# terraytherapeutics/COATI

Hardware: AMD Instinct MI355X
Metric: molecules/sec (contrastive+AR train step), grande_closed (higher is better)
Workload: dtype bf16; 1 GPU; grande_closed d=256 L=16 nh=16 + E3GNN h=256x5, V=10322, batch 1024/GPU, seq_len 80, 16-atom point clouds, InfoNCE + AR loss, bf16 MFMA operands / fp32 accumulate + fp32 master weights, random-init weights; global_batch=1024, seq_len=80, parallelism=dp1

## Files before the change

coati_amd/_lib.py:

```python
import ctypes
import os

from . import _abi
from . import build as _build

try:
    with open(_build.HEADER) as _f:
        _ABI = _abi.parse(_f.read())
except OSError as e:
    raise RuntimeError(f"coati_amd: cannot read {_build.HEADER}, which the binding of libcoati_hip.so is derived from: {e}") from e
try:
    with open(_build.BEAM_HEADER) as _f:
        _BEAM_ABI = _abi.parse(_f.read(), guard="COATI_BEAM_H", name="coati_beam.h", base=_ABI)
except OSError as e:
    raise RuntimeError(f"coati_amd: cannot read {_build.BEAM_HEADER}, which the beam-search binding is derived from: {e}") from e
try:
    with open(_build.SEARCH_HEADER) as _f:
        _SEARCH_ABI = _abi.parse(_f.read(), guard="COATI_SEARCH_H", name="coati_search.h", base=_ABI)
except OSError as e:
    raise RuntimeError(f"coati_amd: cannot read {_build.SEARCH_HEADER}, which the library-search binding is derived from: {e}") from e
try:
    with open(_build.GRAMMAR_HEADER) as _f:
        _GRAMMAR_ABI = _abi.parse(_f.read(), guard="COATI_GRAMMAR_H", name="coati_grammar.h", base=_ABI)
except OSError as e:
    raise RuntimeError(f"coati_amd: cannot read {_build.GRAMMAR_HEADER}, which the constrained-decoding binding is derived from: {e}") from e
try:
    with open(_build.SCREEN_HEADER) as _f:
        _SCREEN_ABI = _abi.parse(_f.read(), guard="COATI_SCREEN_H", name="coati_screen.h", base=_ABI)
except OSError as e:
    raise RuntimeError(f"coati_amd: cannot read {_build.SCREEN_HEADER}, which the property-head binding is derived from: {e}") from e
try:
    with open(_build.GUIDE_HEADER) as _f:
        _GUIDE_ABI = _abi.parse(_f.read(), guard="COATI_GUIDE_H", name="coati_guide.h", base=_ABI)
except OSError as e:
    raise RuntimeError(f"coati_amd: cannot read {_build.GUIDE_HEADER}, which the head-gradient binding is derived from: {e}") from e
try:
    with open(_build.LN_XHAT_HEADER) as _f:
        _LN_XHAT_ABI = _abi.parse(_f.read(), guard="COATI_LN_XHAT_H", name="coati_ln_xhat.h", base=_ABI)
except OSError as e:
    raise RuntimeError(f"coati_amd: cannot read {_build.LN_XHAT_HEADER}, which the saved-xhat binding is derived from: {e}") from e
try:
    with open(_build.GP_HEADER) as _f:
        _GP_ABI = _abi.parse(_f.read(), guard="COATI_GP_H", name="coati_gp.h", base=_ABI)
except OSError as e:
    raise RuntimeError(f"coati_amd: cannot read {_build.GP_HEADER}, which the GP-head binding is derived from: {e}") from e
try:
    with open(_build.ACQ_HEADER) as _f:
        _ACQ_ABI = _abi.parse(_f.read(), guard="COATI_ACQ_H", name="coati_acq.h", base=_ABI)
except OSError as e:
    raise RuntimeError(f"coati_amd: cannot read {_build.ACQ_HEADER}, which the acquisition-gradient binding is derived from: {e}") from e
try:
    with open(_build.CLUSTER_HEADER) as _f:
        _CLUSTER_ABI = _abi.parse(_f.read(), guard="COATI_CLUSTER_H", name="coati_cluster.h", base=_ABI)
except OSError as e:
    raise RuntimeError(f"coati_amd: cannot read {_build.CLUSTER_HEADER}, which the library-clustering binding is derived from: {e}") from e
try:
    with open(_build.IVF_HEADER) as _f:
        _IVF_ABI = _abi.parse(_f.read(), guard="COATI_IVF_H", name="coati_ivf.h", base=_ABI)
except OSError as e:
    raise RuntimeError(f"coati_amd: cannot read {_build.IVF_HEADER}, which the IVF-search binding is derived from: {e}") from e
try:
    with open(_build.RADIUS_HEADER) as _f:
        _RADIUS_ABI = _abi.parse(_f.read(), guard="COATI_RADIUS_H", name="coati_radius.h", base=_ABI)
except OSError as e:
    raise RuntimeError(f"coati_amd: cannot read {_build.RADIUS_HEADER}, which the radius-search binding is derived from: {e}") from e
try:
    with open(_build.GNN_OPS_HEADER) as _f:
        _GNN_OPS_ABI = _abi.parse(_f.read(), guard="COATI_GNN_OPS_H", name="coati_gnn_ops.h", base=_ABI)
except OSError as e:
    raise RuntimeError(f"coati_amd: cannot read {_build.GNN_OPS_HEADER}, which the binding of the point encoder's single kernels is derived from: {e}") from e
try:
    with open(_build.SEARCH8_HEADER) as _f:
        _SEARCH8_ABI = _abi.parse(_f.read(), guard="COATI_SEARCH8_H", name="coati_search8.h", base=_ABI)
except OSError as e:
    raise RuntimeError(f"coati_amd: cannot read {_build.SEARCH8_HEADER}, which the quantised-search binding is derived from: {e}") from e
try:
    with open(_build.IVF8_HEADER) as _f:
        _IVF8_ABI = _abi.parse(_f.read(), guard="COATI_IVF8_H", name="coati_ivf8.h", base=_ABI)
except OSError as e:
    raise RuntimeError(f"coati_amd: cannot read {_build.IVF8_HEADER}, which the binding of the IVF search over fp8 lists is derived from: {e}") from e
try:
    with open(_build.IVF_RADIUS_HEADER) as _f:
        _IVF_RADIUS_ABI = _abi.parse(_f.read(), guard="COATI_IVF_RADIUS_H", name="coati_ivf_radius.h", base=_ABI)
except OSError as e:
    raise RuntimeError(f"coati_amd: cannot read {_build.IVF_RADIUS_HEADER}, which the binding of the radius search over inverted lists is derived from: {e}") from e
try:
    with open(_build.PQ_HEADER) as _f:
        _PQ_ABI = _abi.parse(_f.read(), guard="COATI_PQ_H", name="coati_pq.h", base=_ABI)
except OSError as e:
    raise RuntimeError(f"coati_amd: cannot read {_build.PQ_HEADER}, which the binding of the product-quantised search is derived from: {e}") from e
try:
    with open(_build.IVFPQ_HEADER) as _f:
        _IVFPQ_ABI = _abi.parse(_f.read(), guard="COATI_IVFPQ_H", name="coati_ivfpq.h", base=_ABI)
except OSError as e:
    raise RuntimeError(f"coati_amd: cannot read {_build.IVFPQ_HEADER}, which the binding of the IVF-PQ search is derived from: {e}") from e
try:
    with open(_build.SEARCH4_HEADER) as _f:
        _SEARCH4_ABI = _abi.parse(_f.read(), guard="COATI_SEARCH4_H", name="coati_search4.h", base=_ABI)
except OSError as e:
    raise RuntimeError(f"coati_amd: cannot read {_build.SEARCH4_HEADER}, which the binding of the four-bit search is derived from: {e}") from e

PROTOTYPES = _ABI.prototypes
CoatiConfig = _ABI.CoatiConfig
ABI_VERSION = _ABI.version
BEAM_PROTOTYPES = _BEAM_ABI.prototypes
SEARCH_PROTOTYPES = _SEARCH_ABI.prototypes
GRAMMAR_PROTOTYPES = _GRAMMAR_ABI.prototypes
SCREEN_PROTOTYPES = _SCREEN_ABI.prototypes
GUIDE_PROTOTYPES = _GUIDE_ABI.prototypes
LN_XHAT_PROTOTYPES = _LN_XHAT_ABI.prototypes
GP_PROTOTYPES = _GP_ABI.prototypes
ACQ_PROTOTYPES = _ACQ_ABI.prototypes
CLUSTER_PROTOTYPES = _CLUSTER_ABI.prototypes
IVF_PROTOTYPES = _IVF_ABI.prototypes
RADIUS_PROTOTYPES = _RADIUS_ABI.prototypes
GNN_OPS_PROTOTYPES = _GNN_OPS_ABI.prototypes
SEARCH8_PROTOTYPES = _SEARCH8_ABI.prototypes
IVF8_PROTOTYPES = _IVF8_ABI.prototypes
IVF_RADIUS_PROTOTYPES = _IVF_RADIUS_ABI.prototypes
PQ_PROTOTYPES = _PQ_ABI.prototypes
IVFPQ_PROTOTYPES = _IVFPQ_ABI.prototypes
SEARCH4_PROTOTYPES = _SEARCH4_ABI.prototypes

_lib = None


def has_experimental():
    return hasattr(lib(), "coati_attn_block_fwd")


def lib():
    global _lib
    if _lib is not None:
        return _lib
    path = _build.LIB
    try:
        _build.build(force=os.environ.get("COATI_AMD_REBUILD") == "1", verbose=False)
    except Exception:
        if not os.path.exists(path):
            raise
    if not os.path.exists(path):
        raise RuntimeError(f"coati_amd: {path} is missing and could not be built; there is no CPU fallback")
    import torch
    l = ctypes.CDLL(path)
    for name, (restype, argtypes) in list(PROTOTYPES.items()) + list(BEAM_PROTOTYPES.items()) + list(SEARCH_PROTOTYPES.items()) + list(GRAMMAR_PROTOTYPES.items()) + list(SCREEN_PROTOTYPES.items()) + list(GUIDE_PROTOTYPES.items()) + list(LN_XHAT_PROTOTYPES.items()) + list(GP_PROTOTYPES.items()) + list(ACQ_PROTOTYPES.items()) + list(CLUSTER_PROTOTYPES.items()) + list(IVF_PROTOTYPES.items()) + list(RADIUS_PROTOTYPES.items()) + list(GNN_OPS_PROTOTYPES.items()) + list(SEARCH8_PROTOTYPES.items()) + list(IVF8_PROTOTYPES.items()) + list(IVF_RADIUS_PROTOTYPES.items()) + list(PQ_PROTOTYPES.items()) + list(IVFPQ_PROTOTYPES.items()) + list(SEARCH4_PROTOTYPES.items()):
        if hasattr(l, name):
            getattr(l, name).restype = restype
            getattr(l, name).argtypes = argtypes
    if l.coati_abi_version() != ABI_VERSION:
        raise RuntimeError(f"coati_amd: {path} has ABI version {l.coati_abi_version()}, this package expects {ABI_VERSION}; "
                           "rebuild with `python -m coati_amd.build --force`")
    missing = [n for n in exported_symbols() + sorted(BEAM_PROTOTYPES) + sorted(SEARCH_PROTOTYPES) + sorted(GRAMMAR_PROTOTYPES) + sorted(SCREEN_PROTOTYPES) + sorted(GUIDE_PROTOTYPES) + sorted(LN_XHAT_PROTOTYPES) + sorted(GP_PROTOTYPES) + sorted(ACQ_PROTOTYPES) + sorted(CLUSTER_PROTOTYPES) + sorted(IVF_PROTOTYPES) + sorted(RADIUS_PROTOTYPES) + sorted(GNN_OPS_PROTOTYPES) + sorted(SEARCH8_PROTOTYPES) + sorted(IVF8_PROTOTYPES) + sorted(IVF_RADIUS_PROTOTYPES) + sorted(PQ_PROTOTYPES) + sorted(IVFPQ_PROTOTYPES) + sorted(SEARCH4_PROTOTYPES) if not hasattr(l, n)]
    if missing:
        raise RuntimeError(f"coati_amd: {path} lacks symbols {missing[:6]}; rebuild with `python -m coati_amd.build --force`")
    _lib = l
    return l


def exported_symbols():
    return sorted(n for n in PROTOTYPES if _build.EXPERIMENTAL or n not in _ABI.experimental)


def check(rc, what=""):
    if rc != 0:
        msg = lib().coati_last_error().decode("utf-8", "replace")
        raise RuntimeError(f"libcoati_hip: {what} failed (code {rc}): {msg}")


def call(name, *args):
    if name in _ABI.experimental and not hasattr(lib(), name):
        raise RuntimeError(f"libcoati_hip: {name} is an operator of csrc/experimental/ -- build and load with COATI_AMD_EXPERIMENTAL=1")
    check(getattr(lib(), name)(*args), name)
```

coati_amd/build.py:

```python
import os
import subprocess
import sys
from concurrent.futures import ThreadPoolExecutor

HERE = os.path.dirname(os.path.abspath(__file__))
CSRC = os.path.join(HERE, "csrc")
LIBDIR = os.path.join(HERE, "lib")
LIB = os.path.join(LIBDIR, "libcoati_hip_x.so" if os.environ.get("COATI_AMD_EXPERIMENTAL") == "1" else "libcoati_hip.so")
OBJDIR = os.path.join(HERE, "build")
HEADER = os.path.join(os.path.dirname(HERE), "include", "coati_hip.h")
BEAM_HEADER = os.path.join(os.path.dirname(HERE), "include", "coati_beam.h")
SEARCH_HEADER = os.path.join(os.path.dirname(HERE), "include", "coati_search.h")
GRAMMAR_HEADER = os.path.join(os.path.dirname(HERE), "include", "coati_grammar.h")
SCREEN_HEADER = os.path.join(os.path.dirname(HERE), "include", "coati_screen.h")
GUIDE_HEADER = os.path.join(os.path.dirname(HERE), "include", "coati_guide.h")
LN_XHAT_HEADER = os.path.join(os.path.dirname(HERE), "include", "coati_ln_xhat.h")
GP_HEADER = os.path.join(os.path.dirname(HERE), "include", "coati_gp.h")
ACQ_HEADER = os.path.join(os.path.dirname(HERE), "include", "coati_acq.h")
CLUSTER_HEADER = os.path.join(os.path.dirname(HERE), "include", "coati_cluster.h")
IVF_HEADER = os.path.join(os.path.dirname(HERE), "include", "coati_ivf.h")
RADIUS_HEADER = os.path.join(os.path.dirname(HERE), "include", "coati_radius.h")
GNN_OPS_HEADER = os.path.join(os.path.dirname(HERE), "include", "coati_gnn_ops.h")
SEARCH8_HEADER = os.path.join(os.path.dirname(HERE), "include", "coati_search8.h")
IVF8_HEADER = os.path.join(os.path.dirname(HERE), "include", "coati_ivf8.h")
IVF_RADIUS_HEADER = os.path.join(os.path.dirname(HERE), "include", "coati_ivf_radius.h")
PQ_HEADER = os.path.join(os.path.dirname(HERE), "include", "coati_pq.h")
IVFPQ_HEADER = os.path.join(os.path.dirname(HERE), "include", "coati_ivfpq.h")
SEARCH4_HEADER = os.path.join(os.path.dirname(HERE), "include", "coati_search4.h")
HIP_UNITS = ["gemm.hip", "gemm_rb.hip", "gemm_rb16.hip", "gemm_ring.hip", "gemm_mx8.hip", "norm.hip", "attention.hip", "attention16.hip", "embed.hip", "gnn.hip", "loss.hip", "optim.hip", "batch.hip", "decode.hip", "beam.hip", "search.hip", "grammar.hip", "screen.hip", "guide.hip", "gp.hip", "gp_grad.hip", "cluster.hip", "ivf.hip", "radius.hip", "search8.hip", "ivf8.hip", "ivf_radius.hip", "pq.hip", "ivfpq.hip", "search4.hip"]
CPP_UNITS = ["engine.cpp", "capi.cpp", "tokenizer.cpp", "comm.cpp"]
FLAGS = ["--offload-arch=gfx950", "-O3", "-std=c++17", "-fPIC", "-Wno-unused-value", "-mllvm", "-amdgpu-mfma-vgpr-form=1"] + os.environ.get("COATI_AMD_CXXFLAGS", "").split()


EXPERIMENTAL = os.environ.get("COATI_AMD_EXPERIMENTAL") == "1"
EXPERIMENTAL_UNITS = ["experimental/attn_block.hip", "experimental/mlp64.hip", "experimental/gemm_t32.hip"]
if EXPERIMENTAL:
    HIP_UNITS = HIP_UNITS + EXPERIMENTAL_UNITS
    FLAGS = FLAGS + ["-DCOATI_EXPERIMENTAL"]
UNIT_DROP_FLAGS = {"experimental/mlp64.hip": ("-mllvm", "-amdgpu-mfma-vgpr-form=1")}


def _hipcc():
    for c in (os.environ.get("HIPCC"), "/opt/rocm/bin/hipcc", "hipcc"):
        if c and (os.path.isabs(c) and os.path.exists(c) or not os.path.isabs(c)):
            return c
    return "hipcc"


def _sources():
    deps = [os.path.join(CSRC, f) for f in os.listdir(CSRC) if not os.path.isdir(os.path.join(CSRC, f))]
    if EXPERIMENTAL:
        deps += [os.path.join(CSRC, "experimental", f) for f in os.listdir(os.path.join(CSRC, "experimental"))]
    deps += [HEADER, BEAM_HEADER, SEARCH_HEADER, GRAMMAR_HEADER, SCREEN_HEADER, GUIDE_HEADER, LN_XHAT_HEADER, GP_HEADER, ACQ_HEADER, CLUSTER_HEADER, IVF_HEADER, RADIUS_HEADER, GNN_OPS_HEADER, SEARCH8_HEADER, IVF8_HEADER, IVF_RADIUS_HEADER, PQ_HEADER, IVFPQ_HEADER, SEARCH4_HEADER]
    return deps


def _stamp_path():
    return LIB + ".flags"


def needs_build():
    if not os.path.exists(LIB):
        return True
    try:
        with open(_stamp_path()) as f:
            if f.read() != " ".join(FLAGS):
                return True
    except OSError:
        return True
    t = os.path.getmtime(LIB)
    return any(os.path.getmtime(p) > t for p in _sources())


def build(force=False, verbose=True):
    if not force and not needs_build():
        return LIB
    os.makedirs(LIBDIR, exist_ok=True)
    os.makedirs(OBJDIR, exist_ok=True)
    import fcntl
    with open(os.path.join(LIBDIR, ".build.lock"), "w") as lock:
        fcntl.flock(lock, fcntl.LOCK_EX)
        try:
            if not force and not needs_build():
                return LIB
            return _build_locked(verbose)
        finally:
            fcntl.flock(lock, fcntl.LOCK_UN)


def _build_locked(verbose):
    hipcc = _hipcc()

    def compile_one(unit):
        src = os.path.join(CSRC, unit)
        obj = os.path.join(OBJDIR, unit.replace("/", "_") + (".x.o" if EXPERIMENTAL else ".o"))
        flags = [f for f in FLAGS if f not in UNIT_DROP_FLAGS.get(unit, ())]
        cmd = [hipcc] + flags + (["-x", "hip"] if unit.endswith(".cpp") else []) + ["-c", src, "-o", obj]
        r = subprocess.run(cmd, capture_output=True, text=True)
        if r.returncode != 0:
            raise RuntimeError(f"hipcc failed on {unit}:\n{r.stderr}")
        return obj

    with ThreadPoolExecutor(max_workers=8) as ex:
        objs = list(ex.map(compile_one, HIP_UNITS + CPP_UNITS))
    tmp = LIB + f".tmp{os.getpid()}"
    r = subprocess.run([hipcc, "--offload-arch=gfx950", "-shared", "-fPIC"] + objs + ["-lpthread", "-ldl", "-o", tmp], capture_output=True, text=True)
    if r.returncode != 0:
        raise RuntimeError(f"link failed:\n{r.stderr}")
    os.replace(tmp, LIB)
    with open(_stamp_path(), "w") as f:
        f.write(" ".join(FLAGS))
    if verbose:
        print(f"[coati_amd] built {LIB}", file=sys.stderr)
    return LIB


if __name__ == "__main__":
    build(force="--force" in sys.argv)
```

coati_amd/csrc/capi.cpp:

```cpp
#include <string.h>

#include "../../include/coati_hip.h"
#include "../../include/coati_beam.h"
#include "../../include/coati_search.h"
#include "../../include/coati_grammar.h"
#include "../../include/coati_screen.h"
#include "../../include/coati_guide.h"
#include "../../include/coati_ln_xhat.h"
#include "../../include/coati_gp.h"
#include "../../include/coati_acq.h"
#include "../../include/coati_cluster.h"
#include "../../include/coati_ivf.h"
#include "../../include/coati_radius.h"
#include "../../include/coati_search8.h"
#include "../../include/coati_ivf8.h"
#include "../../include/coati_ivf_radius.h"
#include "../../include/coati_pq.h"
#include "../../include/coati_ivfpq.h"
#include "../../include/coati_search4.h"
#include "../../include/coati_gnn_ops.h"
#include <vector>
#include "kernels.h"

#define S_(x) ((hipStream_t)(x))
#define LL(x) (reinterpret_cast<const long long*>(x))

extern "C" {

int coati_gemm_nt(const void* A, int a_f32, int64_t lda, const uint16_t* B, int64_t ldb, int M, int N, int K,
                  void* C, int64_t ldc, int n_store, const float* bias, const void* aux_in, void* aux_out,
                  int64_t ld_aux, int epi, void* stream) {
  COATI_CHECK_ARG((epi >= EPI_BF16 && epi <= EPI_ACC_F32) || epi == EPI_GELU_GRAD || epi == EPI_MUL_AUX, "coati_gemm_nt: epilogue %d is not a plain epilogue", epi);
  GemmArgs a;
  memset(&a, 0, sizeof(a));
  a.A = A; a.lda = lda; a.B = B; a.ldb = ldb; a.M = M; a.N = N; a.K = K; a.C = C; a.ldc = ldc; a.n_store = n_store;
  a.bias = bias; a.aux_in = aux_in; a.aux_out = aux_out; a.ld_aux = ld_aux;
  return launch_gemm_nt(a, a_f32, epi, S_(stream));
}

#ifdef COATI_EXPERIMENTAL
int coati_mlp_fwd(const float* x, const float* gamma, const float* beta, uint16_t* a2, float* mean, float* rstd, const uint16_t* W1,
                  const float* b1, const uint16_t* W2, const float* b2, uint16_t* g, uint8_t* codes, float* out, int M, void* stream) {
  COATI_CHECK_SHAPE(M >= 1 && M <= 65536, "mlp_fwd: M=%d out of range", M);
  Mlp64Args a;
  a.x = x; a.ldx = 256; a.gamma = gamma; a.beta = beta; a.a2 = a2; a.mean = mean; a.rstd = rstd; a.W1 = W1; a.b1 = b1; a.W2 = W2; a.b2 = b2;
  a.g = g; a.codes = codes; a.out = out; a.ldo = 256; a.M = M;
  return launch_mlp64_fwd(a, S_(stream));
}
#endif

int coati_gemm_lnbwd(const uint16_t* dY, int64_t lda, const uint16_t* WT, int64_t ldw, int M, int K, const float* x, const float* mean,
                     const float* rstd, const float* gamma, const float* dres, float* dx, uint16_t* dx16, float* partial,
                     int32_t* n_partial_rows, const uint16_t* chain_W, uint16_t* chain_C, void* stream) {
  COATI_CHECK_ARG(dY && WT && x && mean && rstd && gamma && dres && dx && partial && n_partial_rows, "gemm_lnbwd: null argument");
  GemmArgs a;
  memset(&a, 0, sizeof(a));
  a.A = dY; a.lda = lda; a.B = WT; a.ldb = ldw; a.M = M; a.N = 256; a.K = K; a.C = dx; a.ldc = 256; a.aux_in = dres; a.ld_aux = 256;
  a.aux_out = dx16; a.lnb_x = x; a.lnb_ldx = 256; a.lnb_mean = mean; a.lnb_rstd = rstd; a.lnb_gamma = gamma; a.lnb_partial = partial;
  COATI_CHECK_ARG((chain_W == nullptr) == (chain_C == nullptr) && (chain_W == nullptr || dx16 != nullptr), "gemm_lnbwd: the chained product needs chain_W, chain_C and dx16");
  a.chain_W = chain_W; a.chain_ldw = 256; a.chain_C = chain_C; a.chain_ldc = 256;
  int nwg = 0;
  COATI_CHECK_SHAPE(gemm_ring_lnbwd_supported(a, &nwg), "gemm_lnbwd: unsupported shape M=%d K=%d (256 columns, 40 961 .. 57 344 rows, K %% 64 == 0)", M, K);
  *n_partial_rows = nwg;
  return launch_gemm_nt(a, 0, EPI_LNBWD, S_(stream));
}

int coati_gemm_lnbwd_xhat(const uint16_t* dY, int64_t lda, const uint16_t* WT, int64_t ldw, int M, int K, const uint16_t* xhat, const float* rstd,
                          const float* gamma, const float* dres, float* dx, uint16_t* dx16, float* partial, int32_t* n_partial_rows,
                          const uint16_t* chain_W, uint16_t* chain_C, void* stream) {
  COATI_CHECK_ARG(dY && WT && xhat && rstd && gamma && dres && dx && partial && n_partial_rows, "gemm_lnbwd_xhat: null argument");
  GemmArgs a;
  memset(&a, 0, sizeof(a));
  a.A = dY; a.lda = lda; a.B = WT; a.ldb = ldw; a.M = M; a.N = 256; a.K = K; a.C = dx; a.ldc = 256; a.aux_in = dres; a.ld_aux = 256;
  a.aux_out = dx16; a.lnb_xhat = xhat; a.lnb_rstd = rstd; a.lnb_gamma = gamma; a.lnb_partial = partial;
  COATI_CHECK_ARG((chain_W == nullptr) == (chain_C == nullptr) && (chain_W == nullptr || dx16 != nullptr), "gemm_lnbwd_xhat: the chained product needs chain_W, chain_C and dx16");
  a.chain_W = chain_W; a.chain_ldw = 256; a.chain_C = chain_C; a.chain_ldc = 256;
  int nwg = 0;
  COATI_CHECK_SHAPE(gemm_ring_lnbwd_supported(a, &nwg), "gemm_lnbwd_xhat: unsupported shape M=%d K=%d (256 columns, 40 961 .. 57 344 rows, K %% 64 == 0)", M, K);
  *n_partial_rows = nwg;
  return launch_gemm_nt(a, 0, EPI_LNBWD, S_(stream));
}

int coati_gemm_ln_gelu_grad(const float* x, int64_t ldx, const float* gamma, const float* beta, const uint16_t* W, int64_t ldw, const float* bias,
                            int M, int N, uint16_t* saved, float* mean, float* rstd, uint16_t* g, uint8_t* codes, int save_xhat, void* stream) {
  COATI_CHECK_ARG(x && gamma && beta && W && saved && mean && rstd && g && codes, "gemm_ln_gelu_grad: null argument");
  COATI_CHECK_SHAPE(M > 0 && N > 0 && N % 16 == 0 && ldx >= 256 && ldx % 4 == 0 && ldw >= 256 && ldw % 8 == 0, "gemm_ln_gelu_grad: shape / alignment (M=%d N=%d ldx=%lld ldw=%lld)", M, N, (long long)ldx, (long long)ldw);
  GemmArgs a;
  memset(&a, 0, sizeof(a));
  a.A = saved; a.lda = 256; a.B = W; a.ldb = ldw; a.M = M; a.N = N; a.K = 256; a.C = g; a.ldc = N; a.bias = bias; a.aux_out = codes; a.ld_aux = N;
  a.ln_x = x; a.ln_ldx = ldx; a.ln_gamma = gamma; a.ln_beta = beta; a.ln_mean = mean; a.ln_rstd = rstd; a.ln_save_xhat = save_xhat ? 1 : 0;
  COATI_CHECK_SHAPE(gemm_rb16_supported(a, 0, EPI_GELU_GRAD), "gemm_ln_gelu_grad: the LayerNorm-fused 16-row-slab kernel takes 36 865 .. 65 536 rows (M=%d N=%d)", M, N);
  return launch_gemm_rb16(a, EPI_GELU_GRAD, S_(stream));
}

int coati_quant_mx8(const void* x, int x_f32, int64_t ldx, uint8_t* q, int64_t ldq, uint8_t* scales, int M, int K, void* stream) {
  return launch_quant_mx8(x, x_f32, ldx, q, ldq, scales, M, K, S_(stream));
}
int coati_gemm_mx8(const uint8_t* A, int64_t lda, const uint8_t* a_scales, const uint8_t* W, int64_t ldw, const uint8_t* w_scales,
                   int M, int N, int K, void* C, int64_t ldc, const float* bias, const void* aux_in, void* aux_out, int64_t ld_aux,
                   int epi, void* stream) {
  GemmArgs a;
  memset(&a, 0, sizeof(a));
  a.A = A; a.lda = lda; a.B = reinterpret_cast<const bf16_t*>(W); a.ldb = ldw; a.M = M; a.N = N; a.K = K; a.C = C; a.ldc = ldc;
  a.bias = bias; a.aux_in = aux_in; a.aux_out = aux_out; a.ld_aux = ld_aux;
  COATI_CHECK_ARG(epi != EPI_QKV_ROPE, "gemm_mx8: the rotary epilogue is an engine-internal call");
  return launch_gemm_mx8(a, a_scales, w_scales, epi, S_(stream));
}
int coati_gemm_ce_partial(const uint16_t* A, int64_t lda, const uint16_t* W, int64_t ldw, int M, int V, int K,
                          void* partial, void* stream) {
  GemmArgs a;
  memset(&a, 0, sizeof(a));
  a.A = A; a.lda = lda; a.B = W; a.ldb = ldw; a.M = M; a.N = V; a.K = K; a.partial = reinterpret_cast<float2*>(partial);
  return launch_gemm_nt(a, 0, EPI_CE_PARTIAL, S_(stream));
}

int coati_ce_finish(const void* partial, int tiles_n, const uint16_t* A, int64_t lda, const uint16_t* W,
                    int64_t ldw, const int64_t* target, float* lse, float* scal, int M, int K, int V, void* stream) {
  return launch_ce_finish(reinterpret_cast<const float2*>(partial), tiles_n, A, lda, W, ldw, LL(target), lse, scal, M, K, V, S_(stream));
}

int coati_gemm_ce_bwd(const uint16_t* A, int64_t lda, const uint16_t* W, int64_t ldw, int M, int V, int K,
                      uint16_t* dlogits, int64_t ldd, int n_store, const float* lse, const int64_t* target,
                      const float* scal, void* stream) {
  GemmArgs a;
  memset(&a, 0, sizeof(a));
  a.A = A; a.lda = lda; a.B = W; a.ldb = ldw; a.M = M; a.N = V; a.K = K; a.C = dlogits; a.ldc = ldd; a.n_store = n_store;
  a.lse = lse; a.target = LL(target); a.scal = scal;
  return launch_gemm_nt(a, 0, EPI_CE_BWD, S_(stream));
}

int coati_wgrad(const void* A, int a_f32, int64_t lda, const uint16_t* B, int64_t ldb, int M, int N, int K,
                float* dW, int64_t ldw, float* dbias, int n_out, void* stream) {
  WgradArgs a;
  a.A = A; a.lda = lda; a.B = B; a.ldb = ldb; a.M = M; a.N = N; a.K = K; a.dW = dW; a.ldw = ldw; a.dbias = dbias; a.n_out = n_out;
  return launch_wgrad(a, a_f32, S_(stream));
}

int64_t coati_wgrad_grouped_workspace_bytes(int n_problems, const int* N, const int* K, int tile_size) {
  if (n_problems <= 0 || !N || !K || (tile_size != 128 && tile_size != 256)) return 0;
  int64_t tiles = 0;
  for (int i = 0; i < n_problems; ++i) tiles += (int64_t)cdiv(N[i], tile_size) * cdiv(K[i], tile_size);
  return tiles * (int64_t)sizeof(WgradTile);
}

int coati_wgrad_grouped(int n_problems, const uint16_t* const* A, const int64_t* lda, const uint16_t* const* B, const int64_t* ldb,
                        int M, const int* N, const int* K, float* const* dW, const int64_t* ldw, float* const* dbias, int tile_size,
                        void* workspace, int64_t workspace_bytes, void* stream) {
  return coati_wgrad_grouped_affine(n_problems, A, lda, B, ldb, M, N, K, dW, ldw, dbias, nullptr, nullptr, tile_size, workspace, workspace_bytes, stream);
}

int coati_wgrad_grouped_affine(int n_problems, const uint16_t* const* A, const int64_t* lda, const uint16_t* const* B, const int64_t* ldb,
                               int M, const int* N, const int* K, float* const* dW, const int64_t* ldw, float* const* dbias,
                               const float* const* b_gamma, const float* const* b_beta, int tile_size, void* workspace, int64_t workspace_bytes,
                               void* stream) {
  COATI_CHECK_ARG(n_problems > 0 && A && lda && B && ldb && N && K && dW && ldw && dbias && workspace, "wgrad_grouped: null argument");
  COATI_CHECK_ARG((b_gamma == nullptr) == (b_beta == nullptr), "wgrad_grouped: b_gamma and b_beta come together");
  std::vector<WgradTile> tab;
  for (int i = 0; i < n_problems; ++i) {
    WgradArgs a;
    a.A = A[i]; a.lda = lda[i]; a.B = B[i]; a.ldb = ldb[i]; a.M = M; a.N = N[i]; a.K = K[i]; a.dW = dW[i]; a.ldw = ldw[i]; a.dbias = dbias[i]; a.n_out = 0;
    if (b_gamma != nullptr) { a.b_gamma = b_gamma[i]; a.b_beta = b_beta[i]; }
    COATI_TRY(wgrad_table_append(tab, a, tile_size));
  }
  COATI_CHECK_ARG((int64_t)(tab.size() * sizeof(WgradTile)) <= workspace_bytes, "wgrad_grouped: workspace too small (%zu tiles)", tab.size());
  hipStream_t s = S_(stream);
  if (hipMemcpyAsync(workspace, tab.data(), tab.size() * sizeof(WgradTile), hipMemcpyHostToDevice, s) != hipSuccess ||
      hipStreamSynchronize(s) != hipSuccess) {
    coati_set_error("wgrad_grouped: table upload failed");
    return COATI_EHIP;
  }
  return launch_wgrad_table(reinterpret_cast<const WgradTile*>(workspace), (int)tab.size(), s, tile_size);
}

int coati_sgemm(const float* A, int64_t ars, int64_t acs, const float* B, int64_t brs, int64_t bcs, float* C,
                int64_t ldc, int M, int N, int K, const float* bias, float alpha, int accumulate, void* stream) {
  return launch_sgemm(A, ars, acs, B, brs, bcs, C, ldc, M, N, K, bias, alpha, accumulate, S_(stream));
}

int coati_layernorm_fwd(const float* x, int64_t ldx, const float* gamma, const float* beta, uint16_t* y16,
                        int64_t ld16, float* y32, int64_t ld32, float* mean, float* rstd, int M, int C, void* stream) {
  return launch_layernorm_fwd(x, ldx, gamma, beta, y16, ld16, y32, ld32, mean, rstd, M, C, S_(stream));
}
int coati_layernorm_bwd(const void* dy, int dy_f32, int64_t lddy, const float* x, int64_t ldx, int x_is_xhat,
                        const float* mean, const float* rstd, const float* gamma, const float* dres, float* dx,
                        uint16_t* dx16, float* dgamma, float* dbeta, float* partial, int M, int C, void* stream) {
  return launch_layernorm_bwd(dy, dy_f32, lddy, x, ldx, x_is_xhat, mean, rstd, gamma, dres, dx, dx16, dgamma, dbeta, partial, M, C, S_(stream));
}

int coati_attn_fwd(const uint16_t* qkv, uint16_t* y, float* lse, int B, int T, int n_head, void* stream) {
  return launch_attn_fwd(qkv, y, lse, B, T, n_head, 16, S_(stream));
}
int coati_attn_fwd_hs(const uint16_t* qkv, uint16_t* y, float* lse, int B, int T, int n_head, int head_size, void* stream) {
  return launch_attn_fwd(qkv, y, lse, B, T, n_head, head_size, S_(stream));
}
int coati_seq_pack(const int64_t* tok, const int64_t* y, int pad_token, int B, int T, int rows_expect, int32_t* off,
                   int32_t* row_src, int32_t* row_t, int64_t* ypk, int32_t* err, void* stream) {
  return launch_seq_pack(LL(tok), LL(y), pad_token, B, T, rows_expect, off, row_src, row_t, reinterpret_cast<long long*>(ypk), err, S_(stream));
}
int coati_attn_fwd_varlen(const uint16_t* qkv, uint16_t* y, float* lse, const int32_t* seq_off, int B, int T, int n_head,
                          int head_size, void* stream) {
  COATI_CHECK_ARG(seq_off, "attn_fwd_varlen: null seq_off");
  return launch_attn_fwd(qkv, y, lse, B, T, n_head, head_size, S_(stream), seq_off);
}
int coati_attn_bwd_varlen(const uint16_t* qkv, const uint16_t* y, const uint16_t* dy, const float* lse, float* dscratch,
                          uint16_t* dqkv, const float* cos_t, const float* sin_t, const int32_t* seq_off, int B, int T,
                          int n_head, int head_size, void* stream) {
  COATI_CHECK_ARG(seq_off, "attn_bwd_varlen: null seq_off");
  return launch_attn_bwd(qkv, y, dy, lse, dscratch, dqkv, cos_t, sin_t, B, T, n_head, head_size, S_(stream), seq_off);
}
#ifdef COATI_EXPERIMENTAL
int coati_attn_groups(const int32_t* seq_off, int B, int T, int32_t* grp, void* stream) {
  return launch_attn_groups(seq_off, B, T, grp, S_(stream));
}
int coati_attn_block_fwd(const float* x, float* xmid, const float* ln_g, const float* ln_b, float* mean, float* rstd, uint16_t* a1,
                         const uint16_t* Wqkv, const float* bqkv, const uint16_t* Wproj, const float* bproj, uint16_t* qkv, uint16_t* y,
                         float* lse, const float* cos_t, const float* sin_t, const int32_t* row_src, const int32_t* grp, int T, int M,
                         void* stream) {
  AttnBlockArgs a;
  a.x = x; a.xmid = xmid; a.ln_g = ln_g; a.ln_b = ln_b; a.mean = mean; a.rstd = rstd; a.a1 = a1; a.Wqkv = Wqkv; a.bqkv = bqkv;
  a.Wproj = Wproj; a.bproj = bproj; a.qkv = qkv; a.y = y; a.lse = lse; a.cos_t = cos_t; a.sin_t = sin_t; a.row_src = row_src;
  a.grp = grp; a.Tl = T; a.M = M;
  return launch_attn_block_fwd(a, S_(stream));
}
int coati_ab_probe_swap(uint32_t* out, void* stream) { return launch_ab_probe_swap(out, S_(stream)); }
#endif
int coati_gemm_qkv_rope(const uint16_t* A, int64_t lda, const uint16_t* W, int64_t ldw, const float* bias, int M, int C,
                        uint16_t* qkv, int64_t ldc, const float* cos_t, const float* sin_t, int T, void* stream) {
  GemmArgs a;
  memset(&a, 0, sizeof(a));
  a.A = A; a.lda = lda; a.B = W; a.ldb = ldw; a.M = M; a.N = 3 * C; a.K = C; a.C = qkv; a.ldc = ldc; a.bias = bias;
  a.rope_cos = cos_t; a.rope_sin = sin_t; a.rope_T = T; a.rope_C = C; a.rope_hs = 16;
  return launch_gemm_nt(a, 0, EPI_QKV_ROPE, S_(stream));
}
int coati_gemm_qkv_rope_hs(const uint16_t* A, int64_t lda, const uint16_t* W, int64_t ldw, const float* bias, int M, int C,
                           uint16_t* qkv, int64_t ldc, const float* cos_t, const float* sin_t, int T, int head_size, void* stream) {
  GemmArgs a;
  memset(&a, 0, sizeof(a));
  a.A = A; a.lda = lda; a.B = W; a.ldb = ldw; a.M = M; a.N = 3 * C; a.K = C; a.C = qkv; a.ldc = ldc; a.bias = bias;
  a.rope_cos = cos_t; a.rope_sin = sin_t; a.rope_T = T; a.rope_C = C; a.rope_hs = head_size;
  return launch_gemm_nt(a, 0, EPI_QKV_ROPE, S_(stream));
}
int coati_attn_bwd(const uint16_t* qkv, const uint16_t* y, const uint16_t* dy, const float* lse, float* dscratch, uint16_t* dqkv,
                   const float* cos_t, const float* sin_t, int B, int T, int n_head, void* stream) {
  return launch_attn_bwd(qkv, y, dy, lse, dscratch, dqkv, cos_t, sin_t, B, T, n_head, 16, S_(stream));
}
int coati_attn_bwd_hs(const uint16_t* qkv, const uint16_t* y, const uint16_t* dy, const float* lse, float* dscratch, uint16_t* dqkv,
                      const float* cos_t, const float* sin_t, int B, int T, int n_head, int head_size, void* stream) {
  return launch_attn_bwd(qkv, y, dy, lse, dscratch, dqkv, cos_t, sin_t, B, T, n_head, head_size, S_(stream));
}

int coati_embed_fwd(const int64_t* idx, const float* table, const float* injection, int unk_token, float* x, int B,
                    int T, int C, int V, void* stream) {
  return launch_embed_fwd(LL(idx), table, injection, unk_token, x, B, T, C, V, S_(stream));
}
int coati_embed_bwd(const int64_t* idx, const float* dx, float* dtable, float* dinjection, int unk_token, int B, int T,
                    int C, int V, void* stream) {
  return launch_embed_bwd(LL(idx), dx, dtable, dinjection, unk_token, B, T, C, V, S_(stream));
}
int coati_find_stop(const int64_t* idx, int stop_token, int32_t* pos, int32_t* err, int B, int T, void* stream) {
  return launch_find_stop(LL(idx), stop_token, pos, err, B, T, S_(stream));
}
int coati_gather_rows(const float* x, const int32_t* pos, float* out, int B, int T, int C, void* stream) {
  return launch_gather_rows(x, pos, out, B, T, C, S_(stream));
}
int coati_scatter_rows_add(const float* dout, const int32_t* pos, float* dx, int B, int T, int C, void* stream) {
  return launch_scatter_rows_add(dout, pos, dx, B, T, C, S_(stream));
}
int coati_bad_rows(const int64_t* tokens, uint8_t* bad, int B, int T, void* stream) {
  return launch_bad_rows(LL(tokens), bad, B, T, S_(stream));
}
int coati_silu(const float* x, float* y, int64_t n, void* stream) { return launch_silu_fwd(x, y, n, S_(stream)); }
int coati_swiglu(const float* u, int64_t ldu, float* g, int64_t ldg, int B, int N, void* stream) {
  return launch_swiglu(u, ldu, g, ldg, B, N, S_(stream));
}
int coati_swiglu_bwd(const float* u, int64_t ldu, const float* dg, int64_t lddg, float* du, int64_t lddu, int B, int N, void* stream) {
  return launch_swiglu_bwd(u, ldu, dg, lddg, du, lddu, B, N, S_(stream));
}
int coati_group_mean_rows(const float* x, int64_t ldx, const int32_t* off, const float* w, const float* fallback, float* out, int G, int E,
                          void* stream) {
  return launch_group_mean_rows(x, ldx, off, w, fallback, out, G, E, S_(stream));
}
int coati_attn_decode(const uint16_t* qkv, uint16_t* cache, uint16_t* y, int B, int n_head, int Tmax, int pos, void* stream) {
  return launch_attn_decode(qkv, cache, y, B, n_head, 16, Tmax, pos, nullptr, S_(stream));
}
int coati_attn_decode_hs(const uint16_t* qkv, uint16_t* cache, uint16_t* y, int B, int n_head, int head_size, int Tmax, int pos, void* stream) {
  return launch_attn_decode(qkv, cache, y, B, n_head, head_size, Tmax, pos, nullptr, S_(stream));
}
int coati_topk_sample(const float* logits, int64_t ldl, int B, int V, int k, float inv_temp, const float* u,
                      int64_t* tokens_out, int32_t* stopped, int stop_token, int pad_token, void* stream) {
  return launch_topk_sample(logits, ldl, B, V, k, inv_temp, u, reinterpret_cast<long long*>(tokens_out), stopped, stop_token, pad_token, S_(stream));
}
int coati_topk_sample_prompt(const float* logits, int64_t ldl, int B, int V, int k, float inv_temp, const float* u, const int64_t* prompt,
                             int64_t ldp, const int32_t* plen, int pos, int64_t* tokens_out, int32_t* stopped, int stop_token, int pad_token,
                             void* stream) {
  return launch_topk_sample_prompt(logits, ldl, B, V, k, inv_temp, u, LL(prompt), ldp, plen, pos, reinterpret_cast<long long*>(tokens_out),
                                   stopped, stop_token, pad_token, S_(stream));
}
int coati_attn_decode_rows(const uint16_t* qkv, uint16_t* cache, uint16_t* y, int B, int n_head, int head_size, int Tmax, const int32_t* pos,
                           void* stream) {
  return launch_attn_decode_rows(qkv, cache, y, B, n_head, head_size, Tmax, pos, S_(stream));
}
int coati_attn_decode_anc(const uint16_t* qkv, uint16_t* cache, uint16_t* y, int B, int n_head, int head_size, int Tmax, int pos,
                          const int32_t* anc, void* stream) {
  return launch_attn_decode_anc(qkv, cache, y, B, n_head, head_size, Tmax, pos, anc, S_(stream));
}
int coati_beam_row_topk(const float* logits, int64_t ldl, int G, int W, int V, const float* cum, const int32_t* fin, int pad_token,
                        float* cand_score, int32_t* cand_tok, void* stream) {
  return launch_beam_row_topk(logits, ldl, G, W, V, cum, fin, pad_token, cand_score, cand_tok, S_(stream));
}
int coati_beam_merge(const float* cand_score, const int32_t* cand_tok, int G, int W, const float* cum_in, const int32_t* fin_in,
                     const int32_t* len_in, const int32_t* anc_in, const int64_t* hist_in, int64_t ldh, int Tmax, int pos, int n,
                     int stop_token, float* cum_out, int32_t* fin_out, int32_t* len_out, int32_t* anc_out, int64_t* hist_out,
                     int64_t* tok_next, int32_t* nfin, void* stream) {
  return launch_beam_merge(cand_score, cand_tok, G, W, cum_in, fin_in, len_in, anc_in, LL(hist_in), ldh, Tmax, pos, n, stop_token, cum_out,
                           fin_out, len_out, anc_out, reinterpret_cast<long long*>(hist_out), reinterpret_cast<long long*>(tok_next), nfin,
                           S_(stream));
}
int coati_search_topk(const uint16_t* lib, int64_t N, int E, const float* bias, const uint16_t* q, int Q, int k, float alpha, int S,
                      float* part_score, int32_t* part_row, float* out_score, int64_t* out_row, void* stream) {
  return launch_search_topk(lib, N, E, bias, q, Q, k, alpha, S, part_score, part_row, out_score, reinterpret_cast<long long*>(out_row),
                            S_(stream));
}
int coati_search_slices(int64_t N, int Q, int k) { return search_slices(N, Q, k); }
int coati_grammar_step(float* logits, int64_t ldl, int B, int V, const uint64_t* table, const int32_t* state_in, int32_t* state_out,
                       const int64_t* tok_prev, const int32_t* parent, int remaining, int stop_token, void* stream) {
  return launch_grammar_step(logits, ldl, B, V, reinterpret_cast<const unsigned long long*>(table), state_in, state_out, LL(tok_prev), parent,
                             remaining, stop_token, S_(stream));
}
int coati_head_eval(const uint16_t* x, int64_t ldx, int64_t N, int E, const uint16_t* w0, const float* b0, const uint16_t* wr, const float* br,
                    int D, const float* wl, const float* bl, int P, int F, float* out, int64_t ldo, void* stream) {
  return launch_head_eval(x, ldx, N, E, w0, b0, wr, br, D, wl, bl, P, F, out, ldo, S_(stream));
}

int coati_head_grad(const uint16_t* x, int64_t ldx, int64_t N, int E, const uint16_t* w0, const float* b0, const uint16_t* wr, const float* br,
                    int D, const float* wl, const float* bl, int P, int F, const uint16_t* w0t, const uint16_t* wrt, const float* cot,
                    int64_t ldc, float* out, int64_t ldo, float* g, int64_t ldg, void* stream) {
  return launch_head_grad(x, ldx, N, E, w0, b0, wr, br, D, wl, bl, P, F, w0t, wrt, cot, ldc, out, ldo, g, ldg, S_(stream));
}
int coati_head_gp(const uint16_t* x, int64_t ldx, int64_t N, int E, const uint16_t* w0, const float* b0, const uint16_t* wr, const float* br,
                  int D, int F, const float* wl, const float* bl, int P_lin, float* out, int64_t ldo, const uint16_t* z, const float* zn,
                  const float* alpha, const float* q, const float* c, float inv2l2, float s2, int P, int Mp, float* mean, int64_t ldm,
                  float* var, void* stream) {
  return launch_head_gp(x, ldx, N, E, w0, b0, wr, br, D, F, wl, bl, P_lin, out, ldo, z, zn, alpha, q, c, inv2l2, s2, P, Mp, mean, ldm, var,
                        S_(stream));
}
int coati_head_gp_grad(const uint16_t* x, int64_t ldx, int64_t N, int E, const uint16_t* w0, const float* b0, const uint16_t* wr,
                       const float* br, int D, int F, const uint16_t* w0t, const uint16_t* wrt, const uint16_t* z, const uint16_t* zt,
                       const float* zn, const float* alpha, const float* qs, const float* c, float inv2l2, float s2, int P, int Mp,
                       const float* wm, float kappa, float var_add, int mode, float best, const float* rs, float* mean, int64_t ldm,
                       float* var, float* acq, float* g, int64_t ldg, void* stream) {
  return launch_head_gp_grad(x, ldx, N, E, w0, b0, wr, br, D, F, w0t, wrt, z, zt, zn, alpha, qs, c, inv2l2, s2, P, Mp, wm, kappa, var_add, mode,
                             best, rs, mean, ldm, var, acq, g, ldg, S_(stream));
}
int coati_cluster_assign(const uint16_t* lib, int64_t N, int E, const float* row_bias, const uint16_t* c, int K, const float* cbias,
                         int32_t* assign, float* best, int blocks, void* stream) {
  return launch_cluster_assign(lib, N, E, row_bias, c, K, cbias, assign, best, blocks, S_(stream));
}
int coati_cluster_sums(const uint16_t* lib, int64_t N, int E, const int32_t* order, int64_t M, const int32_t* offsets,
                       const int32_t* item_off, int K, float* part, int64_t items_max, float* sums, int blocks, void* stream) {
  return launch_cluster_sums(lib, N, E, order, M, offsets, item_off, K, part, items_max, sums, blocks, S_(stream));
}
int coati_cluster_chunk(void) { return cluster_chunk(); }
int64_t coati_cluster_items_max(int64_t M, int K) { return cluster_items_max(M, K); }
int coati_ivf_scan(const uint16_t* lib, const int32_t* ids, const float* bias, const int32_t* list_off, int64_t M, int E, int L,
                   const uint16_t* q, int Q, const int32_t* pair_q, const int32_t* pair_off, const int32_t* item_off, int64_t P, int k,
                   float alpha, int seg_rows, int segs, float* part_score, int32_t* part_row, int blocks, void* stream) {
  return launch_ivf_scan(lib, ids, bias, list_off, M, E, L, q, Q, pair_q, pair_off, item_off, P, k, alpha, seg_rows, segs, part_score, part_row,
                         blocks, S_(stream));
}
int coati_ivf_merge(const float* part_score, const int32_t* part_row, const int32_t* probes, const int32_t* pair_slot, int64_t P,
                    const int32_t* list_off, int L, int Q, int nprobe, int k, int seg_rows, int segs, float* out_score, int64_t* out_row,
                    void* stream) {
  return launch_ivf_merge(part_score, part_row, probes, pair_slot, P, list_off, L, Q, nprobe, k, seg_rows, segs, out_score,
                          reinterpret_cast<long long*>(out_row), S_(stream));
}
int64_t coati_ivf_plan(int64_t max_list_rows, int Q, int nprobe, int k) { return ivf_plan(max_list_rows, Q, nprobe, k); }
int coati_ivf8_scan(const uint8_t* lib8, const float* scale, const int32_t* ids, const float* bias, const int32_t* list_off, int64_t M, int E,
                    int L, const uint8_t* q8, const float* qscale, int Q, const int32_t* pair_q, const int32_t* pair_off,
                    const int32_t* item_off, int64_t P, int k, float alpha, int seg_rows, int segs, float* part_score, int32_t* part_row,
                    int blocks, void* stream) {
  return launch_ivf8_scan(lib8, scale, ids, bias, list_off, M, E, L, q8, qscale, Q, pair_q, pair_off, item_off, P, k, alpha, seg_rows, segs,
                          part_score, part_row, blocks, S_(stream));
}
int coati_radius_count(const uint16_t* lib, int64_t N, int E, const float* bias, const uint16_t* q, int Q, float alpha, const float* sub,
                       int clamp0, const float* thr, const int32_t* row_hi, int S, int32_t* counts, void* stream) {
  return launch_radius_count(lib, N, E, bias, q, Q, alpha, sub, clamp0, thr, row_hi, S, counts, S_(stream));
}
int coati_radius_fill(const uint16_t* lib, int64_t N, int E, const float* bias, const uint16_t* q, int Q, float alpha, const float* sub,
                      int clamp0, const float* thr, const int32_t* row_hi, int S, const int32_t* counts, const int64_t* offsets,
                      float* out_score, int64_t* out_row, void* stream) {
  return launch_radius_fill(lib, N, E, bias, q, Q, alpha, sub, clamp0, thr, row_hi, S, counts, LL(offsets), out_score,
                            reinterpret_cast<long long*>(out_row), S_(stream));
}
int coati_radius_slices(int64_t N, int Q) { return radius_slices(N, Q); }
int coati_ivf_radius_count(const uint16_t* lib, const int32_t* ids, const float* bias, const int32_t* list_off, int64_t M, int E, int L,
                           const uint16_t* q, int Q, const int32_t* pair_q, const int32_t* pair_off, const int32_t* item_off, int64_t P,
                           float alpha, const float* sub, int clamp0, const float* thr, const int32_t* row_hi, int seg_rows, int segs,
                           int32_t* counts, int blocks, void* stream) {
  return launch_ivf_radius_count(lib, ids, bias, list_off, M, E, L, q, Q, pair_q, pair_off, item_off, P, alpha, sub, clamp0, thr, row_hi, seg_rows,
                                 segs, counts, blocks, S_(stream));
}
int coati_ivf_radius_fill(const uint16_t* lib, const int32_t* ids, const float* bias, const int32_t* list_off, int64_t M, int E, int L,
                          const uint16_t* q, int Q, const int32_t* pair_q, const int32_t* pair_off, const int32_t* item_off, int64_t P,
                          float alpha, const float* sub, int clamp0, const float* thr, const int32_t* row_hi, int seg_rows, int segs,
                          const int32_t* counts, const int64_t* offsets, float* out_score, int64_t* out_row, int blocks, void* stream) {
  return launch_ivf_radius_fill(lib, ids, bias, list_off, M, E, L, q, Q, pair_q, pair_off, item_off, P, alpha, sub, clamp0, thr, row_hi, seg_rows,
                                segs, counts, LL(offsets), out_score, reinterpret_cast<long long*>(out_row), blocks, S_(stream));
}
int coati_quant_rows_fp8(const uint16_t* x, int64_t n, int E, uint8_t* out, float* scale, void* stream) {
  return launch_quant_rows_fp8(x, n, E, out, scale, S_(stream));
}
int coati_search8_topk(const uint8_t* lib8, const float* scale, int64_t N, int E, const float* bias, const uint8_t* q8, const float* qscale,
                       int Q, int k, float alpha, int S, float* part_score, int32_t* part_row, float* out_score, int64_t* out_row,
                       void* stream) {
  return launch_search8_topk(lib8, scale, N, E, bias, q8, qscale, Q, k, alpha, S, part_score, part_row, out_score,
                             reinterpret_cast<long long*>(out_row), S_(stream));
}
int coati_search_rescore(const uint16_t* lib, int64_t N, int E, const float* bias, const uint16_t* q, int Q, const int64_t* cand, int R, int k,
                         float alpha, float* out_score, int64_t* out_row, void* stream) {
  return launch_search_rescore(lib, N, E, bias, q, Q, LL(cand), R, k, alpha, out_score, reinterpret_cast<long long*>(out_row), S_(stream));
}
int coati_search8_slices(int64_t N, int Q, int k) { return search8_slices(N, Q, k); }
int coati_pq_encode(const uint16_t* x, int64_t n, int E, const uint16_t* codebook, uint8_t* codes, void* stream) {
  return launch_pq_encode(x, n, E, codebook, codes, S_(stream));
}
int coati_pq_topk(const uint8_t* codes, int64_t N, int E, const uint16_t* codebook, const float* bias, const uint16_t* q, int Q, int k,
                  float alpha, int S, float* part_score, int32_t* part_row, float* out_score, int64_t* out_row, void* stream) {
  return launch_pq_topk(codes, N, E, codebook, bias, q, Q, k, alpha, S, part_score, part_row, out_score, reinterpret_cast<long long*>(out_row),
                        S_(stream));
}
int coati_pq_k_max(int E) { return pq_k_max(E); }
int coati_pq_slices(int64_t N, int E, int Q, int k) { return pq_slices(N, E, Q, k); }
int coati_ivfpq_scan(const uint8_t* codes, const int32_t* ids, const float* bias, const int32_t* list_off, int64_t M, int E, int L,
                     const uint16_t* centres, const uint16_t* codebook, const uint16_t* q, int Q, const int32_t* pair_q,
                     const int32_t* pair_off, const int32_t* item_off, int64_t P, int k, float alpha, int seg_rows, int segs,
                     float* part_score, int32_t* part_row, int blocks, void* stream) {
  return launch_ivfpq_scan(codes, ids, bias, list_off, M, E, L, centres, codebook, q, Q, pair_q, pair_off, item_off, P, k, alpha, seg_rows, segs,
                           part_score, part_row, blocks, S_(stream));
}
int coati_ivfpq_k_max(int E) { return ivfpq_k_max(E); }
int coati_quant_rows_fp4(const uint16_t* x, int64_t n, int E, uint8_t* codes, uint8_t* scales, void* stream) {
  return launch_quant_rows_fp4(x, n, E, codes, scales, S_(stream));
}
int coati_search4_topk(const uint8_t* codes, const uint8_t* scales, int64_t N, int E4, const float* bias, const uint8_t* q8,
                       const float* qscale, int Q, int k, float alpha, int S, float* part_score, int32_t* part_row, float* out_score,
                       int64_t* out_row, void* stream) {
  return launch_search4_topk(codes, scales, N, E4, bias, q8, qscale, Q, k, alpha, S, part_score, part_row, out_score,
                             reinterpret_cast<long long*>(out_row), S_(stream));
}
int coati_search4_slices(int64_t N, int Q, int k) { return search4_slices(N, Q, k); }
int coati_topk_sample_rows(const float* logits, int64_t ldl, int B, int V, int k, float inv_temp, const float* u, int64_t ldu,
                           const int64_t* prompt, int64_t ldp, const int32_t* plen, const int32_t* req, int32_t* pos, int64_t* out, int64_t ldo,
                           int64_t* tok_next, int32_t* done, int Tmax, int stop_token, void* stream) {
  return launch_topk_sample_rows(logits, ldl, B, V, k, inv_temp, u, ldu, LL(prompt), ldp, plen, req, pos, reinterpret_cast<long long*>(out), ldo,
                                 reinterpret_cast<long long*>(tok_next), done, Tmax, stop_token, S_(stream));
}
int coati_batch_ncols(const int64_t* tokens, int B, int n_seq, int32_t* ncols, void* stream) {
  return launch_batch_ncols(LL(tokens), B, n_seq, ncols, S_(stream));
}
int coati_batch_tail(const int64_t* tokens, int B, int n_seq, int ncol, int64_t* tokens_out, int64_t* y_next_out,
                     const int64_t* masked_ids, int n_masked, void* stream) {
  return launch_batch_tail(LL(tokens), B, n_seq, ncol, reinterpret_cast<long long*>(tokens_out),
                           reinterpret_cast<long long*>(y_next_out), LL(masked_ids), n_masked, S_(stream));
}

int coati_gnn_embed(const int64_t* atoms, const int32_t* lut_ix, const int32_t* lut_iy, const float* W, const float* b,
                    float* h32, uint16_t* h16, int64_t ld16, float* rstd, float* mask, int BA, int H, void* stream) {
  return launch_gnn_embed(LL(atoms), lut_ix, lut_iy, W, b, h32, h16, ld16, rstd, mask, BA, H, S_(stream));
}
int coati_gnn_geom(const float* coords, const float* mask, float cutoff, float* d2, float* w, int B, int A, void* stream) {
  return launch_gnn_geom(coords, mask, cutoff, d2, w, B, A, S_(stream));
}
int coati_gnn_compact(const float* w_dense, const float* d2_dense, int32_t* seg, int32_t* n_edges, int32_t* e_bj, int32_t* e_bk,
                      int32_t* e_rev, float* e_d2, float* e_w, int32_t* pos, int B, int A, void* stream) {
  return launch_gnn_compact(w_dense, d2_dense, seg, n_edges, e_bj, e_bk, e_rev, e_d2, e_w, pos, B, A, S_(stream));
}

int coati_gnn_edge_pre(const uint16_t* P, int64_t ldp, const int32_t* seg, const int32_t* e_bk, const float* e_d2, const float* w1c,
                       int64_t w1c_stride, const float* b1, uint16_t* e1, int BA, int H, void* stream) {
  return launch_gnn_edge_pre_c(P, ldp, seg, e_bk, e_d2, w1c, w1c_stride, b1, e1, BA, H, S_(stream));
}
int coati_gnn_edge_reduce(const uint16_t* s2, const int32_t* seg, const float* e_w, uint16_t* mi, int64_t ldmi, int BA, int H, void* stream) {
  return launch_gnn_edge_reduce_c(s2, seg, e_w, mi, ldmi, BA, H, S_(stream));
}

int coati_gnn_edge_fwd_fused(const uint16_t* P, int64_t ldp, const int32_t* seg, const int32_t* e_bk, const float* e_d2, const float* e_w,
                             const float* w1c, int64_t w1c_stride, const float* b1, const uint16_t* W3, int64_t ldw, const float* b3,
                             uint16_t* e1, uint16_t* s2, uint16_t* mi, int64_t ldmi, int BA, int H, void* stream) {
  return launch_gnn_edge_fwd_fused(P, ldp, seg, e_bk, e_d2, e_w, w1c, w1c_stride, b1, W3, ldw, b3, e1, s2, mi, ldmi, BA, H, S_(stream));
}
int coati_gnn_edge_reduce_bwd(const uint16_t* dmi, int64_t lddmi, const uint16_t* s2, const int32_t* seg, const float* e_w, uint16_t* ds2,
                              int BA, int H, void* stream) {
  COATI_CHECK_SHAPE(BA > 0 && H > 0, "gnn_edge_reduce_bwd: empty problem");
  return launch_gnn_edge_reduce_bwd_c(dmi, lddmi, s2, seg, e_w, ds2, BA, H, S_(stream));
}
int coati_gnn_edge_pre_bwd(const uint16_t* dpre, const int32_t* seg, const int32_t* e_rev, const float* e_d2, uint16_t* dP, int64_t lddp,
                           float* dw1c, int64_t dw1c_stride, float* db1, int BA, int H, void* stream) {
  COATI_CHECK_SHAPE(BA > 0 && H > 0, "gnn_edge_pre_bwd: empty problem");
  return launch_gnn_edge_pre_bwd_c(dpre, seg, e_rev, e_d2, dP, lddp, dw1c, dw1c_stride, db1, BA, H, S_(stream));
}
int coati_gnn_node_res_silu(const float* u32, const int64_t* atoms, const int32_t* lut_ix, const int32_t* lut_iy, const float* W3c,
                            int64_t ldw, uint16_t* upre, uint16_t* t16, int BA, int H, void* stream) {
  COATI_CHECK_SHAPE(BA > 0 && H > 0, "gnn_node_res_silu: empty problem");
  return launch_gnn_node_res_silu(u32, LL(atoms), lut_ix, lut_iy, W3c, ldw, upre, t16, BA, H, S_(stream));
}
int coati_gnn_onehot_wgrad(const int64_t* atoms, const int32_t* lut_ix, const int32_t* lut_iy, const uint16_t* du, float* dW, int64_t ldw,
                           int BA, int H, void* stream) {
  COATI_CHECK_SHAPE(BA > 0 && H > 0, "gnn_onehot_wgrad: empty problem");
  return launch_gnn_onehot_wgrad(LL(atoms), lut_ix, lut_iy, du, dW, ldw, BA, H, S_(stream));
}
int coati_gnn_embed_bwd(const int64_t* atoms, const int32_t* lut_ix, const int32_t* lut_iy, const float* de, float* dW, float* db, int BA,
                        int H, void* stream) {
  COATI_CHECK_SHAPE(BA > 0 && H > 0, "gnn_embed_bwd: empty problem");
  return launch_gnn_embed_bwd(LL(atoms), lut_ix, lut_iy, de, dW, db, BA, H, S_(stream));
}
int coati_gnn_readout(const float* o, const float* mask, float* hp, int B, int A, int H, void* stream) {
  COATI_CHECK_SHAPE(B > 0 && A > 0 && H > 0, "gnn_readout: empty problem");
  return launch_gnn_readout(o, mask, hp, B, A, H, S_(stream));
}
int coati_gnn_readout_bwd(const float* dhp, const float* mask, uint16_t* dout, int B, int A, int H, void* stream) {
  COATI_CHECK_SHAPE(B > 0 && A > 0 && H > 0, "gnn_readout_bwd: empty problem");
  return launch_gnn_readout_bwd(dhp, mask, dout, B, A, H, S_(stream));
}
int coati_gemm_rows_dev(const int32_t* m_dev, const uint16_t* A, int64_t lda, const uint16_t* B, int64_t ldb, int M, int N, int K,
                        uint16_t* C, int64_t ldc, const float* bias, int epi, const uint16_t* P, int64_t ldp, const float* d2,
                        const float* w1c, int64_t w1c_stride, const float* b1, int natom, int H, const int32_t* e_bj,
                        const int32_t* e_bk, int32_t* resident, void* stream) {
  COATI_CHECK_ARG(m_dev && A && B && C && resident, "gemm_rows_dev: null argument");
  COATI_CHECK_ARG(epi == EPI_BF16 || epi == EPI_EDGE_DPRE, "gemm_rows_dev: epilogue %d (EPI_BF16 and EPI_EDGE_DPRE only)", epi);
  COATI_CHECK_SHAPE(M > 0 && N > 0 && K > 0, "gemm_rows_dev: empty problem");
  if (epi == EPI_EDGE_DPRE)
    COATI_CHECK_ARG(N == H && (e_bj == nullptr) == (e_bk == nullptr), "gemm_rows_dev: EPI_EDGE_DPRE needs N == H (N=%d H=%d) and e_bj with e_bk", N, H);
  GemmArgs a;
  memset(&a, 0, sizeof(a));
  a.m_dev = m_dev; a.A = A; a.lda = lda; a.B = B; a.ldb = ldb; a.M = M; a.N = N; a.K = K; a.C = C; a.ldc = ldc; a.bias = bias;
  a.P = P; a.ldp = ldp; a.d2 = d2; a.w1c = w1c; a.w1c_stride = w1c_stride; a.b1 = b1; a.natom = natom; a.H = H; a.e_bj = e_bj; a.e_bk = e_bk;
  *resident = gemm_rb16_resident_supported(a, 0, epi) ? 1 : 0;
  return launch_gemm_nt(a, 0, epi, S_(stream));
}
int coati_wgrad_rows_dev(const int32_t* m_dev, const uint16_t* A, int64_t lda, const uint16_t* B, int64_t ldb, int M, int N, int K,
                         float* dW, int64_t ldw, float* dbias, void* stream) {
  COATI_CHECK_ARG(m_dev, "wgrad_rows_dev: null m_dev");
  WgradArgs a;
  a.A = A; a.lda = lda; a.B = B; a.ldb = ldb; a.M = M; a.N = N; a.K = K; a.dW = dW; a.ldw = ldw; a.dbias = dbias; a.n_out = 0; a.m_dev = m_dev;
  return launch_wgrad(a, 0, S_(stream));
}
int64_t coati_wgrad_split_workspace_bytes(int n_problems, const int* N, const int* K, int n_splits) {
  if (n_problems <= 0 || !N || !K || n_splits < 1) return 0;
  int64_t entries = 0;
  for (int i = 0; i < n_problems; ++i) entries += (int64_t)cdiv(N[i], 128) * cdiv(K[i], 128) * n_splits;
  return entries * (int64_t)sizeof(WgradTile);
}
int coati_wgrad_split(int n_problems, const uint16_t* const* A, const int64_t* lda, const uint16_t* const* B, const int64_t* ldb, int M,
                      const int* N, const int* K, float* const* dW, const int64_t* ldw, float* const* dbias, int n_splits,
                      void* workspace, int64_t workspace_bytes, void* stream) {
  COATI_CHECK_ARG(n_problems > 0 && A && lda && B && ldb && N && K && dW && ldw && dbias && workspace, "wgrad_split: null argument");
  COATI_CHECK_ARG(n_splits >= 1, "wgrad_split: n_splits=%d", n_splits);
  std::vector<WgradTile> tab;
  for (int i = 0; i < n_problems; ++i) {
    WgradArgs a;
    a.A = A[i]; a.lda = lda[i]; a.B = B[i]; a.ldb = ldb[i]; a.M = M; a.N = N[i]; a.K = K[i]; a.dW = dW[i]; a.ldw = ldw[i]; a.dbias = dbias[i]; a.n_out = 0;
    COATI_TRY(wgrad_table_append_split(tab, a, n_splits));
  }
  COATI_CHECK_ARG((int64_t)(tab.size() * sizeof(WgradTile)) <= workspace_bytes, "wgrad_split: workspace too small (%zu entries)", tab.size());
  hipStream_t s = S_(stream);
  if (hipMemcpyAsync(workspace, tab.data(), tab.size() * sizeof(WgradTile), hipMemcpyHostToDevice, s) != hipSuccess ||
      hipStreamSynchronize(s) != hipSuccess) {
    coati_set_error("wgrad_split: table upload failed");
    return COATI_EHIP;
  }
  return launch_wgrad_split_table(reinterpret_cast<const WgradTile*>(workspace), (int)tab.size(), s);
}

int coati_infonce_rows(float* logits, int64_t ld, int R, int N, int label0, const uint8_t* bad, float* loss_sum,
                       const float* inv_count, float gscale, void* stream) {
  return launch_infonce_rows(logits, ld, R, N, label0, bad, loss_sum, inv_count, gscale, S_(stream));
}

int coati_count_valid(const uint8_t* bad, int n, float* count, float* inv, void* stream) {
  return launch_count_valid(bad, n, count, inv, S_(stream));
}
int coati_colsum2(const float* a, const float* b2, const uint8_t* bad, float* out, int B, int E, void* stream) {
  return launch_colsum2(a, b2, bad, out, B, E, S_(stream));
}
int coati_center_rows(const float* z, const uint8_t* bad, const float* sum, const float* count, float* zc, int B, int E, void* stream) {
  return launch_center_rows(z, bad, sum, count, zc, B, E, S_(stream));
}
int coati_standardize(const float* z, const uint8_t* bad, const float* stats, const float* count, float* zt, float* rsigma,
                      int B, int E, void* stream) {
  return launch_standardize(z, bad, stats, count, zt, rsigma, B, E, S_(stream));
}
int coati_barlow_dc(float* C, const float* count, float lam, float* loss, int E, void* stream) {
  return launch_barlow_dc(C, count, lam, loss, E, S_(stream));
}
int coati_standardize_bwd(const float* dzt, const float* zt, const uint8_t* bad, const float* rsigma, const float* m,
                          const float* count, float scale, float* dz, int B, int E, void* stream) {
  return launch_standardize_bwd(dzt, zt, bad, rsigma, m, count, scale, dz, B, E, S_(stream));
}

int coati_grad_sqnorm(const float* g, int64_t n, float* partial, int n_partial, float* out_norm, float max_norm,
                      float* out_coef, void* stream) {
  return launch_grad_sqnorm(g, n, partial, n_partial, out_norm, max_norm, out_coef, S_(stream));
}
int coati_adamw(float* p, const float* g, float* m, float* v, uint16_t* shadow, int64_t n, float lr, float b1, float b2,
                float eps, float wd, int step, const float* coef, float gscale, void* stream) {
  return launch_adamw(p, g, m, v, shadow, n, lr, b1, b2, eps, wd, step, coef, gscale, S_(stream));
}

}
```

coati_amd/csrc/embed.hip:

```cpp
#include "kernels.h"

__global__ __launch_bounds__(256) void embed_fwd_kernel(const long long* __restrict__ idx, const float* __restrict__ table,
                                                        const float* __restrict__ injection, int unk, float* __restrict__ x,
                                                        int M, int T, int C, int V, const int* __restrict__ row_src, int mode) {
  const int lane = threadIdx.x & 63, wave = threadIdx.x >> 6;
  const int m = blockIdx.x * 4 + wave;
  if (m >= M) return;
  const int ms = row_src ? row_src[m] : m;
  long long tok = idx[ms];
  const float* src;
  if (mode != 0) {
    if (tok != unk) return;
    float* dstz = x + (long long)m * C;
    if (mode == 2) {
      for (int c = lane * 4; c < C; c += 256) *reinterpret_cast<float4*>(dstz + c) = make_float4(0.f, 0.f, 0.f, 0.f);
      return;
    }
    src = injection + (long long)(ms / T) * C;
  } else if (injection != nullptr && tok == unk) {
    src = injection + (long long)(ms / T) * C;
  } else {
    if (tok < 0) tok = 0;
    if (tok >= V) tok = V - 1;
    src = table + tok * C;
  }
  float* dst = x + (long long)m * C;
  for (int c = lane * 4; c < C; c += 256) *reinterpret_cast<float4*>(dst + c) = *reinterpret_cast<const float4*>(src + c);
}

int launch_embed_fwd(const long long* idx, const float* table, const float* injection, int unk_token, float* x,
                     int B, int T, int C, int V, hipStream_t s, const int* row_src, int rows, int mode) {
  COATI_CHECK_ARG(idx && x && (mode != 0 || table) && (mode != 1 || injection) && mode >= 0 && mode <= 2, "embed_fwd: null operand / bad mode");
  COATI_CHECK_SHAPE(B > 0 && T > 0 && C % 4 == 0 && V > 0, "embed_fwd: unsupported shape");
  const int M = row_src ? rows : B * T;
  hipLaunchKernelGGL(embed_fwd_kernel, dim3(cdiv(M, 4)), dim3(256), 0, s, idx, table, injection, unk_token, x, M, T, C, V, row_src, mode);
  COATI_LAUNCH_CHECK("embed_fwd");
  return COATI_OK;
}

#define EMB_RUN 32
__global__ __launch_bounds__(256) void embed_bwd_kernel(const long long* __restrict__ idx, const float* __restrict__ dx,
                                                        float* __restrict__ dtable, float* __restrict__ dinj, int unk,
                                                        int B, int T, int C, int V, const int* __restrict__ off, int inj_only) {
  const int lane = threadIdx.x & 63, wave = threadIdx.x >> 6;
  const int t = blockIdx.x;
  const int b0 = (blockIdx.y * 4 + wave) * EMB_RUN;
  if (b0 >= B) return;
  const int b1 = (b0 + EMB_RUN < B) ? b0 + EMB_RUN : B;
  for (int c0 = 0; c0 < C; c0 += 256) {
    float* cur = nullptr;
    float acc[4] = {0.f, 0.f, 0.f, 0.f};
    auto flush = [&]() {
      if (cur == nullptr) return;
#pragma unroll
      for (int i = 0; i < 4; ++i) {
        const int c = c0 + lane + 64 * i;
        if (c < C && acc[i] != 0.f) atomicAdd(cur + c, acc[i]);
      }
    };
    for (int b = b0; b < b1; ++b) {
      long long m = (long long)b * T + t;
      long long tok = idx[m];
      if (off != nullptr) {
        const int o = off[b];
        if (t >= off[b + 1] - o) continue;
        m = o + t;
      }
      float* dst;
      if (inj_only && tok != unk) continue;
      if (dinj != nullptr && tok == unk) {
        dst = dinj + (long long)b * C;
      } else {
        if (tok < 0) tok = 0;
        if (tok >= V) tok = V - 1;
        dst = dtable + tok * C;
      }
      float g[4];
#pragma unroll
      for (int i = 0; i < 4; ++i) {
        const int c = c0 + lane + 64 * i;
        g[i] = c < C ? dx[m * C + c] : 0.f;
      }
      if (dst != cur) {
        flush();
        cur = dst;
#pragma unroll
        for (int i = 0; i < 4; ++i) acc[i] = g[i];
      } else {
#pragma unroll
        for (int i = 0; i < 4; ++i) acc[i] += g[i];
      }
    }
    flush();
  }
}

int launch_embed_bwd(const long long* idx, const float* dx, float* dtable, float* dinjection, int unk_token,
                     int B, int T, int C, int V, hipStream_t s, const int* off, int inj_only) {
  COATI_CHECK_ARG(idx && dx && (dtable || inj_only) && (!inj_only || dinjection), "embed_bwd: null operand");
  COATI_CHECK_SHAPE(B > 0 && T > 0 && C % 4 == 0 && V > 0, "embed_bwd: unsupported shape");
  hipLaunchKernelGGL(embed_bwd_kernel, dim3(T, cdiv(B, 4 * EMB_RUN)), dim3(256), 0, s, idx, dx, dtable, dinjection, unk_token, B, T, C, V, off, inj_only);
  COATI_LAUNCH_CHECK("embed_bwd");
  return COATI_OK;
}

__global__ __launch_bounds__(256) void find_stop_kernel(const long long* __restrict__ idx, int stop, int* __restrict__ pos, int* __restrict__ err,
                                                        int B, int T) {
  const int lane = threadIdx.x & 63, b = blockIdx.x * 4 + (threadIdx.x >> 6);
  if (b >= B) return;
  int n = 0, p = 0;
  for (int t0 = 0; t0 < T; t0 += 64) {
    const int t = t0 + lane;
    const bool hit = t < T && idx[(long long)b * T + t] == stop;
    const unsigned long long m = __ballot(hit);
    if (m != 0ull) {
      if (n == 0) p = t0 + __builtin_ctzll(m);
      n += __builtin_popcountll(m);
    }
  }
  if (lane == 0) {
    pos[b] = p;
    if (n != 1) atomicOr(err, 1);
  }
}

int launch_find_stop(const long long* idx, int stop_token, int* pos, int* err, int B, int T, hipStream_t s) {
  COATI_CHECK_ARG(idx && pos && err, "find_stop: null operand");
  hipLaunchKernelGGL(find_stop_kernel, dim3(cdiv(B, 4)), dim3(256), 0, s, idx, stop_token, pos, err, B, T);
  COATI_LAUNCH_CHECK("find_stop");
  return COATI_OK;
}

__global__ __launch_bounds__(256) void gather_rows_kernel(const float* __restrict__ x, const int* __restrict__ pos,
                                                          float* __restrict__ out, int B, int T, int C, const int* __restrict__ off) {
  const int lane = threadIdx.x & 63, b = blockIdx.x * 4 + (threadIdx.x >> 6);
  if (b >= B) return;
  const float* src = x + ((off ? (long long)off[b] : (long long)b * T) + pos[b]) * C;
  for (int c = lane * 4; c < C; c += 256) *reinterpret_cast<float4*>(out + (long long)b * C + c) = *reinterpret_cast<const float4*>(src + c);
}

int launch_gather_rows(const float* x, const int* pos, float* out, int B, int T, int C, hipStream_t s, const int* off) {
  COATI_CHECK_ARG(x && pos && out, "gather_rows: null operand");
  hipLaunchKernelGGL(gather_rows_kernel, dim3(cdiv(B, 4)), dim3(256), 0, s, x, pos, out, B, T, C, off);
  COATI_LAUNCH_CHECK("gather_rows");
  return COATI_OK;
}

__global__ __launch_bounds__(256) void scatter_rows_add_kernel(const float* __restrict__ dout, const int* __restrict__ pos,
                                                               float* __restrict__ dx, int B, int T, int C, const int* __restrict__ off) {
  const int lane = threadIdx.x & 63, b = blockIdx.x * 4 + (threadIdx.x >> 6);
  if (b >= B) return;
  float* dst = dx + ((off ? (long long)off[b] : (long long)b * T) + pos[b]) * C;
  for (int c = lane * 4; c < C; c += 256) {
    float4 d = *reinterpret_cast<float4*>(dst + c);
    const float4 g = *reinterpret_cast<const float4*>(dout + (long long)b * C + c);
    d.x += g.x; d.y += g.y; d.z += g.z; d.w += g.w;
    *reinterpret_cast<float4*>(dst + c) = d;
  }
}

__global__ __launch_bounds__(256) void scatter_rows_bf16_kernel(const bf16_t* __restrict__ src, const int* __restrict__ pos,
                                                                bf16_t* __restrict__ dst, int B, int T, int C, const int* __restrict__ off) {
  const int lane = threadIdx.x & 63, b = blockIdx.x * 4 + (threadIdx.x >> 6);
  if (b >= B) return;
  bf16_t* d = dst + ((off ? (long long)off[b] : (long long)b * T) + pos[b]) * C;
  for (int c = lane * 8; c < C; c += 512) *reinterpret_cast<uint4*>(d + c) = *reinterpret_cast<const uint4*>(src + (long long)b * C + c);
}
int launch_scatter_rows_bf16(const bf16_t* src, const int* pos, bf16_t* dst, int B, int T, int C, hipStream_t s, const int* off) {
  COATI_CHECK_ARG(src && pos && dst && C % 8 == 0, "scatter_rows_bf16: null operand / C % 8");
  hipLaunchKernelGGL(scatter_rows_bf16_kernel, dim3(cdiv(B, 4)), dim3(256), 0, s, src, pos, dst, B, T, C, off);
  COATI_LAUNCH_CHECK("scatter_rows_bf16");
  return COATI_OK;
}

int launch_scatter_rows_add(const float* dout, const int* pos, float* dx, int B, int T, int C, hipStream_t s, const int* off) {
  COATI_CHECK_ARG(dout && pos && dx, "scatter_rows_add: null operand");
  hipLaunchKernelGGL(scatter_rows_add_kernel, dim3(cdiv(B, 4)), dim3(256), 0, s, dout, pos, dx, B, T, C, off);
  COATI_LAUNCH_CHECK("scatter_rows_add");
  return COATI_OK;
}

__global__ __launch_bounds__(256) void seq_len_kernel(const long long* __restrict__ tok, const long long* __restrict__ y, int pad,
                                                      int* __restrict__ len, int B, int T) {
  const int lane = threadIdx.x & 63, b = blockIdx.x * 4 + (threadIdx.x >> 6);
  if (b >= B) return;
  int last = 0;
  for (int t = lane; t < T; t += 64) {
    const bool live = tok[(long long)b * T + t] != pad || (y != nullptr && y[(long long)b * T + t] >= 0);
    if (live) last = t + 1;
  }
#pragma unroll
  for (int o = 32; o > 0; o >>= 1) { const int v = __shfl_xor(last, o, 64); last = v > last ? v : last; }
  if (lane == 0) len[b] = last;
}
__global__ __launch_bounds__(1024) void seq_scan_kernel(int* __restrict__ off, int B, int expect, int* __restrict__ err, int* __restrict__ ord) {
  __shared__ int part[1024];
  __shared__ int cnt[10], cur[10];
  const int t = threadIdx.x, per = (B + 1023) / 1024;
  const int lo = t * per, hi = lo + per < B ? lo + per : B;
  if (t < 10) cnt[t] = 0;
  __syncthreads();
  int sum = 0;
  for (int i = lo; i < hi; ++i) {
    const int l = off[i];
    sum += l;
    if (ord != nullptr) { const int nb = (l + 15) >> 4; atomicAdd(&cnt[9 - (nb < 9 ? nb : 9)], 1); }
  }
  part[t] = sum;
  __syncthreads();
  if (t == 0) { int run = 0; for (int k = 0; k < 10; ++k) { cur[k] = run; run += cnt[k]; } }
  for (int o = 1; o < 1024; o <<= 1) {
    const int v = t >= o ? part[t - o] : 0;
    __syncthreads();
    part[t] += v;
    __syncthreads();
  }
  int run = part[t] - sum;
  for (int i = lo; i < hi; ++i) {
    const int l = off[i];
    off[i] = run;
    run += l;
    if (ord != nullptr) { const int nb = (l + 15) >> 4; ord[atomicAdd(&cur[9 - (nb < 9 ? nb : 9)], 1)] = i; }
  }
  if (t == 1023) {
    off[B] = part[1023];
    if (part[1023] != expect) atomicOr(err, 2);
  }
}
__global__ void seq_fill_kernel(const int* __restrict__ off, const long long* __restrict__ y, int* __restrict__ row_src,
                                int* __restrict__ row_t, long long* __restrict__ ypk, int B, int T, int cap) {
  const long long g = (long long)blockIdx.x * blockDim.x + threadIdx.x;
  if (g >= (long long)B * T) return;
  {
    const long long m = (long long)off[B] + g;
    if (m < cap) {
      row_src[m] = 0;
      row_t[m] = 0;
      if (ypk != nullptr) ypk[m] = -1;
    }
  }
  const int b = (int)(g / T), t = (int)(g - (long long)b * T);
  const int o = off[b];
  if (t >= off[b + 1] - o) return;
  const int m = o + t;
  if (m >= cap) return;
  row_src[m] = (int)g;
  row_t[m] = t;
  if (ypk != nullptr) ypk[m] = y[g];
}
int launch_seq_pack(const long long* tok, const long long* y, int pad_token, int B, int T, int rows_expect, int* off,
                    int* row_src, int* row_t, long long* ypk, int* err, hipStream_t s, int* ord) {
  COATI_CHECK_ARG(tok && off && row_src && row_t && err && (ypk == nullptr || y != nullptr), "seq_pack: null operand");
  COATI_CHECK_SHAPE(B > 0 && T > 0 && rows_expect > 0 && rows_expect <= (long long)B * T, "seq_pack: bad row count %d for %d x %d", rows_expect, B, T);
  hipLaunchKernelGGL(seq_len_kernel, dim3(cdiv(B, 4)), dim3(256), 0, s, tok, y, pad_token, off, B, T);
  hipLaunchKernelGGL(seq_scan_kernel, dim3(1), dim3(1024), 0, s, off, B, rows_expect, err, ord);
  hipLaunchKernelGGL(seq_fill_kernel, dim3(cdiv((long long)B * T, 256)), dim3(256), 0, s, off, y, row_src, row_t, ypk, B, T, rows_expect);
  COATI_LAUNCH_CHECK("seq_pack");
  return COATI_OK;
}

int launch_seq_pack_len(const int* len, int B, int T, int rows_expect, int* off, int* row_src, int* row_t, int* err, hipStream_t s, int* ord) {
  COATI_CHECK_ARG(len && off && row_src && row_t && err, "seq_pack_len: null operand");
  COATI_CHECK_SHAPE(B > 0 && T > 0 && rows_expect > 0 && rows_expect <= (long long)B * T, "seq_pack_len: bad row count %d for %d x %d", rows_expect, B, T);
  hipError_t h = hipMemcpyAsync(off, len, sizeof(int) * B, hipMemcpyDeviceToDevice, s);
  if (h != hipSuccess) { coati_set_error("seq_pack_len: hipMemcpyAsync failed: %s", hipGetErrorString(h)); return COATI_EHIP; }
  hipLaunchKernelGGL(seq_scan_kernel, dim3(1), dim3(1024), 0, s, off, B, rows_expect, err, ord);
  hipLaunchKernelGGL(seq_fill_kernel, dim3(cdiv((long long)B * T, 256)), dim3(256), 0, s, off, (const long long*)nullptr, row_src, row_t,
                     (long long*)nullptr, B, T, rows_expect);
  COATI_LAUNCH_CHECK("seq_pack_len");
  return COATI_OK;
}

__global__ void bad_rows_kernel(const long long* __restrict__ tok, unsigned char* __restrict__ bad, int B, int T) {
  const int b = blockIdx.x * blockDim.x + threadIdx.x;
  if (b >= B) return;
  long long sum = 0;
  for (int t = 0; t < T; ++t) sum += tok[(long long)b * T + t];
  bad[b] = sum < 1 ? 1 : 0;
}

int launch_bad_rows(const long long* tokens, unsigned char* bad, int B, int T, hipStream_t s) {
  COATI_CHECK_ARG(tokens && bad, "bad_rows: null operand");
  hipLaunchKernelGGL(bad_rows_kernel, dim3(cdiv(B, 128)), dim3(128), 0, s, tokens, bad, B, T);
  COATI_LAUNCH_CHECK("bad_rows");
  return COATI_OK;
}

__device__ __forceinline__ float ce_target_logit(const bf16_t* __restrict__ a, long long lda, const bf16_t* __restrict__ W, long long ldw,
                                                 long long tgt, long long row, int C, int lane) {
  float dot = 0.f;
  for (int c = lane * 4; c < C; c += 256) {
    const uint2 ua = *reinterpret_cast<const uint2*>(a + row * lda + c);
    const uint2 uw = *reinterpret_cast<const uint2*>(W + tgt * ldw + c);
    dot += bflo(ua.x) * bflo(uw.x) + bfhi(ua.x) * bfhi(uw.x) + bflo(ua.y) * bflo(uw.y) + bfhi(ua.y) * bfhi(uw.y);
  }
  return wave_sum(dot);
}
__device__ __forceinline__ float ce_row(const float2* __restrict__ partial, int tiles_n, const bf16_t* __restrict__ a, long long lda,
                                        const bf16_t* __restrict__ W, long long ldw, long long tgt, long long row, int C, int V,
                                        float* __restrict__ lse_out, int lane, bool* valid) {
  float mx = -INFINITY;
  for (int t = lane; t < tiles_n; t += 64) mx = fmaxf(mx, partial[row * tiles_n + t].x);
  mx = wave_max(mx);
  float sm = 0.f;
  for (int t = lane; t < tiles_n; t += 64) {
    const float2 p = partial[row * tiles_n + t];
    sm += p.y * __expf(p.x - mx);
  }
  sm = wave_sum(sm);
  const float l = mx + __logf(sm);
  if (lse_out != nullptr && lane == 0) *lse_out = l;
  *valid = tgt >= 0 && tgt < V;
  if (!*valid) return 0.f;
  return l - ce_target_logit(a, lda, W, ldw, tgt, row, C, lane);
}

__global__ __launch_bounds__(256) void ce_finish_kernel(const float2* __restrict__ partial, int tiles_n,
                                                        const bf16_t* __restrict__ a, long long lda,
                                                        const bf16_t* __restrict__ W, long long ldw,
                                                        const long long* __restrict__ target, float* __restrict__ lse,
                                                        float* __restrict__ scal, int M, int C, int V) {
  __shared__ float red[2][4];
  const int lane = threadIdx.x & 63, wave = threadIdx.x >> 6;
  float loss_acc = 0.f, cnt_acc = 0.f;
  for (int row = blockIdx.x * 4 + wave; row < M; row += gridDim.x * 4) {
    bool valid;
    const float d = ce_row(partial, tiles_n, a, lda, W, ldw, target[row], row, C, V, lse + row, lane, &valid);
// ... 149 lines not shown
```

coati_amd/csrc/engine.cpp:

```cpp
#include <stdarg.h>
#include <stdio.h>
#include <stdlib.h>
#include <string.h>

#include <algorithm>
#include <string>
#include <vector>

#include "../../include/coati_hip.h"
#include "../../include/coati_beam.h"
#include "../../include/coati_ln_xhat.h"
#include "kernels.h"

#define HIPCHK(x) do { hipError_t _h = (x); if (_h != hipSuccess) { coati_set_error("%s: %s", #x, hipGetErrorString(_h)); return COATI_EHIP; } } while (0)

static thread_local char g_err[512] = "";
void coati_set_error(const char* fmt, ...) {
  va_list ap;
  va_start(ap, fmt);
  vsnprintf(g_err, sizeof(g_err), fmt, ap);
  va_end(ap);
}
extern "C" const char* coati_last_error(void) { return g_err; }
extern "C" int coati_abi_version(void) { return COATI_ABI_VERSION; }
// ... 882 lines not shown
    }
    COATI_TRY(gemm(e, SITE_FC2_FWD, p.g[l], 0, 4 * C, e->S + w.fc2w, 4 * C, M, C, 4 * C, p.x[l + 1], C, e->P + w.fc2b, EPI_RES_F32, p.xmid[l], nullptr, C, s));
  }
  float* const y32 = (&p == &e->p1) ? p.xf32 : nullptr;
  ProfScope ps(e, SITE_LN_FWD, 0, s, (double)M * C * (y32 ? 8 : 6) + (double)M * 8);
  return launch_layernorm_fwd(p.x[L], C, e->P + e->lnfw, e->P + e->lnfb, y32 ? nullptr : p.af, C, y32, C, p.meanf, p.rstdf, M, C, s);
}

int upload_table(coati_engine* e, int hslot, const std::vector<WgradTile>& tab, WgradTile* dst, hipStream_t s, const char* what) {
  const size_t n = tab.size();
  if (e->h_tab_ev[hslot] == nullptr && hipEventCreateWithFlags(&e->h_tab_ev[hslot], hipEventDisableTiming) != hipSuccess) {
    coati_set_error("%s: event creation failed", what);
    return COATI_EHIP;
  } else if (e->h_tab[hslot] != nullptr && hipEventSynchronize(e->h_tab_ev[hslot]) != hipSuccess) {
    coati_set_error("%s: waiting for the previous upload failed", what);
    return COATI_EHIP;
  }
  if (e->h_tab_cap[hslot] < n) {
    if (e->h_tab[hslot] != nullptr) hipHostFree(e->h_tab[hslot]);
    e->h_tab[hslot] = nullptr;
    if (hipHostMalloc(reinterpret_cast<void**>(&e->h_tab[hslot]), n * sizeof(WgradTile), hipHostMallocDefault) != hipSuccess) {
      coati_set_error("%s: pinned staging allocation failed", what);
      return COATI_EHIP;
    }
    e->h_tab_cap[hslot] = n;
  }
  memcpy(e->h_tab[hslot], tab.data(), n * sizeof(WgradTile));
  if (hipMemcpyAsync(dst, e->h_tab[hslot], n * sizeof(WgradTile), hipMemcpyHostToDevice, s) != hipSuccess || hipEventRecord(e->h_tab_ev[hslot], s) != hipSuccess) {
    coati_set_error("%s: table upload failed", what);
    return COATI_EHIP;
  }
  return COATI_OK;
}

int xformer_wgrad_group(coati_engine* e, XPass& p, int l_lo, int l_hi, hipStream_t s) {
  const int C = e->cfg.n_hidden_xformer, M = p.M, Mtab = p.Mcap;
  const long long sig = e->carve_sig * 2 + (p.tail ? 1 : 0);
  const bool affine_ok = e->wg_tile == 256 && C == 256;
  COATI_CHECK_ARG(!p.ln_xhat || affine_ok, "wgrad group: a1 / a2 hold xhat and the %d-wide tiles cannot apply gamma / beta (C=%d)", e->wg_tile, C);
  int slot = -1;
  for (int i = 0; i < 4; ++i)
    if (e->wtab_key[i].pass == &p && e->wtab_key[i].lo == l_lo && e->wtab_key[i].hi == l_hi && e->wtab_key[i].M == Mtab && e->wtab_key[i].sig == sig) slot = i;
  double flops = 0.0, bytes = 0.0;
  for (int l = l_lo; l < l_hi; ++l) {
    flops += 2.0 * M * (3.0 + 1.0 + 4.0 + 4.0) * C * C;
    bytes += (double)M * (3 + 1 + 1 + 1 + 4 + 1 + 1 + 4) * C * 2 + 12.0 * C * C * 8;
  }
  if (slot < 0) {
    std::vector<WgradTile> tab;
    auto add = [&](const bf16_t* A, int lda, const bf16_t* B, int ldb, int N, int K, int64_t w_off, int64_t b_off, int64_t ln_g = -1, int64_t ln_b = -1) -> int {
      WgradArgs a;
      a.A = A; a.lda = lda; a.B = B; a.ldb = ldb; a.M = Mtab; a.N = N; a.K = K; a.dW = e->G + w_off; a.ldw = K; a.dbias = e->G + b_off; a.n_out = 0;
      if (ln_g >= 0 && affine_ok) { a.b_gamma = e->P + ln_g; a.b_beta = e->P + ln_b; }
      return wgrad_table_append(tab, a, e->wg_tile);
    };
    for (int l = l_hi - 1; l >= l_lo; --l) {
      const XLayerP& w = e->xl[l];
      COATI_TRY(add(e->w_dqkv[l], 3 * C, p.a1[l], C, 3 * C, C, w.attnw, w.attnb, w.ln1w, w.ln1b));
      COATI_TRY(add(e->w_dxb[l], C, p.y[l], C, C, C, w.projw, w.projb));
      if (p.tail && l == e->cfg.n_layer_xformer - 1) continue;
      COATI_TRY(add(e->w_dh4[l], 4 * C, p.a2[l], C, 4 * C, C, w.fc1w, w.fc1b, w.ln2w, w.ln2b));
      COATI_TRY(add(e->w_dxa[l], C, p.g[l], 4 * C, C, 4 * C, w.fc2w, w.fc2b));
    }
    COATI_CHECK_ARG((int)tab.size() <= e->wtab_cap, "wgrad group: table overflow (%zu > %d)", tab.size(), e->wtab_cap);
    slot = e->wtab_rr++ & 3;
    COATI_TRY(upload_table(e, slot, tab, e->d_wtab + (size_t)slot * e->wtab_cap, s, "wgrad group"));
    coati_engine::WTabKey k;
    k.pass = &p; k.lo = l_lo; k.hi = l_hi; k.M = Mtab; k.n = (int)tab.size(); k.sig = sig;
    e->wtab_key[slot] = k;
  }
  ProfScope ps(e, SITE_XF_WGRAD, flops, s, bytes);
  return launch_wgrad_table(e->d_wtab + (size_t)slot * e->wtab_cap, e->wtab_key[slot].n, s, e->wg_tile, M, p.ln_xhat ? 1 : 0);
}

int xformer_bwd(coati_engine* e, XPass& p, const void* dyf, int dyf_f32, float* dinjection, hipStream_t s, int l_hi = -1, int l_lo = 0,
                const bf16_t* lmh_dlogits = nullptr, bool inputs_only = false) {
  const coati_config& c = e->cfg;
  const int C = c.n_hidden_xformer, L = c.n_layer_xformer, M = p.M;
  if (l_hi < 0) l_hi = L;
  float* DX = e->DX;
  const bool defer = 2 * L + 1 <= COATI_LN_MAX_SLOTS;
  const long long slot_stride = (long long)COATI_LN_PARTIAL_ROWS * 2 * C;
  LnFinishBatch fin;
  memset(&fin, 0, sizeof(fin));
  int nblk = 0;
  auto ln_bwd = [&](const void* dy, int dy_f32, const float* x, const float* mean, const float* rstd, const float* gamma,
                    const float* dres, size_t goff, size_t boff, bf16_t* dx16) -> int {
    if (!defer && inputs_only) return launch_layernorm_bwd(dy, dy_f32, C, x, C, 0, mean, rstd, gamma, dres, DX, dx16, nullptr, nullptr, e->ln_partial, M, C, s);
    if (!defer) return launch_layernorm_bwd(dy, dy_f32, C, x, C, 0, mean, rstd, gamma, dres, DX, dx16, e->G + goff, e->G + boff, e->ln_partial, M, C, s);
    fin.dg_off[fin.n] = (long long)goff;
    fin.db_off[fin.n] = (long long)boff;
    return launch_layernorm_bwd_deferred(dy, dy_f32, C, x, C, 0, mean, rstd, gamma, dres, DX, dx16, e->ln_part_x + (fin.n++) * slot_stride, &nblk, M, C, s);
  };
  auto dgrad_lnbwd = [&](int site, const bf16_t* dY, int K, const bf16_t* WT, const float* x, const bf16_t* xhat, const float* mean, const float* rstd,
                         const float* gamma, size_t goff, size_t boff, bf16_t* dx16, const bf16_t* chainW = nullptr,
                         bf16_t* chainC = nullptr, bool has_dres = true) -> int {
    if (!defer || c.use_fp8) return 0;
    GemmArgs a;
    memset(&a, 0, sizeof(a));
    a.A = dY; a.lda = K; a.B = WT; a.ldb = K; a.M = M; a.N = C; a.K = K; a.C = DX; a.ldc = C; a.aux_in = has_dres ? DX : nullptr; a.ld_aux = C; a.aux_out = dx16;
    a.lnb_rstd = rstd; a.lnb_gamma = gamma;
    if (xhat != nullptr) a.lnb_xhat = xhat;
    else { a.lnb_x = x; a.lnb_ldx = C; a.lnb_mean = mean; }
    if (chainW != nullptr && dx16 != nullptr) { a.chain_W = chainW; a.chain_ldw = C; a.chain_C = chainC; a.chain_ldc = C; }
    int nwg = 0;
    if (!lnbwd_rows_supported(a, &nwg) || nwg > COATI_LN_PARTIAL_ROWS) return 0;
    a.lnb_partial = e->ln_part_x + fin.n * slot_stride;
    fin.dg_off[fin.n] = (long long)goff;
    fin.db_off[fin.n] = (long long)boff;
    fin.nblk[fin.n] = nwg;
    ++fin.n;
    ProfScope ps(e, site, 2.0 * M * C * K + (a.chain_W ? 2.0 * M * C * C : 0.0), s,
                 (double)M * K * 2 + (double)C * K * 2 + (double)M * C * ((xhat ? 2 : 4) + (has_dres ? 4 : 0) + 4 + (dx16 ? 2 : 0)) + (a.chain_W ? (double)M * C * 2 + (double)C * C * 2 : 0.0));
    const int rc = gemm_rows(a, 0, EPI_LNBWD, s);
    return rc == COATI_OK ? 1 : rc;
  };
  const bool grp = e->wg_group && M >= 4096 && !inputs_only;
  const bool wg_each = !grp && !inputs_only;
  COATI_CHECK_ARG(!(wg_each && p.ln_xhat), "xformer_bwd: a1 / a2 hold xhat; the per-Linear weight gradients take the Linear's input");
  COATI_CHECK_ARG(!inputs_only || (!p.tail && !c.use_fp8 && dinjection != nullptr), "xformer_bwd: the inputs-only backward serves a full bf16 pass with an injection");
  if (l_hi == L && p.tail) {
    ProfScope ps(e, SITE_XF_TAIL, 0, s, (double)p.B * C * ((dyf_f32 ? 4 : 2) + 4 + 4 + 2));
    COATI_TRY(launch_layernorm_bwd(dyf, dyf_f32, C, p.t_xL, C, 0, p.t_meanf, p.t_rstdf, e->P + e->lnfw, nullptr, e->t_dx, e->t_dxa, e->G + e->lnfw, e->G + e->lnfb, e->ln_partial, p.B, C, s));
  } else if (l_hi == L) {
    int lnf_fused = 0;
    if (lmh_dlogits != nullptr) {
      lnf_fused = dgrad_lnbwd(SITE_LMHEAD_DGRAD, lmh_dlogits, e->Vpad, e->S + e->lmheadT, p.x[L], nullptr, p.meanf, p.rstdf, e->P + e->lnfw, e->lnfw, e->lnfb,
                              grp ? e->w_dxa[L - 1] : e->DX16, nullptr, nullptr, false);
      if (lnf_fused < 0) return lnf_fused;
      if (!lnf_fused) COATI_TRY(gemm(e, SITE_LMHEAD_DGRAD, lmh_dlogits, 0, e->Vpad, e->S + e->lmheadT, e->Vpad, M, C, e->Vpad, e->da, C, nullptr, EPI_BF16, nullptr, nullptr, 0, s));
    }
    if (!lnf_fused) {
      ProfScope ps(e, SITE_LN_BWD, 0, s, (double)M * C * ((dyf_f32 ? 4 : 2) + 4 + 4 + 2));
      COATI_TRY(ln_bwd(dyf, dyf_f32, p.x[L], p.meanf, p.rstdf, e->P + e->lnfw, nullptr, e->lnfw, e->lnfb, grp ? e->w_dxa[L - 1] : e->DX16));
    }
  }
  for (int l = l_hi - 1; l >= l_lo; --l) {
    const XLayerP& w = e->xl[l];
    bf16_t* const dxa = grp ? e->w_dxa[l] : e->DX16;
    bf16_t* const dxb = grp ? e->w_dxb[l] : e->DX16;
    bf16_t* const dh4 = grp ? e->w_dh4[l] : e->dh4;
    bf16_t* const dqkv = grp ? e->w_dqkv[l] : e->dqkv;
    bf16_t* const dx_out = l == 0 ? nullptr : (grp ? e->w_dxa[l - 1] : e->DX16);
    int ln2_fused = 0, ln1_fused = 0;
    if (p.tail && l == L - 1) {
      const int Bt = p.B;
      COATI_TRY(gemm(e, SITE_XF_TAIL, e->t_dxa, 0, C, e->S + w.fc2T, C, Bt, 4 * C, C, e->t_dh4, 4 * C, nullptr, EPI_MUL_AUX, p.t_hpre, nullptr, 4 * C, s));
      COATI_TRY(gemm(e, SITE_XF_TAIL, e->t_dh4, 0, 4 * C, e->S + w.fc1T, 4 * C, Bt, C, 4 * C, e->t_da, C, nullptr, EPI_BF16, nullptr, nullptr, 0, s));
      COATI_TRY(wgrad(e, SITE_XF_TAIL, e->t_dh4, 0, 4 * C, p.t_a2, C, Bt, 4 * C, C, e->G + w.fc1w, C, e->G + w.fc1b, 0, s));
      COATI_TRY(wgrad(e, SITE_XF_TAIL, e->t_dxa, 0, C, p.t_g, 4 * C, Bt, C, 4 * C, e->G + w.fc2w, 4 * C, e->G + w.fc2b, 0, s));
      {
        ProfScope ps(e, SITE_XF_TAIL, 0, s, (double)Bt * C * (2 + 4 + 4 + 4 + 2));
        COATI_TRY(launch_layernorm_bwd(e->t_da, 0, C, p.t_xmid, C, 0, p.t_mean2, p.t_rstd2, e->P + w.ln2w, e->t_dx, e->t_dx, e->t_dxb, e->G + w.ln2w, e->G + w.ln2b, e->ln_partial, Bt, C, s));
        if (hipMemsetAsync(DX, 0, (size_t)M * C * sizeof(float), s) != hipSuccess || hipMemsetAsync(dxb, 0, (size_t)M * C * sizeof(bf16_t), s) != hipSuccess) {
          coati_set_error("xformer_bwd: hipMemsetAsync failed");
          return COATI_EHIP;
        }
        COATI_TRY(launch_scatter_rows_add(e->t_dx, e->stop_pos, DX, Bt, p.T, C, s, p.packed ? p.off : nullptr));
        COATI_TRY(launch_scatter_rows_bf16(e->t_dxb, e->stop_pos, dxb, Bt, p.T, C, s, p.packed ? p.off : nullptr));
      }
    } else {
      if (c.use_fp8) {
        GemmArgs a;
        memset(&a, 0, sizeof(a));
        a.C = dh4; a.ldc = 4 * C; a.aux_in = p.hpre[l]; a.ld_aux = 4 * C;
        COATI_TRY(gemm8(e, SITE_FC2_DGRAD, w, 7, dxa, C, M, 4 * C, C, a, EPI_MUL_AUX, s, true));
        memset(&a, 0, sizeof(a));
        a.C = e->da; a.ldc = C;
        COATI_TRY(gemm8(e, SITE_FC1_DGRAD, w, 6, nullptr, 4 * C, M, C, 4 * C, a, EPI_BF16, s));
      } else {
      COATI_TRY(gemm(e, SITE_FC2_DGRAD, dxa, 0, C, e->S + w.fc2T, C, M, 4 * C, C, dh4, 4 * C, nullptr, EPI_MUL_AUX, p.hpre[l], nullptr, 4 * C, s));
      ln2_fused = dgrad_lnbwd(SITE_FC1_DGRAD, dh4, 4 * C, e->S + w.fc1T, p.xmid[l], p.ln_xhat ? p.a2[l] : nullptr, p.mean2[l], p.rstd2[l], e->P + w.ln2w, w.ln2w, w.ln2b, dxb,
                              e->S + w.projT, e->dyb);
      if (ln2_fused < 0) return ln2_fused;
      if (!ln2_fused) COATI_TRY(gemm(e, SITE_FC1_DGRAD, dh4, 0, 4 * C, e->S + w.fc1T, 4 * C, M, C, 4 * C, e->da, C, nullptr, EPI_BF16, nullptr, nullptr, 0, s));
      }
      if (wg_each) {
        COATI_TRY(wgrad(e, SITE_XF_WGRAD, dh4, 0, 4 * C, p.a2[l], C, M, 4 * C, C, e->G + w.fc1w, C, e->G + w.fc1b, 0, s));
        COATI_TRY(wgrad(e, SITE_XF_WGRAD, dxa, 0, C, p.g[l], 4 * C, M, C, 4 * C, e->G + w.fc2w, 4 * C, e->G + w.fc2b, 0, s));
      }
      if (!ln2_fused) {
        ProfScope ps(e, SITE_LN_BWD, 0, s, (double)M * C * (2 + 4 + 4 + 4 + 2));
        COATI_TRY(ln_bwd(e->da, 0, p.xmid[l], p.mean2[l], p.rstd2[l], e->P + w.ln2w, DX, w.ln2w, w.ln2b, dxb));
      }
    }
    if (c.use_fp8) {
      GemmArgs a;
      memset(&a, 0, sizeof(a));
      a.C = e->dyb; a.ldc = C;
      COATI_TRY(gemm8(e, SITE_PROJ_DGRAD, w, 5, dxb, C, M, C, C, a, EPI_BF16, s));
    } else if (!ln2_fused) {
    COATI_TRY(gemm(e, SITE_PROJ_DGRAD, dxb, 0, C, e->S + w.projT, C, M, C, C, e->dyb, C, nullptr, EPI_BF16, nullptr, nullptr, 0, s));
    }
    if (wg_each) COATI_TRY(wgrad(e, SITE_XF_WGRAD, dxb, 0, C, p.y[l], C, M, C, C, e->G + w.projw, C, e->G + w.projb, 0, s));
    {
      ProfScope ps(e, SITE_ATTN_BWD, 10.0 * M * (double)p.T * C, s, (double)M * 8 * C * 2 + (double)M * c.n_head * 8);
      COATI_TRY(launch_attn_bwd(p.qkv[l], p.y[l], e->dyb, p.lse[l], e->attnD, dqkv, e->cos_t, e->sin_t, p.B, p.T, c.n_head, C / c.n_head, s, p.packed ? p.off : nullptr, p.packed ? p.ord : nullptr));
    }
    if (c.use_fp8) {
      GemmArgs a;
      memset(&a, 0, sizeof(a));
      a.C = e->da; a.ldc = C;
      COATI_TRY(gemm8(e, SITE_QKV_DGRAD, w, 4, dqkv, 3 * C, M, C, 3 * C, a, EPI_BF16, s));
    } else {
    ln1_fused = dgrad_lnbwd(SITE_QKV_DGRAD, dqkv, 3 * C, e->S + w.attnT, p.x[l], p.ln_xhat ? p.a1[l] : nullptr, p.mean1[l], p.rstd1[l], e->P + w.ln1w, w.ln1w, w.ln1b, dx_out);
    if (ln1_fused < 0) return ln1_fused;
    if (!ln1_fused) COATI_TRY(gemm(e, SITE_QKV_DGRAD, dqkv, 0, 3 * C, e->S + w.attnT, 3 * C, M, C, 3 * C, e->da, C, nullptr, EPI_BF16, nullptr, nullptr, 0, s));
    }
    if (wg_each) COATI_TRY(wgrad(e, SITE_XF_WGRAD, dqkv, 0, 3 * C, p.a1[l], C, M, 3 * C, C, e->G + w.attnw, C, e->G + w.attnb, 0, s));
    if (!ln1_fused) {
      ProfScope ps(e, SITE_LN_BWD, 0, s, (double)M * C * (2 + 4 + 4 + 4 + 2));
      COATI_TRY(ln_bwd(e->da, 0, p.x[l], p.mean1[l], p.rstd1[l], e->P + w.ln1w, DX, w.ln1w, w.ln1b, dx_out));
    }
  }
  if (grp && l_hi > l_lo) COATI_TRY(xformer_wgrad_group(e, p, l_lo, l_hi, s));
  if (defer && fin.n > 0 && !inputs_only) {
    ProfScope ps(e, SITE_LN_BWD, 0, s, 0.0);
    COATI_TRY(launch_ln_finish_batched(e->ln_part_x, slot_stride, nblk, e->G, fin, C, s));
  }
  if (l_lo > 0) return COATI_OK;
  ProfScope ps(e, SITE_EMBED, 0, s);
  if (inputs_only) return launch_embed_bwd(p.idx, DX, nullptr, dinjection, c.unk_token, p.B, p.T, C, c.n_tok, s, p.packed ? p.off : nullptr, 1);
  if (c.norm_embed) {
    if (dinjection != nullptr) {
      COATI_TRY(launch_embed_bwd(p.idx, DX, nullptr, dinjection, c.unk_token, p.B, p.T, C, c.n_tok, s, p.packed ? p.off : nullptr, 1));
      COATI_TRY(launch_embed_fwd(p.idx, nullptr, nullptr, c.unk_token, DX, p.B, p.T, C, c.n_tok, s, p.packed ? p.row_src : nullptr, M, 2));
    }
    COATI_TRY(launch_layernorm_bwd(DX, 1, C, p.x_emb, C, 0, p.mean0, p.rstd0, e->P + e->emb_lnw, nullptr, p.x[0], nullptr, e->G + e->emb_lnw, e->G + e->emb_lnb,
                                   e->ln_partial, M, C, s));
    return launch_embed_bwd(p.idx, p.x[0], e->G + e->tok_emb, nullptr, c.unk_token, p.B, p.T, C, c.n_tok, s, p.packed ? p.off : nullptr);
  }
  return launch_embed_bwd(p.idx, DX, e->G + e->tok_emb, dinjection, c.unk_token, p.B, p.T, C, c.n_tok, s, p.packed ? p.off : nullptr);
}

int gnn_fwd(coati_engine* e, const long long* atoms, const float* coords, hipStream_t s) {
  const coati_config& c = e->cfg;
  const int H = c.n_hidden_e3nn, Lg = c.n_layer_e3gnn, B = e->B, A = e->A, BA = B * A, Me = BA * A;
  {
    ProfScope ps(e, SITE_GNN_ELEMWISE, 0, s, (double)BA * (8 + H * 6 + 8) + (double)BA * 12 + (double)Me * 8 * 3 + (double)BA * 4, 20.0);
    bf16_t* h16 = Lg > 0 ? e->g_hcat[0] : e->g_hfin16;
    if (c.torch_emb) COATI_TRY(launch_gnn_embed(atoms, nullptr, nullptr, e->P + e->gembw, nullptr, e->g_h32[0], h16, Lg > 0 ? 2 * H : H, e->g_rstd[0], e->g_mask, BA, H, s, e->err_flag));
    else COATI_TRY(launch_gnn_embed(atoms, e->lut_ix, e->lut_iy, e->P + e->gembw, e->P + e->gembb, e->g_h32[0], h16, Lg > 0 ? 2 * H : H, e->g_rstd[0], e->g_mask, BA, H, s));
    COATI_TRY(launch_gnn_geom(coords, e->g_mask, c.msg_cutoff, e->g_d2, e->g_w, B, A, s));
    COATI_TRY(launch_gnn_compact(e->g_w, e->g_d2, e->g_seg, e->g_ne, e->g_ebj, e->g_ebk, e->g_erev, e->g_ed2, e->g_ew, e->g_pos, B, A, s));
  }
  for (int l = 0; l < Lg; ++l) {
    const GLayerP& w = e->gl[l];
    COATI_TRY(gemm(e, SITE_GNN_NODE_GEMM, e->g_hcat[l], 0, 2 * H, e->S + w.w1ab, H, BA, 2 * H, H, e->g_P[l], 2 * H, nullptr, EPI_BF16, nullptr, nullptr, 0, s));
    if (H == 256) {
      ProfScope ps(e, SITE_GNN_EDGE_GEMM, 0, s, (double)BA * (H * 2 + 4 + H * 2) + (double)H * H * 2, (double)H * 2 + 12 + (double)H * 4, 2.0 * H * H + 6.0 * H);
      COATI_TRY(launch_gnn_edge_fwd_fused(e->g_P[l], 2 * H, e->g_seg, e->g_ebk, e->g_ed2, e->g_ew, e->P + w.e0w + 2 * H, 2 * H + 1, e->P + w.e0b,
                                          e->S + w.e3w, H, e->P + w.e3b, e->g_e1[l], e->g_s2[l], e->g_hcat[l] + H, 2 * H, BA, H, s));
    } else {
    {
      ProfScope ps(e, SITE_GNN_ELEMWISE, 0, s, (double)BA * (H * 2 + 4), (double)H * 4 + 8, 4.0 * H);
      COATI_TRY(launch_gnn_edge_pre_c(e->g_P[l], 2 * H, e->g_seg, e->g_ebk, e->g_ed2, e->P + w.e0w + 2 * H, 2 * H + 1, e->P + w.e0b, e->g_e1[l], BA, H, s));
    }
    {
      GemmArgs a;
      memset(&a, 0, sizeof(a));
      a.m_dev = e->g_ne;
      a.A = e->g_e1[l]; a.lda = H; a.B = e->S + w.e3w; a.ldb = H; a.M = Me; a.N = H; a.K = H; a.C = e->g_s2[l]; a.ldc = H; a.bias = e->P + w.e3b;
      ProfScope ps(e, SITE_GNN_EDGE_GEMM, 0, s, (double)H * H * 2 + H * 4, (double)H * 4, 2.0 * H * H);
      COATI_TRY(launch_gemm_nt(a, 0, EPI_BF16, s));
    }
    {
      ProfScope ps(e, SITE_GNN_ELEMWISE, 0, s, (double)BA * (H * 2 + 4), (double)H * 2 + 4, 2.0 * H);
      COATI_TRY(launch_gnn_edge_reduce_c(e->g_s2[l], e->g_seg, e->g_ew, e->g_hcat[l] + H, 2 * H, BA, H, s));
    }
    }
    if (c.residual) {
      COATI_TRY(gemm(e, SITE_GNN_NODE_GEMM, e->g_hcat[l], 0, 2 * H, e->S + w.n0p, 2 * H, BA, H, 2 * H, e->g_o, H, e->P + w.n0b, EPI_F32, nullptr, nullptr, 0, s));
      ProfScope ps(e, SITE_GNN_ELEMWISE, 0, s, (double)BA * (H * 4 + 8 + H * 4));
      COATI_TRY(launch_gnn_node_res_silu(e->g_o, atoms, e->lut_ix, e->lut_iy, e->P + w.n0w + 2 * H, 2 * H + 28, e->g_upre[l], e->g_t[l], BA, H, s));
    } else {
      COATI_TRY(gemm(e, SITE_GNN_NODE_GEMM, e->g_hcat[l], 0, 2 * H, e->S + w.n0w, 2 * H, BA, H, 2 * H, e->g_t[l], H, e->P + w.n0b, EPI_SILU, nullptr, e->g_upre[l], H, s));
    }
    COATI_TRY(gemm(e, SITE_GNN_NODE_GEMM, e->g_t[l], 0, H, e->S + w.n3w, H, BA, H, H, e->g_o, H, e->P + w.n3b, EPI_RES_F32, e->g_h32[l], nullptr, H, s));
    {
      ProfScope ps(e, SITE_GNN_ELEMWISE, 0, s, (double)BA * (H * 4 + H * 4 + H * 2 + 4));
      const bool last = (l + 1 == Lg);
      COATI_TRY(launch_layernorm_fwd(e->g_o, H, nullptr, nullptr, last ? e->g_hfin16 : e->g_hcat[l + 1], last ? H : 2 * H, e->g_h32[l + 1], H, nullptr, e->g_rstd[l + 1], BA, H, s));
    }
  }
  COATI_TRY(gemm(e, SITE_GNN_NODE_GEMM, e->g_hfin16, 0, H, e->S + e->gd0w, H, BA, H, H, e->g_td, H, e->P + e->gd0b, EPI_SILU, nullptr, e->g_dpre, H, s));
  COATI_TRY(gemm(e, SITE_GNN_NODE_GEMM, e->g_td, 0, H, e->S + e->gd3w, H, BA, H, H, e->g_o2, H, e->P + e->gd3b, EPI_F32, nullptr, nullptr, 0, s));
  ProfScope ps(e, SITE_GNN_ELEMWISE, 0, s, (double)BA * (H * 4 + 4) + (double)B * H * 4);
  return launch_gnn_readout(e->g_o2, e->g_mask, e->hpoint, B, A, H, s);
}

int gnn_wgrad_group(coati_engine* e, hipStream_t s) {
  const coati_config& c = e->cfg;
  const int H = c.n_hidden_e3nn, Lg = c.n_layer_e3gnn, BA = e->B * e->A;
  const long long sig = (e->carve_sig * 1000003 + e->B) * 1000003 + e->A;
  if (e->gtab_sig != sig) {
    std::vector<WgradTile> tab;
    auto add = [&](const bf16_t* A_, int lda, const bf16_t* B_, int ldb, int N, int K, float* dW, int64_t ldw, float* db) -> int {
      WgradArgs a;
      a.A = A_; a.lda = lda; a.B = B_; a.ldb = ldb; a.M = BA; a.N = N; a.K = K; a.dW = dW; a.ldw = ldw; a.dbias = db; a.n_out = 0;
      return wgrad_table_append_split(tab, a, 4);
    };
    COATI_TRY(add(e->g_do2, H, e->g_td, H, H, H, e->G + e->gd3w, H, e->G + e->gd3b));
    COATI_TRY(add(e->g_dtd, H, e->g_hfin16, H, H, H, e->G + e->gd0w, H, e->G + e->gd0b));
    for (int l = Lg - 1; l >= 0; --l) {
      const GLayerP& w = e->gl[l];
      COATI_TRY(add(e->gl_DO16[l], H, e->g_t[l], H, H, H, e->G + w.n3w, H, e->G + w.n3b));
      COATI_TRY(add(e->gl_du[l], H, e->g_hcat[l], 2 * H, H, 2 * H, e->G + w.n0w, 2 * H + (c.residual ? 28 : 0), e->G + w.n0b));
      COATI_TRY(add(e->gl_dP[l], 2 * H, e->g_hcat[l], 2 * H, H, H, e->G + w.e0w, 2 * H + 1, nullptr));
      COATI_TRY(add(e->gl_dP[l] + H, 2 * H, e->g_hcat[l], 2 * H, H, H, e->G + w.e0w + H, 2 * H + 1, nullptr));
    }
    COATI_CHECK_ARG((int)tab.size() <= e->gtab_cap, "gnn wgrad group: table overflow (%zu > %d)", tab.size(), e->gtab_cap);
    COATI_TRY(upload_table(e, 4 + (e->gtab_rr++ & 1), tab, e->d_gtab, s, "gnn wgrad group"));
    e->gtab_n = (int)tab.size();
    e->gtab_sig = sig;
  }
  const double nprob = 2.0 + 4.0 * Lg + Lg;
  ProfScope ps(e, SITE_GNN_WGRAD, 2.0 * BA * H * H * nprob, s, nprob * ((double)BA * H * 4 + (double)H * H * 8));
  return launch_wgrad_split_table(e->d_gtab, e->gtab_n, s);
}

int gnn_bwd(coati_engine* e, const float* dhpoint, hipStream_t s) {
  const coati_config& c = e->cfg;
  const int H = c.n_hidden_e3nn, Lg = c.n_layer_e3gnn, B = e->B, A = e->A, BA = B * A, Me = BA * A;
  float *DH = e->g_DH, *DO = e->g_DO;
  const bool grp = e->gnn_wg_group;
  {
    ProfScope ps(e, SITE_GNN_ELEMWISE, 0, s, (double)B * H * 4 + (double)BA * (H * 2 + 4));
    COATI_TRY(launch_gnn_readout_bwd(dhpoint, e->g_mask, e->g_do2, B, A, H, s));
  }
  COATI_TRY(gemm(e, SITE_GNN_NODE_GEMM, e->g_do2, 0, H, e->S + e->gd3T, H, BA, H, H, e->g_dtd, H, nullptr, EPI_DSILU, e->g_dpre, nullptr, H, s));
  if (!grp) COATI_TRY(wgrad(e, SITE_GNN_WGRAD, e->g_do2, 0, H, e->g_td, H, BA, H, H, e->G + e->gd3w, H, e->G + e->gd3b, 0, s));
  COATI_TRY(gemm(e, SITE_GNN_NODE_GEMM, e->g_dtd, 0, H, e->S + e->gd0T, H, BA, H, H, DH, H, nullptr, EPI_F32, nullptr, nullptr, 0, s));
  if (!grp) COATI_TRY(wgrad(e, SITE_GNN_WGRAD, e->g_dtd, 0, H, e->g_hfin16, H, BA, H, H, e->G + e->gd0w, H, e->G + e->gd0b, 0, s));
  for (int l = Lg - 1; l >= 0; --l) {
    const GLayerP& w = e->gl[l];
    bf16_t* const DO16 = grp ? e->gl_DO16[l] : e->g_DO16;
    bf16_t* const du = grp ? e->gl_du[l] : e->g_du;
    bf16_t* const dP = grp ? e->gl_dP[l] : e->g_dP;
    {
      ProfScope ps(e, SITE_GNN_ELEMWISE, 0, s, (double)BA * (H * 4 + H * 4 + 4 + H * 4 + H * 2));
      COATI_TRY(launch_layernorm_bwd(DH, 1, H, e->g_h32[l + 1], H, 1, nullptr, e->g_rstd[l + 1], nullptr, nullptr, DO, DO16, nullptr, nullptr, e->ln_partial, BA, H, s));
    }
    COATI_TRY(gemm(e, SITE_GNN_NODE_GEMM, DO16, 0, H, e->S + w.n3T, H, BA, H, H, du, H, nullptr, EPI_DSILU, e->g_upre[l], nullptr, H, s));
    if (!grp) COATI_TRY(wgrad(e, SITE_GNN_WGRAD, DO16, 0, H, e->g_t[l], H, BA, H, H, e->G + w.n3w, H, e->G + w.n3b, 0, s));
    COATI_TRY(gemm(e, SITE_GNN_NODE_GEMM, du, 0, H, e->S + w.n0T, H, BA, H, H, DO, H, nullptr, EPI_ACC_F32, nullptr, nullptr, 0, s));
    COATI_TRY(gemm(e, SITE_GNN_NODE_GEMM, du, 0, H, e->S + w.n0T + (int64_t)H * H, H, BA, H, H, e->g_dmi, H, nullptr, EPI_BF16, nullptr, nullptr, 0, s));
    if (!grp) COATI_TRY(wgrad(e, SITE_GNN_WGRAD, du, 0, H, e->g_hcat[l], 2 * H, BA, H, 2 * H, e->G + w.n0w, 2 * H + (c.residual ? 28 : 0), e->G + w.n0b, 0, s));
    if (c.residual) {
      ProfScope ps(e, SITE_GNN_ELEMWISE, 0, s, (double)BA * (H * 2 + 8));
      COATI_TRY(launch_gnn_onehot_wgrad(e->atoms, e->lut_ix, e->lut_iy, du, e->G + w.n0w + 2 * H, 2 * H + 28, BA, H, s));
    }
    {
      ProfScope ps(e, SITE_GNN_ELEMWISE, 0, s, (double)BA * (H * 2 + 4), (double)H * 4 + 4, 6.0 * H);
      COATI_TRY(launch_gnn_edge_reduce_bwd_c(e->g_dmi, H, e->g_s2[l], e->g_seg, e->g_ew, e->g_ds2, BA, H, s));
    }
    {
      GemmArgs a;
      memset(&a, 0, sizeof(a));
      a.A = e->g_ds2; a.lda = H; a.B = e->S + w.e3T; a.ldb = H; a.M = Me; a.N = H; a.K = H; a.C = e->g_dpre1; a.ldc = H;
      a.P = e->g_P[l]; a.ldp = 2 * H; a.d2 = e->g_ed2; a.w1c = e->P + w.e0w + 2 * H; a.w1c_stride = 2 * H + 1;
      a.b1 = e->P + w.e0b; a.natom = A; a.H = H;
      a.m_dev = e->g_ne; a.e_bj = e->g_ebj; a.e_bk = e->g_ebk;
      ProfScope ps(e, SITE_GNN_EDGE_GEMM, 0, s, (double)H * H * 2, (double)H * 8 + 12, 2.0 * H * H + 8.0 * H);
      COATI_TRY(launch_gemm_nt(a, 0, EPI_EDGE_DPRE, s));
    }
    {
      WgradArgs a;
      a.A = e->g_ds2; a.lda = H; a.B = e->g_e1[l]; a.ldb = H; a.M = Me; a.N = H; a.K = H; a.dW = e->G + w.e3w; a.ldw = H; a.dbias = e->G + w.e3b;
      a.n_out = 0; a.m_dev = e->g_ne;
      ProfScope ps(e, SITE_GNN_WGRAD, 0, s, (double)H * H * 8, (double)H * 4, 2.0 * H * H);
      COATI_TRY(launch_wgrad(a, 0, s));
    }
    {
      ProfScope ps(e, SITE_GNN_ELEMWISE, 0, s, (double)BA * (H * 4 + 4), (double)H * 4 + 8, 4.0 * H);
      COATI_TRY(launch_gnn_edge_pre_bwd_c(e->g_dpre1, e->g_seg, e->g_erev, e->g_ed2, dP, 2 * H, e->G + w.e0w + 2 * H, 2 * H + 1, e->G + w.e0b, BA, H, s));
    }
    COATI_TRY(gemm(e, SITE_GNN_NODE_GEMM, dP, 0, 2 * H, e->S + w.w1abT, 2 * H, BA, H, 2 * H, DO, H, nullptr, EPI_ACC_F32, nullptr, nullptr, 0, s));
    if (!grp) {
      COATI_TRY(wgrad(e, SITE_GNN_WGRAD, dP, 0, 2 * H, e->g_hcat[l], 2 * H, BA, H, H, e->G + w.e0w, 2 * H + 1, nullptr, 0, s));
      COATI_TRY(wgrad(e, SITE_GNN_WGRAD, dP + H, 0, 2 * H, e->g_hcat[l], 2 * H, BA, H, H, e->G + w.e0w + H, 2 * H + 1, nullptr, 0, s));
    }
    float* t = DH; DH = DO; DO = t;
  }
  if (grp) COATI_TRY(gnn_wgrad_group(e, s));
  {
    ProfScope ps(e, SITE_GNN_ELEMWISE, 0, s, (double)BA * (H * 4 + H * 4 + 4 + H * 4) + (double)BA * (8 + H * 4) + 30.0 * H * 4);
    COATI_TRY(launch_layernorm_bwd(DH, 1, H, e->g_h32[0], H, 1, nullptr, e->g_rstd[0], nullptr, nullptr, DO, nullptr, nullptr, nullptr, e->ln_partial, BA, H, s));
    if (e->cfg.torch_emb) COATI_TRY(launch_gnn_embed_bwd(e->atoms, nullptr, nullptr, DO, e->G + e->gembw, nullptr, BA, H, s));
    else COATI_TRY(launch_gnn_embed_bwd(e->atoms, e->lut_ix, e->lut_iy, DO, e->G + e->gembw, e->G + e->gembb, BA, H, s));
  }
  return COATI_OK;
}

int head_linear_bwd(coati_engine* e, SgemmBatch& sb, const float* dY, const float* X, int64_t w_off, int64_t b_off, float* dX, int B,
                    int N, int K) {
  const float* W = e->P + w_off;
  COATI_TRY(sgemm_batch_add(sb, dY, 1, N, X, K, 1, e->G + w_off, K, N, K, B, nullptr, 1.f, 1));
  COATI_TRY(sgemm_batch_add(sb, e->ones, 0, 1, dY, N, 1, e->G + b_off, N, 1, N, B, nullptr, 1.f, 1));
  if (dX) COATI_TRY(sgemm_batch_add(sb, dY, N, 1, W, K, 1, dX, K, B, K, N, nullptr, 1.f, 0));
  return COATI_OK;
}

int ensure_side(coati_engine* e) {
  if (e->side) return COATI_OK;
  if (hipStreamCreateWithFlags(&e->side, hipStreamNonBlocking) != hipSuccess ||
      hipEventCreateWithFlags(&e->ev_fork, hipEventDisableTiming) != hipSuccess ||
      hipEventCreateWithFlags(&e->ev_join, hipEventDisableTiming) != hipSuccess) {
    coati_set_error("engine: could not create the side stream");
    return COATI_EHIP;
  }
  return COATI_OK;
}
int fork_side(coati_engine* e, hipStream_t main) {
  COATI_TRY(ensure_side(e));
  if (hipEventRecord(e->ev_fork, main) != hipSuccess || hipStreamWaitEvent(e->side, e->ev_fork, 0) != hipSuccess) {
    coati_set_error("engine: fork failed");
    return COATI_EHIP;
  }
  return COATI_OK;
}
int join_side(coati_engine* e, hipStream_t main) {
  if (hipEventRecord(e->ev_join, e->side) != hipSuccess || hipStreamWaitEvent(main, e->ev_join, 0) != hipSuccess) {
    coati_set_error("engine: join failed");
    return COATI_EHIP;
  }
  return COATI_OK;
}

int point_head_fwd(coati_engine* e, float* out, hipStream_t s) {
  const coati_config& c = e->cfg;
  const int H = c.n_hidden_e3nn, E = c.n_embd_common, B = e->B;
  if (!c.use_point_encoder) return COATI_OK;
  const float* x = e->hpoint;
  if (c.norm_clips && c.old_architecture) {
    COATI_TRY(launch_sgemm(x, H, 1, e->P + e->p2c_w, 1, H, e->hp_ln, E, B, E, H, e->P + e->p2c_b, 1.f, 0, s));
    return launch_layernorm_fwd(e->hp_ln, E, e->P + e->p2c_lnw, e->P + e->p2c_lnb, nullptr, 0, out, E, e->hp_mean, e->hp_rstd, B, E, s);
  }
  if (c.norm_clips) {
    COATI_TRY(launch_layernorm_fwd(e->hpoint, H, e->P + e->p2c_lnw, e->P + e->p2c_lnb, nullptr, 0, e->hp_ln, H, e->hp_mean, e->hp_rstd, B, H, s));
    x = e->hp_ln;
  }
  return launch_sgemm(x, H, 1, e->P + e->p2c_w, 1, H, out, E, B, E, H, e->P + e->p2c_b, 1.f, 0, s);
}
int smiles_head_fwd(coati_engine* e, float* out, hipStream_t s) {
  const coati_config& c = e->cfg;
  const int C = c.n_hidden_xformer, E = c.n_embd_common, B = e->B;
  const float* x = e->hstop;
  if (c.norm_clips && c.old_architecture) {
    COATI_TRY(launch_sgemm(x, C, 1, e->P + e->s2c_w, 1, C, e->hs_ln, E, B, E, C, e->P + e->s2c_b, 1.f, 0, s));
    return launch_layernorm_fwd(e->hs_ln, E, e->P + e->s2c_lnw, e->P + e->s2c_lnb, nullptr, 0, out, E, e->hs_mean, e->hs_rstd, B, E, s);
  }
  if (c.norm_clips) {
    COATI_TRY(launch_layernorm_fwd(e->hstop, C, e->P + e->s2c_lnw, e->P + e->s2c_lnb, nullptr, 0, e->hs_ln, C, e->hs_mean, e->hs_rstd, B, C, s));
    x = e->hs_ln;
  }
  return launch_sgemm(x, C, 1, e->P + e->s2c_w, 1, C, out, E, B, E, C, e->P + e->s2c_b, 1.f, 0, s);
}

int coati2_head_fwd(coati_engine* e, const coati_engine::Coati2Head& h, const coati_engine::Coati2Save& sv, const float* x, float* out, int B,
                    hipStream_t s) {
  const int C = e->cfg.n_hidden_xformer, E = e->cfg.n_embd_common;
  const float* P = e->P;
  COATI_TRY(launch_layernorm_fwd(x, C, P + h.lnw, P + h.lnb, nullptr, 0, sv.ln, C, sv.mean, sv.rstd, B, C, s));
  COATI_TRY(launch_sgemm(sv.ln, C, 1, P + h.w1, 1, C, sv.u, 2 * E, B, 2 * E, C, P + h.b1, 1.f, 0, s));
  COATI_TRY(launch_swiglu(sv.u, 2 * E, sv.g, E, B, E, s));
  COATI_TRY(launch_sgemm(sv.g, E, 1, P + h.w2, 1, E, out, E, B, E, E, P + h.b2, 1.f, 0, s));
  if (h.residual) COATI_TRY(launch_axpy(x, out, 1.f, (long long)B * E, s));
  return COATI_OK;
}

int coati2_head_bwd(coati_engine* e, const coati_engine::Coati2Head& h, const coati_engine::Coati2Save& sv, const float* x, const float* dy,
                    const float* dres, float* dx, int B, bool wgrad, hipStream_t s) {
  const int C = e->cfg.n_hidden_xformer, E = e->cfg.n_embd_common;
  const float* P = e->P;
  if (wgrad) {
    SgemmBatch sb;
    COATI_TRY(head_linear_bwd(e, sb, dy, sv.g, h.w2, h.b2, e->dsa, B, E, E));
    COATI_TRY(launch_sgemm_batch(sb, s));
  } else {
    COATI_TRY(launch_sgemm(dy, E, 1, P + h.w2, E, 1, e->dsa, E, B, E, E, nullptr, 1.f, 0, s));
  }
  COATI_TRY(launch_swiglu_bwd(sv.u, 2 * E, e->dsa, E, e->c2_du, 2 * E, B, E, s));
  if (wgrad) {
    SgemmBatch sb;
    COATI_TRY(head_linear_bwd(e, sb, e->c2_du, sv.ln, h.w1, h.b1, e->dhs_ln, B, 2 * E, C));
    COATI_TRY(launch_sgemm_batch(sb, s));
  } else {
    COATI_TRY(launch_sgemm(e->c2_du, 2 * E, 1, P + h.w1, C, 1, e->dhs_ln, C, B, C, 2 * E, nullptr, 1.f, 0, s));
  }
  return launch_layernorm_bwd(e->dhs_ln, 1, C, x, C, 0, sv.mean, sv.rstd, P + h.lnw, dres, dx, nullptr, wgrad ? e->G + h.lnw : nullptr,
                              wgrad ? e->G + h.lnb : nullptr, wgrad ? e->ln_partial : nullptr, B, C, s);
}

int begin_call(coati_engine* e, const char* entry, void* workspace, int64_t workspace_bytes, int B, int T1, int T2, int A, float* scal) {
  Arena ar{reinterpret_cast<char*>(workspace), 0, (size_t)workspace_bytes, false};
  const size_t need = carve(e, ar, B, T1, T2, A, B);
  COATI_CHECK_ARG((int64_t)need <= workspace_bytes, "%s: workspace too small (%zu > %lld)", entry, need, (long long)workspace_bytes);
  if (e->nce) e->nce_cap = ((size_t)workspace_bytes - (size_t)(reinterpret_cast<char*>(e->nce) - reinterpret_cast<char*>(workspace))) / sizeof(float);
  e->B = B; e->T1 = T1; e->T2 = T2; e->A = A;
  if (scal) e->scal = scal;
  e->have_fwd = false;
  e->decoder_pending = false;
  e->have_ws = true;
  return COATI_OK;
}
int clear_errors(coati_engine* e, float* scal, hipStream_t s) {
  if (scal) HIPCHK(hipMemsetAsync(scal, 0, 16 * sizeof(float), s));
  HIPCHK(hipMemsetAsync(e->err_flag, 0, 4 * sizeof(int), s));
  return COATI_OK;
}
int publish_errors(coati_engine* e, float* scal, hipStream_t s) {
  HIPCHK(hipMemcpyAsync(scal + 6, e->err_flag, sizeof(int), hipMemcpyDeviceToDevice, s));
  return COATI_OK;
}

int pack_pass(coati_engine* e, XPass& p, const long long* targets, int64_t rows, hipStream_t s) {
  COATI_TRY(launch_seq_pack(p.idx, targets, e->cfg.pad_token, p.B, p.T, (int)rows, p.off, p.row_src, p.row_t, targets ? p.ypk : nullptr, e->err_flag, s, p.ord));
  p.packed = true;
  p.M = (int)rows;
  return COATI_OK;
}

int stop_rows_head_fwd(coati_engine* e, float* out, hipStream_t s) {
  const XPass& p = e->p1;
  const int C = e->cfg.n_hidden_xformer;
  if (p.tail) HIPCHK(hipMemcpyAsync(e->hstop, p.t_xf, (size_t)p.B * C * sizeof(float), hipMemcpyDeviceToDevice, s));
  else COATI_TRY(launch_gather_rows(p.xf32, e->stop_pos, e->hstop, p.B, p.T, C, s, p.packed ? p.off : nullptr));
  if (e->enc_to_coati > 0) return coati2_head_fwd(e, e->c2s, e->c2s_sv, e->hstop, out, p.B, s);
  return smiles_head_fwd(e, out, s);
}
int token_tower_fwd(coati_engine* e, float* out, hipStream_t s) {
  COATI_TRY(launch_find_stop(e->p1.idx, e->cfg.stop_token, e->stop_pos, e->err_flag, e->p1.B, e->p1.T, s));
  COATI_TRY(xformer_fwd(e, e->p1, nullptr, s));
  return stop_rows_head_fwd(e, out, s);
}

int special_token_add(coati_engine* e, SgemmBatch& sb, const float* h, float* act, float* tok, const float** out, hipStream_t s) {
  const int E = e->cfg.n_embd_common, B = e->B;
  *out = h;
  if (!e->cfg.token_mlp) return COATI_OK;
  COATI_TRY(launch_silu_fwd(h, act, (long long)B * E, s));
  COATI_TRY(sgemm_batch_add(sb, act, E, 1, e->P + e->tokw, 1, E, tok, E, B, E, E, e->P + e->tokb, 1.f, 0));
// ... 1029 lines not shown
```

coati_amd/csrc/gnn.hip:

```cpp
#include "kernels.h"

#define IN_EPS 1e-5f

__global__ __launch_bounds__(256) void gnn_embed_kernel(const long long* __restrict__ atoms, const int* __restrict__ lut_ix,
                                                        const int* __restrict__ lut_iy, const float* __restrict__ W,
                                                        const float* __restrict__ bias, float* __restrict__ h32,
                                                        bf16_t* __restrict__ h16, long long ld16, float* __restrict__ rstd_out,
                                                        float* __restrict__ mask, int BA, int H, int* __restrict__ err) {
  const int lane = threadIdx.x & 63, wave = threadIdx.x >> 6;
  const int row = blockIdx.x * 4 + wave;
  if (row >= BA) return;
  long long z = atoms[row];
  if (lane == 0) mask[row] = z > 0 ? 1.f : 0.f;
  if (lut_ix == nullptr && z > 83 && lane == 0 && err != nullptr) atomicOr(err, 4);
  if (z < 0) z = 0;
  if (z > 119) z = 119;
  const bool table = lut_ix == nullptr;
  if (table && z > 83) z = 83;
  const int ix = table ? 0 : lut_ix[z], iy = table ? 0 : lut_iy[z];
  float e[16];
  float s = 0.f;
#pragma unroll
  for (int i = 0; i < 16; ++i) {
    const int c = lane + 64 * i;
    float v = 0.f;
    if (c < H) {
      if (table) {
        v = W[z * H + c];
      } else {
        v = bias[c];
        if (ix >= 0) v += W[c * 28 + ix];
        if (iy >= 0) v += W[c * 28 + iy];
      }
    }
    e[i] = v;
    s += v;
  }
  const float mean = wave_sum(s) / (float)H;
  float q = 0.f;
#pragma unroll
  for (int i = 0; i < 16; ++i)
    if (lane + 64 * i < H) q += (e[i] - mean) * (e[i] - mean);
  const float rstd = 1.0f / sqrtf(wave_sum(q) / (float)H + IN_EPS);
  if (lane == 0) rstd_out[row] = rstd;
#pragma unroll
  for (int i = 0; i < 16; ++i) {
    const int c = lane + 64 * i;
    if (c < H) {
      const float v = (e[i] - mean) * rstd;
      h32[(long long)row * H + c] = v;
      h16[(long long)row * ld16 + c] = f2bf(v);
    }
  }
}

int launch_gnn_embed(const long long* atoms, const int* lut_ix, const int* lut_iy, const float* W, const float* b,
                     float* h32, bf16_t* h16, long long ld16, float* rstd, float* mask, int BA, int H,
                     hipStream_t s, int* err) {
  COATI_CHECK_ARG(atoms && W && h32 && h16 && rstd && mask && ((lut_ix && lut_iy && b) || (!lut_ix && !lut_iy && !b)), "gnn_embed: null operand");
  COATI_CHECK_SHAPE(BA > 0 && H > 0 && H <= 1024, "gnn_embed: unsupported shape");
  hipLaunchKernelGGL(gnn_embed_kernel, dim3(cdiv(BA, 4)), dim3(256), 0, s, atoms, lut_ix, lut_iy, W, b, h32, h16, ld16, rstd, mask, BA, H, err);
  COATI_LAUNCH_CHECK("gnn_embed");
  return COATI_OK;
}

__global__ __launch_bounds__(256) void gnn_embed_bwd_kernel(const long long* __restrict__ atoms, const int* __restrict__ lut_ix,
                                                            const int* __restrict__ lut_iy, const float* __restrict__ de,
                                                            float* __restrict__ dW, float* __restrict__ db, int BA, int H,
                                                            int rows_per_chunk) {
  extern __shared__ float acc[];
  for (int i = threadIdx.x; i < 29 * H; i += blockDim.x) acc[i] = 0.f;
  __syncthreads();
  const int r0 = blockIdx.x * rows_per_chunk;
  int r1 = r0 + rows_per_chunk;
  if (r1 > BA) r1 = BA;
  for (int c = threadIdx.x; c < H; c += blockDim.x) {
    float bsum = 0.f;
    for (int row = r0; row < r1; ++row) {
      long long z = atoms[row];
      if (z < 0) z = 0;
      if (z > 119) z = 119;
      const int ix = lut_ix[z], iy = lut_iy[z];
      const float v = de[(long long)row * H + c];
      bsum += v;
      if (ix >= 0) acc[ix * H + c] += v;
      if (iy >= 0 && iy != ix) acc[iy * H + c] += v;
    }
    acc[28 * H + c] = bsum;
  }
  __syncthreads();
  for (int f = threadIdx.x; f < 28 * H; f += blockDim.x) {
    const int c = f / 28, i = f - c * 28;
    const float v = acc[i * H + c];
    if (v != 0.f) atomicAdd(dW + f, v);
  }
  for (int c = threadIdx.x; c < H; c += blockDim.x) atomicAdd(db + c, acc[28 * H + c]);
}

__global__ __launch_bounds__(256) void gnn_embed_table_bwd_kernel(const long long* __restrict__ atoms, const float* __restrict__ de,
                                                                  float* __restrict__ dT, int BA, int H, int rows_per_chunk) {
  const int r0 = blockIdx.x * rows_per_chunk;
  int r1 = r0 + rows_per_chunk;
  if (r1 > BA) r1 = BA;
  for (int c = threadIdx.x; c < H; c += blockDim.x) {
    float run = 0.f;
    long long zr = -1;
    for (int row = r0; row < r1; ++row) {
      long long z = atoms[row];
      if (z < 0) z = 0;
      if (z > 83) z = 83;
      if (z != zr) {
        if (zr >= 0 && run != 0.f) atomicAdd(dT + zr * H + c, run);
        zr = z;
        run = 0.f;
      }
      run += de[(long long)row * H + c];
    }
    if (zr >= 0 && run != 0.f) atomicAdd(dT + zr * H + c, run);
  }
}

int launch_gnn_embed_bwd(const long long* atoms, const int* lut_ix, const int* lut_iy, const float* de,
                         float* dW, float* db, int BA, int H, hipStream_t s) {
  if (lut_ix == nullptr && lut_iy == nullptr && db == nullptr) {
    COATI_CHECK_ARG(atoms && de && dW, "gnn_embed_bwd: null operand");
    const int rpc = 32;
    hipLaunchKernelGGL(gnn_embed_table_bwd_kernel, dim3(cdiv(BA, rpc)), dim3(256), 0, s, atoms, de, dW, BA, H, rpc);
    COATI_LAUNCH_CHECK("gnn_embed_table_bwd");
    return COATI_OK;
  }
  COATI_CHECK_ARG(atoms && lut_ix && lut_iy && de && dW && db, "gnn_embed_bwd: null operand");
  COATI_CHECK_SHAPE((size_t)29 * H * 4 <= 64 * 1024, "gnn_embed_bwd: H=%d too wide for the LDS accumulator", H);
  const int chunks = BA >= 4096 ? 128 : (BA >= 256 ? 8 : 1);
  const int rpc = cdiv(BA, chunks);
  hipLaunchKernelGGL(gnn_embed_bwd_kernel, dim3(cdiv(BA, rpc)), dim3(256), (size_t)29 * H * 4, s, atoms, lut_ix, lut_iy, de, dW, db, BA, H, rpc);
  COATI_LAUNCH_CHECK("gnn_embed_bwd");
  return COATI_OK;
}

__global__ __launch_bounds__(256) void gnn_node_res_silu_kernel(const float* __restrict__ u32, const long long* __restrict__ atoms,
                                                                const int* __restrict__ lut_ix, const int* __restrict__ lut_iy,
                                                                const float* __restrict__ W3c, long long ldw, bf16_t* __restrict__ upre,
                                                                bf16_t* __restrict__ t16, int BA, int H) {
  const int row = blockIdx.x;
  if (row >= BA) return;
  long long z = atoms[row];
  if (z < 0) z = 0;
  if (z > 119) z = 119;
  const int ix = lut_ix[z], iy = lut_iy[z];
  for (int c = threadIdx.x; c < H; c += blockDim.x) {
    float v = u32[(long long)row * H + c];
    if (ix >= 0) v += W3c[c * ldw + ix];
    if (iy >= 0 && iy != ix) v += W3c[c * ldw + iy];
    upre[(long long)row * H + c] = f2bf(v);
    t16[(long long)row * H + c] = f2bf(silu_f(v));
  }
}

int launch_gnn_node_res_silu(const float* u32, const long long* atoms, const int* lut_ix, const int* lut_iy, const float* W3c, long long ldw,
                             bf16_t* upre, bf16_t* t16, int BA, int H, hipStream_t s) {
  COATI_CHECK_ARG(u32 && atoms && lut_ix && lut_iy && W3c && upre && t16, "gnn_node_res_silu: null operand");
  hipLaunchKernelGGL(gnn_node_res_silu_kernel, dim3(BA), dim3(256), 0, s, u32, atoms, lut_ix, lut_iy, W3c, ldw, upre, t16, BA, H);
  COATI_LAUNCH_CHECK("gnn_node_res_silu");
  return COATI_OK;
}

__global__ __launch_bounds__(256) void gnn_onehot_wgrad_kernel(const long long* __restrict__ atoms, const int* __restrict__ lut_ix,
                                                               const int* __restrict__ lut_iy, const bf16_t* __restrict__ du,
                                                               float* __restrict__ dW, long long ldw, int BA, int H, int rows_per_chunk) {
  extern __shared__ float acc[];
  for (int i = threadIdx.x; i < 28 * H; i += blockDim.x) acc[i] = 0.f;
  __syncthreads();
  const int r0 = blockIdx.x * rows_per_chunk;
  int r1 = r0 + rows_per_chunk;
  if (r1 > BA) r1 = BA;
  for (int c = threadIdx.x; c < H; c += blockDim.x) {
    for (int row = r0; row < r1; ++row) {
      long long z = atoms[row];
      if (z < 0) z = 0;
      if (z > 119) z = 119;
      const int ix = lut_ix[z], iy = lut_iy[z];
      const float v = bf2f(du[(long long)row * H + c]);
      if (ix >= 0) acc[ix * H + c] += v;
      if (iy >= 0 && iy != ix) acc[iy * H + c] += v;
    }
  }
  __syncthreads();
  for (int f = threadIdx.x; f < 28 * H; f += blockDim.x) {
    const int c = f / 28, i = f - c * 28;
    const float v = acc[i * H + c];
    if (v != 0.f) atomicAdd(dW + c * ldw + i, v);
  }
}

int launch_gnn_onehot_wgrad(const long long* atoms, const int* lut_ix, const int* lut_iy, const bf16_t* du, float* dW, long long ldw, int BA,
                            int H, hipStream_t s) {
  COATI_CHECK_ARG(atoms && lut_ix && lut_iy && du && dW, "gnn_onehot_wgrad: null operand");
  COATI_CHECK_SHAPE((size_t)28 * H * 4 <= 64 * 1024, "gnn_onehot_wgrad: H=%d too wide for the LDS accumulator", H);
  const int chunks = BA >= 4096 ? 128 : (BA >= 256 ? 8 : 1);
  const int rpc = cdiv(BA, chunks);
  hipLaunchKernelGGL(gnn_onehot_wgrad_kernel, dim3(cdiv(BA, rpc)), dim3(256), (size_t)28 * H * 4, s, atoms, lut_ix, lut_iy, du, dW, ldw, BA, H, rpc);
  COATI_LAUNCH_CHECK("gnn_onehot_wgrad");
  return COATI_OK;
}

__global__ void gnn_geom_kernel(const float* __restrict__ coords, const float* __restrict__ mask, float rc,
                                float* __restrict__ d2o, float* __restrict__ wo, int B, int A) {
  const long long e = (long long)blockIdx.x * blockDim.x + threadIdx.x;
  const long long n = (long long)B * A * A;
  if (e >= n) return;
  const int k = (int)(e % A);
  const long long bj = e / A;
  const int j = (int)(bj % A);
  const long long b = bj / A;
  const float* xj = coords + (b * A + j) * 3;
  const float* xk = coords + (b * A + k) * 3;
  const float dx = xj[0] - xk[0], dy = xj[1] - xk[1], dz = xj[2] - xk[2];
  const float d2 = dx * dx + dy * dy + dz * dz;
  const float d = sqrtf(d2);
  const bool valid = (mask[b * A + j] > 0.f) && (mask[b * A + k] > 0.f) && (j != k) && (d < rc);
  float w = 0.f;
  if (valid) {
    const float c2 = -1.5f / (rc * rc), c3 = 0.5f / (rc * rc * rc);
    w = (d <= 0.f) ? 1.f : (1.f + c2 * d * d + c3 * d * d * d);
  }
  d2o[e] = d2;
  wo[e] = w;
}

int launch_gnn_geom(const float* coords, const float* mask, float cutoff, float* d2, float* w, int B, int A,
                    hipStream_t s) {
  COATI_CHECK_ARG(coords && mask && d2 && w, "gnn_geom: null operand");
  const long long n = (long long)B * A * A;
  hipLaunchKernelGGL(gnn_geom_kernel, dim3(cdiv(n, 256)), dim3(256), 0, s, coords, mask, cutoff, d2, w, B, A);
  COATI_LAUNCH_CHECK("gnn_geom");
  return COATI_OK;
}

__global__ void gnn_compact_count_kernel(const float* __restrict__ w, int* __restrict__ cnt, int BA, int A) {
  const int bj = blockIdx.x * blockDim.x + threadIdx.x;
  if (bj >= BA) return;
  int n = 0;
  for (int k = 0; k < A; ++k) n += w[(long long)bj * A + k] > 0.f;
  cnt[bj] = n;
}
__global__ __launch_bounds__(1024) void gnn_scan_kernel(const int* __restrict__ cnt, int* __restrict__ seg, int* __restrict__ total, int n) {
  __shared__ int wtot[16];
  const int t = threadIdx.x, lane = t & 63, wave = t >> 6, per = (n + 1023) / 1024;
  const int lo = t * per, hi = lo + per < n ? lo + per : n;
  int s = 0;
  for (int i = lo; i < hi; ++i) s += cnt[i];
  int incl = s;
#pragma unroll
  for (int off = 1; off < 64; off <<= 1) {
    const int v = __shfl_up(incl, off, 64);
    if (lane >= off) incl += v;
  }
  if (lane == 63) wtot[wave] = incl;
  __syncthreads();
  if (wave == 0) {
    int w = lane < 16 ? wtot[lane] : 0;
#pragma unroll
    for (int off = 1; off < 16; off <<= 1) {
      const int v = __shfl_up(w, off, 64);
      if (lane >= off) w += v;
    }
    if (lane < 16) wtot[lane] = w;
  }
  __syncthreads();
  int run = incl - s + (wave > 0 ? wtot[wave - 1] : 0);
  for (int i = lo; i < hi; ++i) { seg[i] = run; run += cnt[i]; }
  if (t == 1023) { seg[n] = wtot[15]; total[0] = wtot[15]; }
}
__global__ void gnn_compact_fill_kernel(const float* __restrict__ w, const float* __restrict__ d2, const int* __restrict__ seg,
                                        int* __restrict__ e_bj, int* __restrict__ e_bk, float* __restrict__ e_d2,
                                        float* __restrict__ e_w, int* __restrict__ pos, int BA, int A) {
  const int bj = blockIdx.x * blockDim.x + threadIdx.x;
  if (bj >= BA) return;
  const int b = bj / A;
  int e = seg[bj];
  for (int k = 0; k < A; ++k) {
    const long long slot = (long long)bj * A + k;
    const float ww = w[slot];
    if (ww > 0.f) {
      e_bj[e] = bj; e_bk[e] = b * A + k; e_d2[e] = d2[slot]; e_w[e] = ww;
      pos[slot] = e++;
    }
  }
}
// ... 77 lines not shown
  if (bj >= BA) return;
  const int e0 = seg[bj], n = seg[bj + 1] - e0;
  for (int c0 = 0; c0 < H; c0 += 256) {
    const bool act = c0 + lane * 4 < H;
    const int c = act ? c0 + lane * 4 : 0;
    float acc[4] = {0.f, 0.f, 0.f, 0.f};
    for (int base = 0; base < n; base += 64) {
      const int nn = n - base < 64 ? n - base : 64;
      const float my_w = lane < nn ? e_w[e0 + base + lane] : 0.f;
      for (int i0 = 0; i0 < nn; i0 += 4) {
        uint2 u[4];
        float ww[4];
#pragma unroll
        for (int q = 0; q < 4; ++q) {
          const int i = i0 + q < nn ? i0 + q : nn - 1;
          ww[q] = i0 + q < nn ? __builtin_bit_cast(float, __builtin_amdgcn_readlane(__builtin_bit_cast(int, my_w), i)) : 0.f;
          u[q] = *reinterpret_cast<const uint2*>(s2 + (long long)(e0 + base + i) * H + c);
        }
#pragma unroll
        for (int q = 0; q < 4; ++q) {
          acc[0] += silu_f(bflo(u[q].x)) * ww[q]; acc[1] += silu_f(bfhi(u[q].x)) * ww[q];
          acc[2] += silu_f(bflo(u[q].y)) * ww[q]; acc[3] += silu_f(bfhi(u[q].y)) * ww[q];
        }
      }
    }
    if (act) *reinterpret_cast<uint2*>(mi + (long long)bj * ldmi + c) = make_uint2(pack2bf(acc[0], acc[1]), pack2bf(acc[2], acc[3]));
  }
}
int launch_gnn_edge_reduce_c(const bf16_t* s2, const int* seg, const float* e_w, bf16_t* mi, long long ldmi, int BA, int H, hipStream_t s) {
  COATI_CHECK_ARG(s2 && seg && e_w && mi, "gnn_edge_reduce_c: null operand");
  COATI_CHECK_SHAPE(H % 4 == 0 && ldmi % 4 == 0, "gnn_edge_reduce_c: alignment");
  hipLaunchKernelGGL(gnn_edge_reduce_c_kernel, dim3(cdiv(BA, 4)), dim3(256), 0, s, s2, seg, e_w, mi, ldmi, BA, H);
  COATI_LAUNCH_CHECK("gnn_edge_reduce_c");
  return COATI_OK;
}

__global__ __launch_bounds__(256) void gnn_edge_reduce_bwd_c_kernel(const bf16_t* __restrict__ dmi, long long lddmi,
                                                                    const bf16_t* __restrict__ s2, const int* __restrict__ seg,
                                                                    const float* __restrict__ e_w, bf16_t* __restrict__ ds2, int BA, int H) {
  const int lane = threadIdx.x & 63, wave = threadIdx.x >> 6;
  const int bj = blockIdx.x * 4 + wave;
  if (bj >= BA) return;
  const int e0 = seg[bj], n = seg[bj + 1] - e0;
  for (int c0 = 0; c0 < H; c0 += 256) {
    const bool act = c0 + lane * 4 < H;
    const int c = act ? c0 + lane * 4 : 0;
    const uint2 ug = *reinterpret_cast<const uint2*>(dmi + (long long)bj * lddmi + c);
    const float g[4] = {bflo(ug.x), bfhi(ug.x), bflo(ug.y), bfhi(ug.y)};
    for (int base = 0; base < n; base += 64) {
      const int nn = n - base < 64 ? n - base : 64;
      const float my_w = lane < nn ? e_w[e0 + base + lane] : 0.f;
      for (int i0 = 0; i0 < nn; i0 += 4) {
        uint2 u[4];
#pragma unroll
        for (int q = 0; q < 4; ++q) u[q] = *reinterpret_cast<const uint2*>(s2 + (long long)(e0 + base + (i0 + q < nn ? i0 + q : nn - 1)) * H + c);
#pragma unroll
        for (int q = 0; q < 4; ++q) {
          if (i0 + q >= nn) break;
          const float ww = __builtin_bit_cast(float, __builtin_amdgcn_readlane(__builtin_bit_cast(int, my_w), i0 + q));
          if (act) *reinterpret_cast<uint2*>(ds2 + (long long)(e0 + base + i0 + q) * H + c) =
              make_uint2(pack2bf(g[0] * ww * dsilu_f(bflo(u[q].x)), g[1] * ww * dsilu_f(bfhi(u[q].x))),
                         pack2bf(g[2] * ww * dsilu_f(bflo(u[q].y)), g[3] * ww * dsilu_f(bfhi(u[q].y))));
        }
      }
    }
  }
}
int launch_gnn_edge_reduce_bwd_c(const bf16_t* dmi, long long lddmi, const bf16_t* s2, const int* seg, const float* e_w,
                                 bf16_t* ds2, int BA, int H, hipStream_t s) {
  COATI_CHECK_ARG(dmi && s2 && seg && e_w && ds2, "gnn_edge_reduce_bwd_c: null operand");
  COATI_CHECK_SHAPE(H % 4 == 0 && lddmi % 4 == 0, "gnn_edge_reduce_bwd_c: alignment");
  hipLaunchKernelGGL(gnn_edge_reduce_bwd_c_kernel, dim3(cdiv(BA, 4)), dim3(256), 0, s, dmi, lddmi, s2, seg, e_w, ds2, BA, H);
  COATI_LAUNCH_CHECK("gnn_edge_reduce_bwd_c");
  return COATI_OK;
}

#define EPB_WAVES 16
__global__ __launch_bounds__(64 * EPB_WAVES) void gnn_edge_pre_bwd_c_kernel(const bf16_t* __restrict__ dpre, const int* __restrict__ seg,
                                                                 const int* __restrict__ e_rev, const float* __restrict__ e_d2,
                                                                 bf16_t* __restrict__ dP, long long lddp, float* __restrict__ dw1c,
                                                                 long long dw1c_stride, float* __restrict__ db1, int BA, int H) {
  const int lane = threadIdx.x & 63, wave = threadIdx.x >> 6;
  for (int c0 = 0; c0 < H; c0 += 256) {
    const bool act = c0 + lane * 4 < H;
    const int c = act ? c0 + lane * 4 : 0;
    float sw[4] = {0.f, 0.f, 0.f, 0.f}, sb[4] = {0.f, 0.f, 0.f, 0.f};
    for (int bj = blockIdx.x * EPB_WAVES + wave; bj < BA; bj += gridDim.x * EPB_WAVES) {
      const int e0 = seg[bj], n = seg[bj + 1] - e0;
      float a[4] = {0.f, 0.f, 0.f, 0.f}, bsum[4] = {0.f, 0.f, 0.f, 0.f};
      for (int base = 0; base < n; base += 64) {
        const int nn = n - base < 64 ? n - base : 64;
        const int my_rev = lane < nn ? e_rev[e0 + base + lane] : 0;
        const float my_d2 = lane < nn ? e_d2[e0 + base + lane] : 0.f;
        for (int i0 = 0; i0 < nn; i0 += 4) {
          uint2 u[4], r[4];
          float dd[4];
#pragma unroll
          for (int q = 0; q < 4; ++q) {
            const bool ok = i0 + q < nn;
            const int i = ok ? i0 + q : nn - 1;
            const int rv = __builtin_amdgcn_readlane(my_rev, i);
            dd[q] = ok ? __builtin_bit_cast(float, __builtin_amdgcn_readlane(__builtin_bit_cast(int, my_d2), i)) : 0.f;
            u[q] = *reinterpret_cast<const uint2*>(dpre + (long long)(e0 + base + i) * H + c);
            r[q] = *reinterpret_cast<const uint2*>(dpre + (long long)rv * H + c);
            if (!ok) { u[q] = make_uint2(0, 0); r[q] = make_uint2(0, 0); }
          }
#pragma unroll
          for (int q = 0; q < 4; ++q) {
            const float x[4] = {bflo(u[q].x), bfhi(u[q].x), bflo(u[q].y), bfhi(u[q].y)};
#pragma unroll
            for (int i = 0; i < 4; ++i) { a[i] += x[i]; sw[i] = fmaf(x[i], dd[q], sw[i]); }
            bsum[0] += bflo(r[q].x); bsum[1] += bfhi(r[q].x); bsum[2] += bflo(r[q].y); bsum[3] += bfhi(r[q].y);
          }
        }
      }
#pragma unroll
      for (int i = 0; i < 4; ++i) sb[i] += a[i];
      if (act) {
        *reinterpret_cast<uint2*>(dP + (long long)bj * lddp + c) = make_uint2(pack2bf(a[0], a[1]), pack2bf(a[2], a[3]));
        *reinterpret_cast<uint2*>(dP + (long long)bj * lddp + H + c) = make_uint2(pack2bf(bsum[0], bsum[1]), pack2bf(bsum[2], bsum[3]));
      }
    }
    __shared__ float red[2][EPB_WAVES][256];
#pragma unroll
    for (int i = 0; i < 4; ++i) { red[0][wave][lane * 4 + i] = act ? sw[i] : 0.f; red[1][wave][lane * 4 + i] = act ? sb[i] : 0.f; }
    __syncthreads();
    if (wave == 0 && act) {
#pragma unroll
      for (int i = 0; i < 4; ++i) {
        const int k = lane * 4 + i;
        float t0 = 0.f, t1 = 0.f;
#pragma unroll
        for (int w = 0; w < EPB_WAVES; ++w) { t0 += red[0][w][k]; t1 += red[1][w][k]; }
        atomicAdd(dw1c + (long long)(c + i) * dw1c_stride, t0);
        atomicAdd(db1 + c + i, t1);
      }
    }
    __syncthreads();
  }
}
int launch_gnn_edge_pre_bwd_c(const bf16_t* dpre, const int* seg, const int* e_rev, const float* e_d2, bf16_t* dP, long long lddp,
                              float* dw1c, long long dw1c_stride, float* db1, int BA, int H, hipStream_t s) {
  COATI_CHECK_ARG(dpre && seg && e_rev && e_d2 && dP && dw1c && db1, "gnn_edge_pre_bwd_c: null operand");
  COATI_CHECK_SHAPE(H % 4 == 0 && lddp % 4 == 0, "gnn_edge_pre_bwd_c: alignment");
  int blocks = cdiv(BA, EPB_WAVES);
  if (blocks > 256) blocks = 256;
  hipLaunchKernelGGL(gnn_edge_pre_bwd_c_kernel, dim3(blocks), dim3(64 * EPB_WAVES), 0, s, dpre, seg, e_rev, e_d2, dP, lddp, dw1c, dw1c_stride, db1, BA, H);
  COATI_LAUNCH_CHECK("gnn_edge_pre_bwd_c");
  return COATI_OK;
}

__global__ __launch_bounds__(256) void gnn_readout_kernel(const float* __restrict__ o, const float* __restrict__ mask,
                                                          float* __restrict__ hp, int A, int H) {
  const int b = blockIdx.x;
  float n = 0.f;
  for (int a = 0; a < A; ++a) n += mask[b * A + a];
  n = fmaxf(n, 1.f);
  for (int c = threadIdx.x; c < H; c += blockDim.x) {
    float acc = 0.f;
    for (int a = 0; a < A; ++a) acc += o[((long long)b * A + a) * H + c] * mask[b * A + a];
    hp[(long long)b * H + c] = acc / n;
  }
}

int launch_gnn_readout(const float* o, const float* mask, float* hp, int B, int A, int H, hipStream_t s) {
  COATI_CHECK_ARG(o && mask && hp, "gnn_readout: null operand");
  hipLaunchKernelGGL(gnn_readout_kernel, dim3(B), dim3(256), 0, s, o, mask, hp, A, H);
  COATI_LAUNCH_CHECK("gnn_readout");
  return COATI_OK;
}

__global__ __launch_bounds__(256) void gnn_readout_bwd_kernel(const float* __restrict__ dhp, const float* __restrict__ mask,
                                                              bf16_t* __restrict__ dout, int A, int H) {
  const int b = blockIdx.x;
  float n = 0.f;
  for (int a = 0; a < A; ++a) n += mask[b * A + a];
  n = fmaxf(n, 1.f);
  for (int c = threadIdx.x; c < H; c += blockDim.x) {
    const float g = dhp[(long long)b * H + c] / n;
    for (int a = 0; a < A; ++a) dout[((long long)b * A + a) * H + c] = f2bf(g * mask[b * A + a]);
  }
}

int launch_gnn_readout_bwd(const float* dhp, const float* mask, bf16_t* dout, int B, int A, int H, hipStream_t s) {
  COATI_CHECK_ARG(dhp && mask && dout, "gnn_readout_bwd: null operand");
  hipLaunchKernelGGL(gnn_readout_bwd_kernel, dim3(B), dim3(256), 0, s, dhp, mask, dout, A, H);
  COATI_LAUNCH_CHECK("gnn_readout_bwd");
  return COATI_OK;
}
```

coati_amd/csrc/kernels.h:

```cpp
#pragma once
#include "common.h"

enum CoatiEpi {
  EPI_BF16 = 0,
  EPI_F32 = 1,
  EPI_RES_F32 = 2,
  EPI_GELU = 3,
  EPI_DGELU = 4,
  EPI_SILU = 5,
  EPI_DSILU = 6,
  EPI_ACC_F32 = 7,
  EPI_CE_PARTIAL = 8,
  EPI_CE_BWD = 9,
  EPI_EDGE_DPRE = 10,
  EPI_QKV_ROPE = 11,
  EPI_GELU_GRAD = 12,
  EPI_MUL_AUX = 13,
  EPI_LNBWD = 14,
  EPI_CE_BWD_ROW = 15,
  EPI_CE_LSE = 16,
  EPI_COUNT = 17
};

struct GemmArgs {
// ... 65 lines not shown
int gemm_ce_tile_width(const GemmArgs& a);
int launch_gemm_rb256(const GemmArgs& a, int epi, hipStream_t s);
bool gemm_rb16_supported(const GemmArgs& a, int a_f32, int epi);
bool gemm_rb16_resident_supported(const GemmArgs& a, int a_f32, int epi);
int launch_gemm_rb16_resident(const GemmArgs& a, int epi, hipStream_t s);
int launch_gemm_rb16(const GemmArgs& a, int epi, hipStream_t s);
#ifdef COATI_EXPERIMENTAL
struct Mlp64Args {
  const float* x;
  long long ldx;
  const float* gamma;
  const float* beta;
  bf16_t* a2;
  float* mean;
  float* rstd;
  const bf16_t* W1;
  const float* b1;
  const bf16_t* W2;
  const float* b2;
  bf16_t* g;
  unsigned char* codes;
  float* out;
  long long ldo;
  int M;
};
bool mlp64_fwd_supported(int M, int C, int hidden);
int launch_mlp64_fwd(const Mlp64Args& a, hipStream_t s);
bool gemm_t32_supported(const GemmArgs& a, int a_f32, int epi);
int launch_gemm_t32(const GemmArgs& a, int epi, hipStream_t s);
#endif
bool gemm_ring256_supported(const GemmArgs& a, int a_f32, int epi);
int launch_gemm_ring256(const GemmArgs& a, int epi, hipStream_t s);
int launch_gemm_mx8(const GemmArgs& a, const unsigned char* sa, const unsigned char* sb, int epi, hipStream_t s);
int launch_quant_mx8(const void* x, int x_f32, long long ldx, unsigned char* q, long long ldq, unsigned char* scales, int M, int K, hipStream_t s);

struct WgradArgs {
  const void* A;
  long long lda;
  const bf16_t* B;
  long long ldb;
  int M, N, K;
  float* dW;
  long long ldw;
  float* dbias;
  int n_out;
  const int* m_dev = nullptr;
  const float* b_gamma = nullptr;
  const float* b_beta = nullptr;
};
int launch_wgrad(const WgradArgs& a, int a_f32, hipStream_t s);
struct WgradTile {
  WgradArgs p;
  int tiles_k;
  int tile;
  int c_begin = 0, c_end = 0;
};
int launch_wgrad_table(const WgradTile* dev_table, int n_tiles, hipStream_t s, int tile_size = 128, int M_rt = 0, int b_affine = 1);
bool wgrad_table_tile256_ok(const WgradArgs& a);
int launch_wgrad_split_table(const WgradTile* dev_table, int n_entries, hipStream_t s);
#ifdef __cplusplus
#include <vector>
int wgrad_table_append(std::vector<WgradTile>& tab, const WgradArgs& a, int tile_size = 128);
int wgrad_table_append_split(std::vector<WgradTile>& tab, const WgradArgs& a, int n_splits);
#endif

#define SGEMM_BATCH_MAX 6
struct SgemmProb {
  const float *A, *B, *bias;
  float* C;
  long long ars, acs, brs, bcs, ldc;
  int M, N, K, accumulate, ksplit, tx, ty, tz, wg0;
  float alpha;
};
struct SgemmBatch {
  int n = 0;
  SgemmProb p[SGEMM_BATCH_MAX];
};
int sgemm_batch_add(SgemmBatch& b, const float* A, long long ars, long long acs, const float* B, long long brs, long long bcs,
                    float* C, long long ldc, int M, int N, int K, const float* bias, float alpha, int accumulate);
int launch_sgemm_batch(const SgemmBatch& b, hipStream_t s);
int launch_sgemm(const float* A, long long ars, long long acs, const float* B, long long brs, long long bcs,
                 float* C, long long ldc, int M, int N, int K, const float* bias, float alpha, int accumulate,
                 hipStream_t s);

int launch_layernorm_fwd(const float* x, long long ldx, const float* gamma, const float* beta, bf16_t* y16,
                         long long ld16, float* y32, long long ld32, float* mean, float* rstd, int M, int C,
                         hipStream_t s);
int launch_layernorm_bwd(const void* dy, int dy_f32, long long lddy, const float* x, long long ldx, int x_is_xhat,
                         const float* mean, const float* rstd, const float* gamma, const float* dres,
                         float* dx, bf16_t* dx16, float* dgamma, float* dbeta, float* partial, int M, int C, hipStream_t s);
int launch_layernorm_bwd_deferred(const void* dy, int dy_f32, long long lddy, const float* x, long long ldx, int x_is_xhat,
                                  const float* mean, const float* rstd, const float* gamma, const float* dres, float* dx,
                                  bf16_t* dx16, float* partial, int* nblk_out, int M, int C, hipStream_t s);
#define COATI_LN_MAX_SLOTS 72
struct LnFinishBatch {
  int n;
  long long dg_off[COATI_LN_MAX_SLOTS];
  long long db_off[COATI_LN_MAX_SLOTS];
  int nblk[COATI_LN_MAX_SLOTS];
};
int launch_ln_finish_batched(const float* partial, long long slot_stride, int nblk, float* grad_base, const LnFinishBatch& b,
                             int C, hipStream_t s);
#define COATI_LN_PARTIAL_ROWS 2048

int launch_attn_fwd(const bf16_t* qkv, bf16_t* y, float* lse, int B, int T, int n_head, int head_size, hipStream_t s,
                    const int* seq_off = nullptr, const int* seq_ord = nullptr);
int launch_attn_bwd(const bf16_t* qkv, const bf16_t* y, const bf16_t* dy, const float* lse, float* dscratch, bf16_t* dqkv,
                    const float* cos, const float* sin, int B, int T, int n_head, int head_size, hipStream_t s,
                    const int* seq_off = nullptr, const int* seq_ord = nullptr);
int launch_attn16_fwd(const bf16_t* qkv, bf16_t* y, float* lse, int B, int T, int n_head, hipStream_t s, const int* seq_off, const int* seq_ord = nullptr);
int launch_attn16_bwd(const bf16_t* qkv, const bf16_t* y, const bf16_t* dy, const float* lse, bf16_t* dqkv, const float* cos_t,
                      const float* sin_t, int B, int T, int n_head, hipStream_t s, const int* seq_off, const int* seq_ord = nullptr);

#ifdef COATI_EXPERIMENTAL
struct AttnBlockArgs {
  const float* x;
  float* xmid;
  const float* ln_g;
  const float* ln_b;
  float* mean;
  float* rstd;
  bf16_t* a1;
  const bf16_t* Wqkv;
  const float* bqkv;
  const bf16_t* Wproj;
  const float* bproj;
  bf16_t* qkv;
  bf16_t* y;
  float* lse;
  const float* cos_t;
  const float* sin_t;
  const int* row_src;
  const int* grp;
  int Tl, M;
};
bool attn_block_fwd_supported(int B, int T, int C, int n_head);
int launch_attn_groups(const int* seq_off, int B, int T, int* grp, hipStream_t s);
int launch_attn_block_fwd(const AttnBlockArgs& a, hipStream_t s);
int launch_ab_probe_swap(unsigned* out, hipStream_t s);
#endif

int launch_embed_fwd(const long long* idx, const float* table, const float* injection, int unk_token, float* x,
                     int B, int T, int C, int V, hipStream_t s, const int* row_src = nullptr, int rows = 0, int mode = 0);
int launch_embed_bwd(const long long* idx, const float* dx, float* dtable, float* dinjection, int unk_token,
                     int B, int T, int C, int V, hipStream_t s, const int* off = nullptr, int inj_only = 0);
int launch_seq_pack(const long long* tok, const long long* y, int pad_token, int B, int T, int rows_expect, int* off,
                    int* row_src, int* row_t, long long* ypk, int* err, hipStream_t s, int* ord = nullptr);
int launch_seq_pack_len(const int* len, int B, int T, int rows_expect, int* off, int* row_src, int* row_t, int* err, hipStream_t s,
                        int* ord = nullptr);
int launch_find_stop(const long long* idx, int stop_token, int* pos, int* err, int B, int T, hipStream_t s);
int launch_gather_rows(const float* x, const int* pos, float* out, int B, int T, int C, hipStream_t s, const int* off = nullptr);
int launch_scatter_rows_add(const float* dout, const int* pos, float* dx, int B, int T, int C, hipStream_t s, const int* off = nullptr);
int launch_scatter_rows_bf16(const bf16_t* src, const int* pos, bf16_t* dst, int B, int T, int C, hipStream_t s, const int* off = nullptr);
int launch_bad_rows(const long long* tokens, unsigned char* bad, int B, int T, hipStream_t s);
int launch_attn_decode(const bf16_t* qkv, bf16_t* cache, bf16_t* y, int B, int n_head, int head_size, int Tmax, int pos,
                       const int* pos_dev, hipStream_t s);
int launch_add_int(int* x, int v, int set, hipStream_t s);
int launch_attn_decode_rows(const bf16_t* qkv, bf16_t* cache, bf16_t* y, int B, int n_head, int head_size, int Tmax, const int* pos,
                            hipStream_t s);
int launch_decode_rows_prep(const int* pos, const int* inj_len, const long long* tokens, int* rope_t, long long* tok_inj, int B, int Tmax,
                            hipStream_t s);
int launch_topk_sample(const float* logits, long long ldl, int B, int V, int k, float inv_temp, const float* u,
                       long long* tok_out, int* stopped, int stop_token, int pad_token, hipStream_t s);
int launch_topk_sample_prompt(const float* logits, long long ldl, int B, int V, int k, float inv_temp, const float* u,
                              const long long* prompt, long long ldp, const int* plen, int pos, long long* tok_out, int* stopped,
                              int stop_token, int pad_token, hipStream_t s);
int launch_topk_sample_rows(const float* logits, long long ldl, int B, int V, int k, float inv_temp, const float* u, long long ldu,
                            const long long* prompt, long long ldp, const int* plen, const int* req, int* pos, long long* out,
                            long long ldo, long long* tok_next, int* done, int Tmax, int stop_token, hipStream_t s);
int launch_kv_cache_fill_rows(const bf16_t* qkv, bf16_t* cache, const int* row_src, int R, int B, int T, int n_head, int head_size,
                              int Tmax, hipStream_t s);
int launch_gather_last_rows(const float* x, const int* off, float* out, int B, int C, int R, hipStream_t s);
int launch_kv_cache_fill(const bf16_t* qkv, bf16_t* cache, int B, int m, int n_head, int head_size, int Tmax, hipStream_t s);
int launch_attn_decode_anc(const bf16_t* qkv, bf16_t* cache, bf16_t* y, int B, int n_head, int head_size, int Tmax, int pos,
                           const int* anc, hipStream_t s);
int launch_beam_row_topk(const float* logits, long long ldl, int G, int W, int V, const float* cum, const int* fin, int pad_token,
                         float* cand_score, int* cand_tok, hipStream_t s);
int launch_beam_merge(const float* cand_score, const int* cand_tok, int G, int W, const float* cum_in, const int* fin_in, const int* len_in,
                      const int* anc_in, const long long* hist_in, long long ldh, int Tmax, int pos, int n, int stop_token, float* cum_out,
                      int* fin_out, int* len_out, int* anc_out, long long* hist_out, long long* tok_next, int* nfin, hipStream_t s);
int launch_search_topk(const bf16_t* lib, long long N, int E, const float* bias, const bf16_t* q, int Q, int k, float alpha, int S,
                       float* part_score, int* part_row, float* out_score, long long* out_row, hipStream_t s);
int search_slices(long long N, int Q, int k);
int launch_grammar_step(float* logits, long long ldl, int B, int V, const unsigned long long* table, const int* state_in, int* state_out,
                        const long long* tok_prev, const int* parent, int remaining, int stop_token, hipStream_t s);
int launch_head_eval(const bf16_t* x, long long ldx, long long N, int E, const bf16_t* w0, const float* b0, const bf16_t* wr, const float* br,
                     int D, const float* wl, const float* bl, int P, int F, float* out, long long ldo, hipStream_t s);
int launch_head_grad(const bf16_t* x, long long ldx, long long N, int E, const bf16_t* w0, const float* b0, const bf16_t* wr, const float* br,
                     int D, const float* wl, const float* bl, int P, int F, const bf16_t* w0t, const bf16_t* wrt, const float* cot,
                     long long ldc, float* out, long long ldo, float* g, long long ldg, hipStream_t s);
int launch_head_gp(const bf16_t* x, long long ldx, long long N, int E, const bf16_t* w0, const float* b0, const bf16_t* wr, const float* br,
                   int D, int F, const float* wl, const float* bl, int P_lin, float* out, long long ldo, const bf16_t* z, const float* zn,
                   const float* alpha, const float* q, const float* c, float inv2l2, float s2, int P, int Mp, float* mean, long long ldm,
                   float* var, hipStream_t s);
int launch_head_gp_grad(const bf16_t* x, long long ldx, long long N, int E, const bf16_t* w0, const float* b0, const bf16_t* wr,
                        const float* br, int D, int F, const bf16_t* w0t, const bf16_t* wrt, const bf16_t* z, const bf16_t* zt,
                        const float* zn, const float* alpha, const float* qs, const float* c, float inv2l2, float s2, int P, int Mp,
                        const float* wm, float kappa, float var_add, int mode, float best, const float* rs, float* mean, long long ldm,
                        float* var, float* acq, float* g, long long ldg, hipStream_t s);
int launch_cluster_assign(const bf16_t* lib, long long N, int E, const float* row_bias, const bf16_t* c, int K, const float* cbias, int* assign,
                          float* best, int blocks, hipStream_t s);
int launch_cluster_sums(const bf16_t* lib, long long N, int E, const int* order, long long M, const int* offsets, const int* item_off, int K,
                        float* part, long long items_max, float* sums, int blocks, hipStream_t s);
int cluster_chunk(void);
long long cluster_items_max(long long M, int K);
int launch_ivf_scan(const bf16_t* lib, const int* ids, const float* bias, const int* list_off, long long M, int E, int L, const bf16_t* q, int Q,
                    const int* pair_q, const int* pair_off, const int* item_off, long long P, int k, float alpha, int seg_rows, int segs,
                    float* part_score, int* part_row, int blocks, hipStream_t s);
int launch_ivf_merge(const float* part_score, const int* part_row, const int* probes, const int* pair_slot, long long P, const int* list_off,
                     int L, int Q, int nprobe, int k, int seg_rows, int segs, float* out_score, long long* out_row, hipStream_t s);
long long ivf_plan(long long max_list_rows, int Q, int nprobe, int k);
int ivf_scan_grid(const char* what, long long M, int E, int L, int Q, long long P, int k, int seg_rows, int segs, int blocks);
int launch_ivf8_scan(const unsigned char* lib, const float* scale, const int* ids, const float* bias, const int* list_off, long long M, int E,
                     int L, const unsigned char* q, const float* qscale, int Q, const int* pair_q, const int* pair_off, const int* item_off,
                     long long P, int k, float alpha, int seg_rows, int segs, float* part_score, int* part_row, int blocks, hipStream_t s);
int launch_radius_count(const bf16_t* lib, long long N, int E, const float* bias, const bf16_t* q, int Q, float alpha, const float* sub,
                        int clamp0, const float* thr, const int* row_hi, int S, int* counts, hipStream_t s);
int launch_radius_fill(const bf16_t* lib, long long N, int E, const float* bias, const bf16_t* q, int Q, float alpha, const float* sub,
                       int clamp0, const float* thr, const int* row_hi, int S, const int* counts, const long long* offsets, float* out_score,
                       long long* out_row, hipStream_t s);
int radius_slices(long long N, int Q);
int launch_ivf_radius_count(const bf16_t* lib, const int* ids, const float* bias, const int* list_off, long long M, int E, int L, const bf16_t* q,
                            int Q, const int* pair_q, const int* pair_off, const int* item_off, long long P, float alpha, const float* sub,
                            int clamp0, const float* thr, const int* row_hi, int seg_rows, int segs, int* counts, int blocks, hipStream_t s);
int launch_ivf_radius_fill(const bf16_t* lib, const int* ids, const float* bias, const int* list_off, long long M, int E, int L, const bf16_t* q,
                           int Q, const int* pair_q, const int* pair_off, const int* item_off, long long P, float alpha, const float* sub,
                           int clamp0, const float* thr, const int* row_hi, int seg_rows, int segs, const int* counts, const long long* offsets,
                           float* out_score, long long* out_row, int blocks, hipStream_t s);
int launch_search_merge(const float* part_score, const int* part_row, int Q, int V, int k, float* out_score, long long* out_row, hipStream_t s);
int launch_quant_rows_fp8(const bf16_t* x, long long n, int E, unsigned char* out, float* scale, hipStream_t s);
int launch_search8_topk(const unsigned char* lib, const float* scale, long long N, int E, const float* bias, const unsigned char* q,
                        const float* qscale, int Q, int k, float alpha, int S, float* part_score, int* part_row, float* out_score,
                        long long* out_row, hipStream_t s);
int launch_search_rescore(const bf16_t* lib, long long N, int E, const float* bias, const bf16_t* q, int Q, const long long* cand, int R, int k,
                          float alpha, float* out_score, long long* out_row, hipStream_t s);
int search8_slices(long long N, int Q, int k);
int launch_pq_encode(const bf16_t* x, long long n, int E, const bf16_t* codebook, unsigned char* codes, hipStream_t s);
int launch_pq_topk(const unsigned char* codes, long long N, int E, const bf16_t* codebook, const float* bias, const bf16_t* q, int Q, int k,
                   float alpha, int S, float* part_score, int* part_row, float* out_score, long long* out_row, hipStream_t s);
int pq_k_max(int E);
int pq_slices(long long N, int E, int Q, int k);
int launch_ivfpq_scan(const unsigned char* codes, const int* ids, const float* bias, const int* list_off, long long M, int E, int L,
                      const bf16_t* centres, const bf16_t* codebook, const bf16_t* q, int Q, const int* pair_q, const int* pair_off,
                      const int* item_off, long long P, int k, float alpha, int seg_rows, int segs, float* part_score, int* part_row, int blocks,
                      hipStream_t s);
int ivfpq_k_max(int E);
int launch_quant_rows_fp4(const bf16_t* x, long long n, int E, unsigned char* codes, unsigned char* scales, hipStream_t s);
int launch_search4_topk(const unsigned char* codes, const unsigned char* scales, long long N, int E4, const float* bias, const unsigned char* q,
                        const float* qscale, int Q, int k, float alpha, int S, float* part_score, int* part_row, float* out_score,
                        long long* out_row, hipStream_t s);
int search4_slices(long long N, int Q, int k);
__device__ __forceinline__ int item_owner(const int* __restrict__ item_off, int n, long long item) {
  int lo = 0, hi = n;
  while (hi - lo > 1) {
    const int mid = (lo + hi) >> 1;
    if (item_off[mid] <= item) lo = mid; else hi = mid;
  }
  return lo;
}
int launch_batch_ncols(const long long* tok, int B, int S, int* ncols, hipStream_t s);
int launch_batch_tail(const long long* tok, int B, int S, int ncol, long long* tok_out, long long* y_out,
                      const long long* masked, int n_masked, hipStream_t s);

int launch_ce_finish(const float2* partial, int tiles_n, const bf16_t* a, long long lda, const bf16_t* W,
                     long long ldw, const long long* target, float* lse, float* scal, int M, int C, int V,
                     hipStream_t s);
int launch_ce_lse_finish(const bf16_t* a, long long lda, const bf16_t* W, long long ldw, const long long* target, const float* lse,
                         float* scal, int M, int C, int V, hipStream_t s);
int launch_ce_lse_finish_picked(const long long* target, const float* lse, const float* tl, float* scal, int M, int V, hipStream_t s);
int launch_ce_seq(const float2* partial, int tiles_n, const bf16_t* a, long long lda, const bf16_t* W, long long ldw,
                  const long long* target, const int* off, float* nll, int B, int T, int C, int V, hipStream_t s);
int launch_ce_seq_bwd(const float2* partial, int tiles_n, const bf16_t* a, long long lda, const bf16_t* W, long long ldw,
                      const long long* target, const int* off, const float* weights, float* nll, float* lse, float* row_scale, int B, int T,
                      int C, int V, hipStream_t s);

int launch_gnn_embed(const long long* atoms, const int* lut_ix, const int* lut_iy, const float* W, const float* b,
                     float* h32, bf16_t* h16, long long ld16, float* rstd, float* mask, int BA, int H,
                     hipStream_t s, int* err = nullptr);
int launch_gnn_node_res_silu(const float* u32, const long long* atoms, const int* lut_ix, const int* lut_iy, const float* W3c, long long ldw,
                             bf16_t* upre, bf16_t* t16, int BA, int H, hipStream_t s);
int launch_gnn_onehot_wgrad(const long long* atoms, const int* lut_ix, const int* lut_iy, const bf16_t* du, float* dW, long long ldw, int BA,
                            int H, hipStream_t s);
int launch_gnn_embed_bwd(const long long* atoms, const int* lut_ix, const int* lut_iy, const float* de,
                         float* dW, float* db, int BA, int H, hipStream_t s);
int launch_gnn_geom(const float* coords, const float* mask, float cutoff, float* d2, float* w, int B, int A,
                    hipStream_t s);
int launch_gnn_compact(const float* w_dense, const float* d2_dense, int* seg, int* n_edges, int* e_bj, int* e_bk, int* e_rev,
                       float* e_d2, float* e_w, int* pos, int B, int A, hipStream_t s);
int launch_gnn_edge_pre_c(const bf16_t* P, long long ldp, const int* seg, const int* e_bk, const float* e_d2, const float* w1c,
                          long long w1c_stride, const float* b1, bf16_t* e1, int BA, int H, hipStream_t s);
int launch_gnn_edge_reduce_c(const bf16_t* s2, const int* seg, const float* e_w, bf16_t* mi, long long ldmi, int BA, int H, hipStream_t s);
int launch_gnn_edge_fwd_fused(const bf16_t* P, long long ldp, const int* seg, const int* e_bk, const float* e_d2, const float* e_w,
                              const float* w1c, long long w1c_stride, const float* b1, const bf16_t* W3, long long ldw, const float* b3,
                              bf16_t* e1, bf16_t* s2, bf16_t* mi, long long ldmi, int BA, int H, hipStream_t s);
int launch_gnn_edge_reduce_bwd_c(const bf16_t* dmi, long long lddmi, const bf16_t* s2, const int* seg, const float* e_w,
                                 bf16_t* ds2, int BA, int H, hipStream_t s);
int launch_gnn_edge_pre_bwd_c(const bf16_t* dpre, const int* seg, const int* e_rev, const float* e_d2, bf16_t* dP, long long lddp,
                              float* dw1c, long long dw1c_stride, float* db1, int BA, int H, hipStream_t s);
int launch_gnn_readout(const float* o, const float* mask, float* hp, int B, int A, int H, hipStream_t s);
int launch_gnn_readout_bwd(const float* dhp, const float* mask, bf16_t* dout, int B, int A, int H, hipStream_t s);

int launch_silu_fwd(const float* x, float* y, long long n, hipStream_t s);
int launch_silu_bwd(const float* x, const float* dy, float* dx, long long n, int accumulate, hipStream_t s);
int launch_swiglu(const float* u, long long ldu, float* g, long long ldg, int B, int N, hipStream_t s);
int launch_swiglu_bwd(const float* u, long long ldu, const float* dg, long long lddg, float* du, long long lddu, int B, int N, hipStream_t s);
int launch_group_mean_rows(const float* x, long long ldx, const int* off, const float* w, const float* fallback, float* out, int G, int E,
                           hipStream_t s);
int launch_select_rows(const unsigned char* use_a, const float* a, const float* b, float* out, int B, int C,
                       hipStream_t s);
int launch_select_rows_bwd(const unsigned char* use_a, const float* dout, float* da, float* db, int B, int C,
                           hipStream_t s);
int launch_axpy(const float* x, float* y, float alpha, long long n, hipStream_t s);
int launch_infonce_rows2(float* logits, float* logits2, long long ld, int R, int N, int label0, const unsigned char* bad,
                         float* loss_sum, float* loss_sum2, const float* inv_count, float gscale, hipStream_t s);
int launch_infonce_rows(float* logits, long long ld, int R, int N, int label0, const unsigned char* bad,
                        float* loss_sum, const float* inv_count, float gscale, hipStream_t s);
int launch_count_valid(const unsigned char* bad, int n, float* out_count, float* out_inv, hipStream_t s);
int launch_colsum2(const float* a, const float* b2, const unsigned char* bad, float* out, int B, int E, hipStream_t s);
int launch_center_rows(const float* z, const unsigned char* bad, const float* sum, const float* count, float* zc, int B, int E, hipStream_t s);
int launch_standardize(const float* z, const unsigned char* bad, const float* stats, const float* count, float* zt, float* rsigma,
                       int B, int E, hipStream_t s);
int launch_barlow_dc(float* C, const float* count, float lam, float* loss, int E, hipStream_t s);
int launch_standardize_bwd(const float* dzt, const float* zt, const unsigned char* bad, const float* rsigma, const float* m,
                           const float* count, float scale, float* dz, int B, int E, hipStream_t s);

int launch_grad_sqnorm(const float* g, long long n, float* partial, int n_partial, float* out_norm, float max_norm,
                       float* out_coef, hipStream_t s);
int launch_adamw(float* p, const float* g, float* m, float* v, bf16_t* shadow, long long n, float lr, float b1,
                 float b2, float eps, float wd, int step, const float* coef, float gscale, hipStream_t s, const int* skip = nullptr);
int launch_cast_bf16(const float* src, bf16_t* dst, long long n, hipStream_t s);
int launch_transpose_cast(const float* src, long long ld_src, bf16_t* dst, long long ld_dst, int rows, int cols,
                          hipStream_t s);
int launch_pack_rows_cast(const float* src, long long ld_src, bf16_t* dst, long long ld_dst, int rows, int cols,
                          hipStream_t s);

struct ShadowJob {
  long long src_off, dst_off;
  int ld_src, ld_dst, rows, cols, transpose;
};
int launch_shadow_jobs(const ShadowJob* jobs, const int* tile_start, int n_jobs, int n_tiles, const float* P, bf16_t* S,
                       hipStream_t s);
```

Before: 50190 molecules/s.

## Fuse stop-row spreading, batch embed rows, and deterministic GNN embedding backward

Replaces the two memsets plus two scatters in the transformer backward tail with a single kernel that writes zero or the stop-row gradient into both the fp32 and bf16 buffers. The embedding forward now handles four rows per wave to put more loads in flight. The GNN embedding backward writes per-chunk partials into a workspace (reusing DH in the engine) and reduces them in a finish kernel, where it used to use atomics. The GNN readout loop is also unrolled for memory-level parallelism. It adds C API seam wrappers, and the C API path for embed backward allocates and syncs a temporary workspace.

```diff
diff --git a/coati_amd/_lib.py b/coati_amd/_lib.py
--- a/coati_amd/_lib.py
+++ b/coati_amd/_lib.py
@@ -99,6 +99,11 @@
         _SEARCH4_ABI = _abi.parse(_f.read(), guard="COATI_SEARCH4_H", name="coati_search4.h", base=_ABI)
 except OSError as e:
     raise RuntimeError(f"coati_amd: cannot read {_build.SEARCH4_HEADER}, which the binding of the four-bit search is derived from: {e}") from e
+try:
+    with open(_build.SEAMS_HEADER) as _f:
+        _SEAMS_ABI = _abi.parse(_f.read(), guard="COATI_SEAMS_H", name="coati_seams.h", base=_ABI)
+except OSError as e:
+    raise RuntimeError(f"coati_amd: cannot read {_build.SEAMS_HEADER}, which the binding of the step's seam kernels is derived from: {e}") from e
 
 PROTOTYPES = _ABI.prototypes
 CoatiConfig = _ABI.CoatiConfig
@@ -121,6 +126,7 @@
 PQ_PROTOTYPES = _PQ_ABI.prototypes
 IVFPQ_PROTOTYPES = _IVFPQ_ABI.prototypes
 SEARCH4_PROTOTYPES = _SEARCH4_ABI.prototypes
+SEAMS_PROTOTYPES = _SEAMS_ABI.prototypes
 
 _lib = None
 
@@ -143,14 +149,14 @@
         raise RuntimeError(f"coati_amd: {path} is missing and could not be built; there is no CPU fallback")
     import torch
     l = ctypes.CDLL(path)
-    for name, (restype, argtypes) in list(PROTOTYPES.items()) + list(BEAM_PROTOTYPES.items()) + list(SEARCH_PROTOTYPES.items()) + list(GRAMMAR_PROTOTYPES.items()) + list(SCREEN_PROTOTYPES.items()) + list(GUIDE_PROTOTYPES.items()) + list(LN_XHAT_PROTOTYPES.items()) + list(GP_PROTOTYPES.items()) + list(ACQ_PROTOTYPES.items()) + list(CLUSTER_PROTOTYPES.items()) + list(IVF_PROTOTYPES.items()) + list(RADIUS_PROTOTYPES.items()) + list(GNN_OPS_PROTOTYPES.items()) + list(SEARCH8_PROTOTYPES.items()) + list(IVF8_PROTOTYPES.items()) + list(IVF_RADIUS_PROTOTYPES.items()) + list(PQ_PROTOTYPES.items()) + list(IVFPQ_PROTOTYPES.items()) + list(SEARCH4_PROTOTYPES.items()):
+    for name, (restype, argtypes) in list(PROTOTYPES.items()) + list(BEAM_PROTOTYPES.items()) + list(SEARCH_PROTOTYPES.items()) + list(GRAMMAR_PROTOTYPES.items()) + list(SCREEN_PROTOTYPES.items()) + list(GUIDE_PROTOTYPES.items()) + list(LN_XHAT_PROTOTYPES.items()) + list(GP_PROTOTYPES.items()) + list(ACQ_PROTOTYPES.items()) + list(CLUSTER_PROTOTYPES.items()) + list(IVF_PROTOTYPES.items()) + list(RADIUS_PROTOTYPES.items()) + list(GNN_OPS_PROTOTYPES.items()) + list(SEARCH8_PROTOTYPES.items()) + list(IVF8_PROTOTYPES.items()) + list(IVF_RADIUS_PROTOTYPES.items()) + list(PQ_PROTOTYPES.items()) + list(IVFPQ_PROTOTYPES.items()) + list(SEARCH4_PROTOTYPES.items()) + list(SEAMS_PROTOTYPES.items()):
         if hasattr(l, name):
             getattr(l, name).restype = restype
             getattr(l, name).argtypes = argtypes
     if l.coati_abi_version() != ABI_VERSION:
         raise RuntimeError(f"coati_amd: {path} has ABI version {l.coati_abi_version()}, this package expects {ABI_VERSION}; "
                            "rebuild with `python -m coati_amd.build --force`")
-    missing = [n for n in exported_symbols() + sorted(BEAM_PROTOTYPES) + sorted(SEARCH_PROTOTYPES) + sorted(GRAMMAR_PROTOTYPES) + sorted(SCREEN_PROTOTYPES) + sorted(GUIDE_PROTOTYPES) + sorted(LN_XHAT_PROTOTYPES) + sorted(GP_PROTOTYPES) + sorted(ACQ_PROTOTYPES) + sorted(CLUSTER_PROTOTYPES) + sorted(IVF_PROTOTYPES) + sorted(RADIUS_PROTOTYPES) + sorted(GNN_OPS_PROTOTYPES) + sorted(SEARCH8_PROTOTYPES) + sorted(IVF8_PROTOTYPES) + sorted(IVF_RADIUS_PROTOTYPES) + sorted(PQ_PROTOTYPES) + sorted(IVFPQ_PROTOTYPES) + sorted(SEARCH4_PROTOTYPES) if not hasattr(l, n)]
+    missing = [n for n in exported_symbols() + sorted(BEAM_PROTOTYPES) + sorted(SEARCH_PROTOTYPES) + sorted(GRAMMAR_PROTOTYPES) + sorted(SCREEN_PROTOTYPES) + sorted(GUIDE_PROTOTYPES) + sorted(LN_XHAT_PROTOTYPES) + sorted(GP_PROTOTYPES) + sorted(ACQ_PROTOTYPES) + sorted(CLUSTER_PROTOTYPES) + sorted(IVF_PROTOTYPES) + sorted(RADIUS_PROTOTYPES) + sorted(GNN_OPS_PROTOTYPES) + sorted(SEARCH8_PROTOTYPES) + sorted(IVF8_PROTOTYPES) + sorted(IVF_RADIUS_PROTOTYPES) + sorted(PQ_PROTOTYPES) + sorted(IVFPQ_PROTOTYPES) + sorted(SEARCH4_PROTOTYPES) + sorted(SEAMS_PROTOTYPES) if not hasattr(l, n)]
     if missing:
         raise RuntimeError(f"coati_amd: {path} lacks symbols {missing[:6]}; rebuild with `python -m coati_amd.build --force`")
     _lib = l
diff --git a/coati_amd/build.py b/coati_amd/build.py
--- a/coati_amd/build.py
+++ b/coati_amd/build.py
@@ -27,6 +27,7 @@
 PQ_HEADER = os.path.join(os.path.dirname(HERE), "include", "coati_pq.h")
 IVFPQ_HEADER = os.path.join(os.path.dirname(HERE), "include", "coati_ivfpq.h")
 SEARCH4_HEADER = os.path.join(os.path.dirname(HERE), "include", "coati_search4.h")
+SEAMS_HEADER = os.path.join(os.path.dirname(HERE), "include", "coati_seams.h")
 HIP_UNITS = ["gemm.hip", "gemm_rb.hip", "gemm_rb16.hip", "gemm_ring.hip", "gemm_mx8.hip", "norm.hip", "attention.hip", "attention16.hip", "embed.hip", "gnn.hip", "loss.hip", "optim.hip", "batch.hip", "decode.hip", "beam.hip", "search.hip", "grammar.hip", "screen.hip", "guide.hip", "gp.hip", "gp_grad.hip", "cluster.hip", "ivf.hip", "radius.hip", "search8.hip", "ivf8.hip", "ivf_radius.hip", "pq.hip", "ivfpq.hip", "search4.hip"]
 CPP_UNITS = ["engine.cpp", "capi.cpp", "tokenizer.cpp", "comm.cpp"]
 FLAGS = ["--offload-arch=gfx950", "-O3", "-std=c++17", "-fPIC", "-Wno-unused-value", "-mllvm", "-amdgpu-mfma-vgpr-form=1"] + os.environ.get("COATI_AMD_CXXFLAGS", "").split()
@@ -51,7 +52,7 @@
     deps = [os.path.join(CSRC, f) for f in os.listdir(CSRC) if not os.path.isdir(os.path.join(CSRC, f))]
     if EXPERIMENTAL:
         deps += [os.path.join(CSRC, "experimental", f) for f in os.listdir(os.path.join(CSRC, "experimental"))]
-    deps += [HEADER, BEAM_HEADER, SEARCH_HEADER, GRAMMAR_HEADER, SCREEN_HEADER, GUIDE_HEADER, LN_XHAT_HEADER, GP_HEADER, ACQ_HEADER, CLUSTER_HEADER, IVF_HEADER, RADIUS_HEADER, GNN_OPS_HEADER, SEARCH8_HEADER, IVF8_HEADER, IVF_RADIUS_HEADER, PQ_HEADER, IVFPQ_HEADER, SEARCH4_HEADER]
+    deps += [HEADER, BEAM_HEADER, SEARCH_HEADER, GRAMMAR_HEADER, SCREEN_HEADER, GUIDE_HEADER, LN_XHAT_HEADER, GP_HEADER, ACQ_HEADER, CLUSTER_HEADER, IVF_HEADER, RADIUS_HEADER, GNN_OPS_HEADER, SEARCH8_HEADER, IVF8_HEADER, IVF_RADIUS_HEADER, PQ_HEADER, IVFPQ_HEADER, SEARCH4_HEADER, SEAMS_HEADER]
     return deps
 
 
diff --git a/coati_amd/csrc/capi.cpp b/coati_amd/csrc/capi.cpp
--- a/coati_amd/csrc/capi.cpp
+++ b/coati_amd/csrc/capi.cpp
@@ -19,6 +19,7 @@
 #include "../../include/coati_ivfpq.h"
 #include "../../include/coati_search4.h"
 #include "../../include/coati_gnn_ops.h"
+#include "../../include/coati_seams.h"
 #include <vector>
 #include "kernels.h"
 
@@ -257,6 +258,19 @@
                     int C, int V, void* stream) {
   return launch_embed_bwd(LL(idx), dx, dtable, dinjection, unk_token, B, T, C, V, S_(stream));
 }
+int coati_embed_fwd_rows(const int64_t* idx, const float* table, const float* injection, int unk_token, float* x, int B, int T, int C,
+                         int V, const int32_t* row_src, int rows, int mode, void* stream) {
+  COATI_CHECK_SHAPE(row_src == nullptr || rows > 0, "embed_fwd_rows: empty problem");
+  return launch_embed_fwd(LL(idx), table, injection, unk_token, x, B, T, C, V, S_(stream), row_src, rows, mode);
+}
+int coati_embed_bwd_rows(const int64_t* idx, const float* dx, float* dtable, float* dinjection, int unk_token, int B, int T, int C, int V,
+                         const int32_t* off, int inj_only, void* stream) {
+  return launch_embed_bwd(LL(idx), dx, dtable, dinjection, unk_token, B, T, C, V, S_(stream), off, inj_only);
+}
+int coati_spread_stop_rows(const float* src, const uint16_t* src16, const int32_t* pos, const int32_t* row_src, const int32_t* off, float* dx,
+                           uint16_t* dxb, int B, int M, int T, int C, void* stream) {
+  return launch_spread_stop_rows(src, src16, pos, row_src, off, dx, dxb, B, M, T, C, S_(stream));
+}
 int coati_find_stop(const int64_t* idx, int stop_token, int32_t* pos, int32_t* err, int B, int T, void* stream) {
   return launch_find_stop(LL(idx), stop_token, pos, err, B, T, S_(stream));
 }
@@ -512,7 +526,22 @@
 int coati_gnn_embed_bwd(const int64_t* atoms, const int32_t* lut_ix, const int32_t* lut_iy, const float* de, float* dW, float* db, int BA,
                         int H, void* stream) {
   COATI_CHECK_SHAPE(BA > 0 && H > 0, "gnn_embed_bwd: empty problem");
-  return launch_gnn_embed_bwd(LL(atoms), lut_ix, lut_iy, de, dW, db, BA, H, S_(stream));
+  const long long wsf = lut_ix != nullptr ? gnn_embed_bwd_ws_floats(BA, H) : 0;
+  float* ws = nullptr;
+  if (wsf > 0 && hipMalloc(&ws, (size_t)wsf * sizeof(float)) != hipSuccess) {
+    coati_set_error("gnn_embed_bwd: hipMalloc of %lld floats failed", wsf);
+    return COATI_EHIP;
+  }
+  const int rc = launch_gnn_embed_bwd(LL(atoms), lut_ix, lut_iy, de, dW, db, BA, H, S_(stream), ws);
+  if (ws != nullptr) {
+    const hipError_t h = hipStreamSynchronize(S_(stream));
+    (void)hipFree(ws);
+    if (rc == COATI_OK && h != hipSuccess) {
+      coati_set_error("gnn_embed_bwd: %s", hipGetErrorString(h));
+      return COATI_EHIP;
+    }
+  }
+  return rc;
 }
 int coati_gnn_readout(const float* o, const float* mask, float* hp, int B, int A, int H, void* stream) {
   COATI_CHECK_SHAPE(B > 0 && A > 0 && H > 0, "gnn_readout: empty problem");
diff --git a/coati_amd/csrc/embed.hip b/coati_amd/csrc/embed.hip
--- a/coati_amd/csrc/embed.hip
+++ b/coati_amd/csrc/embed.hip
@@ -1,31 +1,45 @@
 #include "kernels.h"
 
+#define EMB_FWD_ROWS 4
 __global__ __launch_bounds__(256) void embed_fwd_kernel(const long long* __restrict__ idx, const float* __restrict__ table,
                                                         const float* __restrict__ injection, int unk, float* __restrict__ x,
                                                         int M, int T, int C, int V, const int* __restrict__ row_src, int mode) {
   const int lane = threadIdx.x & 63, wave = threadIdx.x >> 6;
-  const int m = blockIdx.x * 4 + wave;
-  if (m >= M) return;
-  const int ms = row_src ? row_src[m] : m;
-  long long tok = idx[ms];
-  const float* src;
-  if (mode != 0) {
-    if (tok != unk) return;
-    float* dstz = x + (long long)m * C;
-    if (mode == 2) {
-      for (int c = lane * 4; c < C; c += 256) *reinterpret_cast<float4*>(dstz + c) = make_float4(0.f, 0.f, 0.f, 0.f);
-      return;
-    }
-    src = injection + (long long)(ms / T) * C;
-  } else if (injection != nullptr && tok == unk) {
-    src = injection + (long long)(ms / T) * C;
-  } else {
-    if (tok < 0) tok = 0;
-    if (tok >= V) tok = V - 1;
-    src = table + tok * C;
-  }
-  float* dst = x + (long long)m * C;
-  for (int c = lane * 4; c < C; c += 256) *reinterpret_cast<float4*>(dst + c) = *reinterpret_cast<const float4*>(src + c);
+  const int m0 = (blockIdx.x * 4 + wave) * EMB_FWD_ROWS;
+  if (m0 >= M) return;
+  const float* src[EMB_FWD_ROWS];
+  bool own[EMB_FWD_ROWS];
+#pragma unroll
+  for (int r = 0; r < EMB_FWD_ROWS; ++r) {
+    src[r] = nullptr;
+    own[r] = false;
+    const int m = m0 + r;
+    if (m >= M) continue;
+    const int ms = row_src ? row_src[m] : m;
+    long long tok = idx[ms];
+    if (mode != 0) {
+      if (tok != unk) continue;
+      own[r] = true;
+      if (mode == 1) src[r] = injection + (long long)(ms / T) * C;
+    } else if (injection != nullptr && tok == unk) {
+      own[r] = true;
+      src[r] = injection + (long long)(ms / T) * C;
+    } else {
+      if (tok < 0) tok = 0;
+      if (tok >= V) tok = V - 1;
+      own[r] = true;
+      src[r] = table + tok * C;
+    }
+  }
+  for (int c = lane * 4; c < C; c += 256) {
+    float4 v[EMB_FWD_ROWS];
+#pragma unroll
+    for (int r = 0; r < EMB_FWD_ROWS; ++r)
+      v[r] = src[r] != nullptr ? *reinterpret_cast<const float4*>(src[r] + c) : make_float4(0.f, 0.f, 0.f, 0.f);
+#pragma unroll
+    for (int r = 0; r < EMB_FWD_ROWS; ++r)
+      if (own[r]) *reinterpret_cast<float4*>(x + (long long)(m0 + r) * C + c) = v[r];
+  }
 }
 
 int launch_embed_fwd(const long long* idx, const float* table, const float* injection, int unk_token, float* x,
@@ -33,7 +47,7 @@
   COATI_CHECK_ARG(idx && x && (mode != 0 || table) && (mode != 1 || injection) && mode >= 0 && mode <= 2, "embed_fwd: null operand / bad mode");
   COATI_CHECK_SHAPE(B > 0 && T > 0 && C % 4 == 0 && V > 0, "embed_fwd: unsupported shape");
   const int M = row_src ? rows : B * T;
-  hipLaunchKernelGGL(embed_fwd_kernel, dim3(cdiv(M, 4)), dim3(256), 0, s, idx, table, injection, unk_token, x, M, T, C, V, row_src, mode);
+  hipLaunchKernelGGL(embed_fwd_kernel, dim3(cdiv(M, 4 * EMB_FWD_ROWS)), dim3(256), 0, s, idx, table, injection, unk_token, x, M, T, C, V, row_src, mode);
   COATI_LAUNCH_CHECK("embed_fwd");
   return COATI_OK;
 }
@@ -173,6 +187,39 @@
   return COATI_OK;
 }
 
+__global__ __launch_bounds__(256) void spread_stop_rows_kernel(const float* __restrict__ src, const bf16_t* __restrict__ src16,
+                                                               const int* __restrict__ pos, const int* __restrict__ row_src,
+                                                               const int* __restrict__ off, float* __restrict__ dx, bf16_t* __restrict__ dxb,
+                                                               int M, int T, int C) {
+  const int per_row = C >> 3;
+  const long long g = (long long)blockIdx.x * 256 + threadIdx.x;
+  if (g >= (long long)M * per_row) return;
+  const int m = (int)(g / per_row), c = (int)(g - (long long)m * per_row) << 3;
+  const int ms = row_src ? row_src[m] : m;
+  const int b = ms / T, t = ms - b * T;
+  const bool hit = pos[b] == t && (off == nullptr || off[b] + t == m);
+  float4 v0 = make_float4(0.f, 0.f, 0.f, 0.f), v1 = v0;
+  uint4 h = make_uint4(0u, 0u, 0u, 0u);
+  if (hit) {
+    const float4 a0 = *reinterpret_cast<const float4*>(src + (long long)b * C + c);
+    const float4 a1 = *reinterpret_cast<const float4*>(src + (long long)b * C + c + 4);
+    v0 = make_float4(0.f + a0.x, 0.f + a0.y, 0.f + a0.z, 0.f + a0.w);
+    v1 = make_float4(0.f + a1.x, 0.f + a1.y, 0.f + a1.z, 0.f + a1.w);
+    h = *reinterpret_cast<const uint4*>(src16 + (long long)b * C + c);
+  }
+  *reinterpret_cast<float4*>(dx + (long long)m * C + c) = v0;
+  *reinterpret_cast<float4*>(dx + (long long)m * C + c + 4) = v1;
+  *reinterpret_cast<uint4*>(dxb + (long long)m * C + c) = h;
+}
+int launch_spread_stop_rows(const float* src, const bf16_t* src16, const int* pos, const int* row_src, const int* off, float* dx, bf16_t* dxb,
+                            int B, int M, int T, int C, hipStream_t s) {
+  COATI_CHECK_ARG(src && src16 && pos && dx && dxb && (row_src == nullptr) == (off == nullptr), "spread_stop_rows: null operand");
+  COATI_CHECK_SHAPE(B > 0 && M > 0 && T > 0 && C > 0 && C % 8 == 0 && (row_src != nullptr || M == (long long)B * T), "spread_stop_rows: unsupported shape");
+  hipLaunchKernelGGL(spread_stop_rows_kernel, dim3((unsigned)cdiv((long long)M * (C >> 3), 256)), dim3(256), 0, s, src, src16, pos, row_src, off, dx, dxb, M, T, C);
+  COATI_LAUNCH_CHECK("spread_stop_rows");
+  return COATI_OK;
+}
+
 int launch_scatter_rows_add(const float* dout, const int* pos, float* dx, int B, int T, int C, hipStream_t s, const int* off) {
   COATI_CHECK_ARG(dout && pos && dx, "scatter_rows_add: null operand");
   hipLaunchKernelGGL(scatter_rows_add_kernel, dim3(cdiv(B, 4)), dim3(256), 0, s, dout, pos, dx, B, T, C, off);
diff --git a/coati_amd/csrc/engine.cpp b/coati_amd/csrc/engine.cpp
--- a/coati_amd/csrc/engine.cpp
+++ b/coati_amd/csrc/engine.cpp
@@ -1058,12 +1058,7 @@
       {
         ProfScope ps(e, SITE_XF_TAIL, 0, s, (double)Bt * C * (2 + 4 + 4 + 4 + 2));
         COATI_TRY(launch_layernorm_bwd(e->t_da, 0, C, p.t_xmid, C, 0, p.t_mean2, p.t_rstd2, e->P + w.ln2w, e->t_dx, e->t_dx, e->t_dxb, e->G + w.ln2w, e->G + w.ln2b, e->ln_partial, Bt, C, s));
-        if (hipMemsetAsync(DX, 0, (size_t)M * C * sizeof(float), s) != hipSuccess || hipMemsetAsync(dxb, 0, (size_t)M * C * sizeof(bf16_t), s) != hipSuccess) {
-          coati_set_error("xformer_bwd: hipMemsetAsync failed");
-          return COATI_EHIP;
-        }
-        COATI_TRY(launch_scatter_rows_add(e->t_dx, e->stop_pos, DX, Bt, p.T, C, s, p.packed ? p.off : nullptr));
-        COATI_TRY(launch_scatter_rows_bf16(e->t_dxb, e->stop_pos, dxb, Bt, p.T, C, s, p.packed ? p.off : nullptr));
+        COATI_TRY(launch_spread_stop_rows(e->t_dx, e->t_dxb, e->stop_pos, p.packed ? p.row_src : nullptr, p.packed ? p.off : nullptr, DX, dxb, Bt, M, p.T, C, s));
       }
     } else {
       if (c.use_fp8) {
@@ -1293,7 +1288,10 @@
     ProfScope ps(e, SITE_GNN_ELEMWISE, 0, s, (double)BA * (H * 4 + H * 4 + 4 + H * 4) + (double)BA * (8 + H * 4) + 30.0 * H * 4);
     COATI_TRY(launch_layernorm_bwd(DH, 1, H, e->g_h32[0], H, 1, nullptr, e->g_rstd[0], nullptr, nullptr, DO, nullptr, nullptr, nullptr, e->ln_partial, BA, H, s));
     if (e->cfg.torch_emb) COATI_TRY(launch_gnn_embed_bwd(e->atoms, nullptr, nullptr, DO, e->G + e->gembw, nullptr, BA, H, s));
-    else COATI_TRY(launch_gnn_embed_bwd(e->atoms, e->lut_ix, e->lut_iy, DO, e->G + e->gembw, e->G + e->gembb, BA, H, s));
+    else {
+      COATI_CHECK_SHAPE(gnn_embed_bwd_ws_floats(BA, H) <= (long long)BA * H, "gnn_backward: %d x %d leaves no room for the embedding backward's partials", BA, H);
+      COATI_TRY(launch_gnn_embed_bwd(e->atoms, e->lut_ix, e->lut_iy, DO, e->G + e->gembw, e->G + e->gembb, BA, H, s, DH));
+    }
   }
   return COATI_OK;
 }
diff --git a/coati_amd/csrc/gnn.hip b/coati_amd/csrc/gnn.hip
--- a/coati_amd/csrc/gnn.hip
+++ b/coati_amd/csrc/gnn.hip
@@ -64,37 +64,82 @@
   return COATI_OK;
 }
 
+#define GEB_ROWS 64
+#define GEB_DEPTH 16
 __global__ __launch_bounds__(256) void gnn_embed_bwd_kernel(const long long* __restrict__ atoms, const int* __restrict__ lut_ix,
                                                             const int* __restrict__ lut_iy, const float* __restrict__ de,
-                                                            float* __restrict__ dW, float* __restrict__ db, int BA, int H,
-                                                            int rows_per_chunk) {
+                                                            float* __restrict__ dW, float* __restrict__ db, float* __restrict__ part,
+                                                            int BA, int H) {
   extern __shared__ float acc[];
+  __shared__ int six[GEB_ROWS], siy[GEB_ROWS];
   for (int i = threadIdx.x; i < 29 * H; i += blockDim.x) acc[i] = 0.f;
+  const int r0 = blockIdx.x * GEB_ROWS;
+  if (threadIdx.x < GEB_ROWS) {
+    int ix = -1, iy = -1;
+    if (r0 + (int)threadIdx.x < BA) {
+      long long z = atoms[r0 + threadIdx.x];
+      if (z < 0) z = 0;
+      if (z > 119) z = 119;
+      ix = lut_ix[z];
+      iy = lut_iy[z];
+    }
+    six[threadIdx.x] = ix;
+    siy[threadIdx.x] = iy;
+  }
   __syncthreads();
-  const int r0 = blockIdx.x * rows_per_chunk;
-  int r1 = r0 + rows_per_chunk;
-  if (r1 > BA) r1 = BA;
   for (int c = threadIdx.x; c < H; c += blockDim.x) {
     float bsum = 0.f;
-    for (int row = r0; row < r1; ++row) {
-      long long z = atoms[row];
-      if (z < 0) z = 0;
-      if (z > 119) z = 119;
-      const int ix = lut_ix[z], iy = lut_iy[z];
-      const float v = de[(long long)row * H + c];
-      bsum += v;
-      if (ix >= 0) acc[ix * H + c] += v;
-      if (iy >= 0 && iy != ix) acc[iy * H + c] += v;
-    }
-    acc[28 * H + c] = bsum;
-  }
+    for (int j0 = 0; j0 < GEB_ROWS && r0 + j0 < BA; j0 += GEB_DEPTH) {
+      float v[GEB_DEPTH];
+#pragma unroll
+      for (int j = 0; j < GEB_DEPTH; ++j) v[j] = r0 + j0 + j < BA ? de[(long long)(r0 + j0 + j) * H + c] : 0.f;
+#pragma unroll
+      for (int j = 0; j < GEB_DEPTH; ++j) {
+        const int ix = six[j0 + j], iy = siy[j0 + j];
+        bsum += v[j];
+        if (ix >= 0) acc[ix * H + c] += v[j];
+        if (iy >= 0 && iy != ix) acc[iy * H + c] += v[j];
+      }
+    }
+    if (gridDim.x == 1) {
+      for (int i = 0; i < 28; ++i) {
+        const float s = acc[i * H + c];
+        if (s != 0.f) dW[c * 28 + i] += s;
+      }
+      db[c] += bsum;
+    } else {
+      float* out = part + (long long)blockIdx.x * 29 * H + c;
+      for (int i = 0; i < 28; ++i) out[i * H] = acc[i * H + c];
+      out[28 * H] = bsum;
+    }
+  }
+}
+
+__global__ __launch_bounds__(256) void gnn_embed_bwd_finish_kernel(const float* __restrict__ part, float* __restrict__ dW, float* __restrict__ db,
+                                                                   int chunks, int H) {
+  __shared__ float red[4][64];
+  const int lane = threadIdx.x & 63, wave = threadIdx.x >> 6;
+  const int i = blockIdx.x, c = blockIdx.y * 64 + lane;
+  const int per = (chunks + 3) >> 2;
+  const int k0 = wave * per, k1 = k0 + per < chunks ? k0 + per : chunks;
+  float s = 0.f;
+  if (c < H) {
+    const float* src = part + (long long)i * H + c;
+    for (int k = k0; k < k1; k += GEB_DEPTH) {
+      float v[GEB_DEPTH];
+#pragma unroll
+      for (int j = 0; j < GEB_DEPTH; ++j) v[j] = k + j < k1 ? src[(long long)(k + j) * 29 * H] : 0.f;
+#pragma unroll
+      for (int j = 0; j < GEB_DEPTH; ++j) s += v[j];
+    }
+  }
+  red[wave][lane] = s;
   __syncthreads();
-  for (int f = threadIdx.x; f < 28 * H; f += blockDim.x) {
-    const int c = f / 28, i = f - c * 28;
-    const float v = acc[i * H + c];
-    if (v != 0.f) atomicAdd(dW + f, v);
-  }
-  for (int c = threadIdx.x; c < H; c += blockDim.x) atomicAdd(db + c, acc[28 * H + c]);
+  if (wave == 0 && c < H) {
+    const float tot = ((red[0][lane] + red[1][lane]) + red[2][lane]) + red[3][lane];
+    if (i == 28) db[c] += tot;
+    else if (tot != 0.f) dW[c * 28 + i] += tot;
+  }
 }
 
 __global__ __launch_bounds__(256) void gnn_embed_table_bwd_kernel(const long long* __restrict__ atoms, const float* __restrict__ de,
@@ -120,8 +165,13 @@
   }
 }
 
+long long gnn_embed_bwd_ws_floats(int BA, int H) {
+  const int chunks = cdiv(BA, GEB_ROWS);
+  return chunks > 1 ? (long long)chunks * 29 * H : 0;
+}
+
 int launch_gnn_embed_bwd(const long long* atoms, const int* lut_ix, const int* lut_iy, const float* de,
-                         float* dW, float* db, int BA, int H, hipStream_t s) {
+                         float* dW, float* db, int BA, int H, hipStream_t s, float* ws) {
   if (lut_ix == nullptr && lut_iy == nullptr && db == nullptr) {
     COATI_CHECK_ARG(atoms && de && dW, "gnn_embed_bwd: null operand");
     const int rpc = 32;
@@ -131,10 +181,14 @@
   }
   COATI_CHECK_ARG(atoms && lut_ix && lut_iy && de && dW && db, "gnn_embed_bwd: null operand");
   COATI_CHECK_SHAPE((size_t)29 * H * 4 <= 64 * 1024, "gnn_embed_bwd: H=%d too wide for the LDS accumulator", H);
-  const int chunks = BA >= 4096 ? 128 : (BA >= 256 ? 8 : 1);
-  const int rpc = cdiv(BA, chunks);
-  hipLaunchKernelGGL(gnn_embed_bwd_kernel, dim3(cdiv(BA, rpc)), dim3(256), (size_t)29 * H * 4, s, atoms, lut_ix, lut_iy, de, dW, db, BA, H, rpc);
+  const int chunks = cdiv(BA, GEB_ROWS);
+  COATI_CHECK_ARG(chunks == 1 || ws != nullptr, "gnn_embed_bwd: %d chunks need the workspace", chunks);
+  hipLaunchKernelGGL(gnn_embed_bwd_kernel, dim3(chunks), dim3(256), (size_t)29 * H * 4, s, atoms, lut_ix, lut_iy, de, dW, db, ws, BA, H);
   COATI_LAUNCH_CHECK("gnn_embed_bwd");
+  if (chunks > 1) {
+    hipLaunchKernelGGL(gnn_embed_bwd_finish_kernel, dim3(29, cdiv(H, 64)), dim3(256), 0, s, ws, dW, db, chunks, H);
+    COATI_LAUNCH_CHECK("gnn_embed_bwd_finish");
+  }
   return COATI_OK;
 }
 
@@ -518,14 +572,29 @@
 
 __global__ __launch_bounds__(256) void gnn_readout_kernel(const float* __restrict__ o, const float* __restrict__ mask,
                                                           float* __restrict__ hp, int A, int H) {
+  constexpr int RO_DEPTH = 8;
   const int b = blockIdx.x;
-  float n = 0.f;
-  for (int a = 0; a < A; ++a) n += mask[b * A + a];
-  n = fmaxf(n, 1.f);
+  const float* __restrict__ ob = o + (long long)b * A * H;
+  const float* __restrict__ mb = mask + (long long)b * A;
   for (int c = threadIdx.x; c < H; c += blockDim.x) {
-    float acc = 0.f;
-    for (int a = 0; a < A; ++a) acc += o[((long long)b * A + a) * H + c] * mask[b * A + a];
-    hp[(long long)b * H + c] = acc / n;
+    float acc = 0.f, n = 0.f;
+    for (int a0 = 0; a0 < A; a0 += RO_DEPTH) {
+      float v[RO_DEPTH], mk[RO_DEPTH];
+#pragma unroll
+      for (int j = 0; j < RO_DEPTH; ++j) {
+        const bool in = a0 + j < A;
+        v[j] = in ? ob[(long long)(a0 + j) * H + c] : 0.f;
+        mk[j] = in ? mb[a0 + j] : 0.f;
+      }
+#pragma unroll
+      for (int j = 0; j < RO_DEPTH; ++j) {
+        if (a0 + j < A) {
+          n += mk[j];
+          acc += v[j] * mk[j];
+        }
+      }
+    }
+    hp[(long long)b * H + c] = acc / fmaxf(n, 1.f);
   }
 }
 
diff --git a/coati_amd/csrc/kernels.h b/coati_amd/csrc/kernels.h
--- a/coati_amd/csrc/kernels.h
+++ b/coati_amd/csrc/kernels.h
@@ -241,6 +241,8 @@
 int launch_gather_rows(const float* x, const int* pos, float* out, int B, int T, int C, hipStream_t s, const int* off = nullptr);
 int launch_scatter_rows_add(const float* dout, const int* pos, float* dx, int B, int T, int C, hipStream_t s, const int* off = nullptr);
 int launch_scatter_rows_bf16(const bf16_t* src, const int* pos, bf16_t* dst, int B, int T, int C, hipStream_t s, const int* off = nullptr);
+int launch_spread_stop_rows(const float* src, const bf16_t* src16, const int* pos, const int* row_src, const int* off, float* dx, bf16_t* dxb,
+                            int B, int M, int T, int C, hipStream_t s);
 int launch_bad_rows(const long long* tokens, unsigned char* bad, int B, int T, hipStream_t s);
 int launch_attn_decode(const bf16_t* qkv, bf16_t* cache, bf16_t* y, int B, int n_head, int head_size, int Tmax, int pos,
                        const int* pos_dev, hipStream_t s);
@@ -370,8 +372,9 @@
                              bf16_t* upre, bf16_t* t16, int BA, int H, hipStream_t s);
 int launch_gnn_onehot_wgrad(const long long* atoms, const int* lut_ix, const int* lut_iy, const bf16_t* du, float* dW, long long ldw, int BA,
                             int H, hipStream_t s);
+long long gnn_embed_bwd_ws_floats(int BA, int H);
 int launch_gnn_embed_bwd(const long long* atoms, const int* lut_ix, const int* lut_iy, const float* de,
-                         float* dW, float* db, int BA, int H, hipStream_t s);
+                         float* dW, float* db, int BA, int H, hipStream_t s, float* ws = nullptr);
 int launch_gnn_geom(const float* coords, const float* mask, float cutoff, float* d2, float* w, int B, int A,
                     hipStream_t s);
 int launch_gnn_compact(const float* w_dense, const float* d2_dense, int* seg, int* n_edges, int* e_bj, int* e_bk, int* e_rev,
diff --git a/include/coati_seams.h b/include/coati_seams.h
--- /dev/null
+++ b/include/coati_seams.h
@@ -0,0 +1,21 @@
+#ifndef COATI_SEAMS_H
+#define COATI_SEAMS_H
+
+#include "coati_hip.h"
+
+#ifdef __cplusplus
+extern "C" {
+#endif
+
+int coati_embed_fwd_rows(const int64_t* idx, const float* table, const float* injection, int unk_token, float* x, int B, int T, int C,
+                         int V, const int32_t* row_src, int rows, int mode, void* stream);
+int coati_embed_bwd_rows(const int64_t* idx, const float* dx, float* dtable, float* dinjection, int unk_token, int B, int T, int C, int V,
+                         const int32_t* off, int inj_only, void* stream);
+int coati_spread_stop_rows(const float* src, const uint16_t* src16, const int32_t* pos, const int32_t* row_src, const int32_t* off, float* dx,
+                           uint16_t* dxb, int B, int M, int T, int C, void* stream);
+
+#ifdef __cplusplus
+}
+#endif
+
+#endif
```

Result: no change. 50130 molecules/s (-0.1%).
